# Soltanilara/av-aloha

Measured on AMD Instinct MI355X. Metric: env-steps/sec (whole node) at 4096 parallel envs, SlotInsertion-3Arms, higher is better.
Workload: dtype f32

## Files before the change

### av_aloha_amd/build.py

```python
import os
import subprocess
import sys

HERE = os.path.dirname(os.path.abspath(__file__))
ROOT = os.path.dirname(HERE)
LIB = os.path.join(HERE, "libavsim.so")
SRC = os.path.join(HERE, "csrc")


def _stale(target, sources):
    if not os.path.exists(target):
        return True
    t = os.path.getmtime(target)
    return any(os.path.getmtime(s) > t for s in sources)


def build_hip(force=False, verbose=False):
    srcs = [os.path.join(SRC, f) for f in sorted(os.listdir(SRC)) if not f.endswith(".o") and not f.startswith(".")] + [os.path.join(ROOT, "include", "avsim.h"), os.path.abspath(__file__)]
    if not force and not _stale(LIB, srcs):
        return LIB
    import fcntl
    with open(os.path.join(SRC, ".build.lock"), "w") as lock:
        fcntl.flock(lock, fcntl.LOCK_EX)
        if not force and not _stale(LIB, srcs):
            return LIB
        return _build_hip_locked(verbose)


def _build_hip_locked(verbose):
    hipcc = os.environ.get("HIPCC", "/opt/rocm/bin/hipcc")
    common = [hipcc, "--offload-arch=gfx950", "-std=c++17", "-fPIC", "-fno-gpu-rdc", "-c"]
    F32_FLAGS = ["-O2", "-fno-hip-fp32-correctly-rounded-divide-sqrt", "-fgpu-flush-denormals-to-zero", "-fno-slp-vectorize", "-fno-vectorize",
                 "-mllvm", "-amdgpu-atomic-optimizer-strategy=None", "-mllvm", "-amdgpu-sched-strategy=max-ilp"]
    units = [
        ("avsim_api", F32_FLAGS + (["-DAVSIM_RENDER_STATS"] if os.environ.get("AVSIM_RENDER_STATS") else []) + os.environ.get("AVSIM_EXTRA_FLAGS", "").split()),
        ("avsim_phys_spec", F32_FLAGS + os.environ.get("AVSIM_EXTRA_FLAGS", "").split()),
        ("avsim_phys_f64", ["-O3", "-ffp-contract=off", "-mllvm", "-amdgpu-sched-strategy=max-ilp"] + os.environ.get("AVSIM_EXTRA_FLAGS_F64", "").split()),
        ("avsim_imgaug", ["-O3", "-ffp-contract=off", "-fhip-fp32-correctly-rounded-divide-sqrt", "-fno-gpu-flush-denormals-to-zero"] + os.environ.get("AVSIM_EXTRA_FLAGS_IMGAUG", "").split()),
        ("avsim_chunks", ["-O3", "-ffp-contract=off", "-fhip-fp32-correctly-rounded-divide-sqrt", "-fno-gpu-flush-denormals-to-zero"] + os.environ.get("AVSIM_EXTRA_FLAGS_CHUNKS", "").split()),
        ("avsim_obshist", ["-O3", "-ffp-contract=off", "-fhip-fp32-correctly-rounded-divide-sqrt", "-fno-gpu-flush-denormals-to-zero"] + os.environ.get("AVSIM_EXTRA_FLAGS_OBSHIST", "").split()),
        ("avsim_imgresize", ["-O3", "-ffp-contract=off", "-fhip-fp32-correctly-rounded-divide-sqrt", "-fno-gpu-flush-denormals-to-zero"] + os.environ.get("AVSIM_EXTRA_FLAGS_IMGRESIZE", "").split()),
        ("avsim_pointcloud", ["-O3", "-ffp-contract=off", "-fhip-fp32-correctly-rounded-divide-sqrt", "-fno-gpu-flush-denormals-to-zero"] + os.environ.get("AVSIM_EXTRA_FLAGS_POINTCLOUD", "").split()),
    ]
    procs = []
    for name, extra in units:
        cmd = common + extra + ["-o", os.path.join(SRC, name + ".o"), os.path.join(SRC, name + ".hip")]
        if verbose:
            print(" ".join(cmd), file=sys.stderr)
        procs.append((cmd, subprocess.Popen(cmd)))
    for cmd, p in procs:
        if p.wait() != 0:
            raise subprocess.CalledProcessError(p.returncode, cmd)
    tmp = LIB + ".tmp%d" % os.getpid()
    link = [hipcc, "--offload-arch=gfx950", "-shared", "-fPIC", "-fno-gpu-rdc", "-o", tmp] + [os.path.join(SRC, n + ".o") for n, _ in units]
    if verbose:
        print(" ".join(link).replace(tmp, LIB), file=sys.stderr)
    subprocess.check_call(link)
    os.replace(tmp, LIB)
    return LIB


def build_oracle(force=False):
    d = os.path.join(ROOT, "oracle")
    so = os.path.join(d, "liborc.so")
    srcs = [os.path.join(d, f) for f in os.listdir(d) if f.endswith((".c", ".h"))]
    if force or _stale(so, srcs):
        subprocess.check_call(["make", "-C", d, "-B", "liborc.so"], stdout=subprocess.DEVNULL)
    return so


if __name__ == "__main__":
    print(build_hip(force="--force" in sys.argv, verbose=True))
    print(build_oracle(force="--force" in sys.argv))
```

### av_aloha_amd/csrc/avsim_collide.hip.h

```cpp
#pragma once
#include "avsim_math.hip.h"

namespace avs {

enum { G_SPHERE = 2, G_CYLINDER = 5, G_BOX = 6, G_MESH = 7 };
constexpr int SLOT_W = 24, SLOT_P = 5, SLOT_N = 20, SLOT_MAXC = 5;
constexpr int BOX_MAXC = 8, BOX_SLOTC = 4, BOX_OVF_W = 16;

template <typename T>
struct Shape {
    int type;
    T size[3];
    T pos[3];
    T mat[9];
    GLB_PTR(const T) hull;
    int hbase, hR, hovf;
    int nh;
    T center[3];
    T lc[3], lh[3];
};

template <typename T> struct TieTol;
template <> struct TieTol<double> { static constexpr double rel = 1e-9, len = 1e-12; };
template <> struct TieTol<float> { static constexpr float rel = 1e-5f, len = 1e-7f; };

template <typename T> AVS_DEV T sel3c(const T* v, int k) { return k == 0 ? v[0] : (k == 1 ? v[1] : v[2]); }

template <typename T>
AVS_DEV void support(const Shape<T>& s, const T* d, T* out) {
    T l[3], p[3] = {0, 0, 0};
    mulmatT(s.mat, d, l);
    const T lz = TieTol<T>::rel * (fabs(l[0]) + fabs(l[1]) + fabs(l[2]));
    switch (s.type) {
        case G_SPHERE: {
            T n = sqrt(dot3(l, l));
            if (n > T(0)) { T k = s.size[0] / n; p[0] = k * l[0]; p[1] = k * l[1]; p[2] = k * l[2]; }
            break;
        }
        case G_BOX:
            p[0] = l[0] >= -lz ? s.size[0] : -s.size[0];
            p[1] = l[1] >= -lz ? s.size[1] : -s.size[1];
            p[2] = l[2] >= -lz ? s.size[2] : -s.size[2];
            break;
        case G_CYLINDER: {
            T n = sqrt(l[0] * l[0] + l[1] * l[1]);
            if (n > lz) { T k = s.size[0] / n; p[0] = k * l[0]; p[1] = k * l[1]; }
            p[2] = l[2] >= -lz ? s.size[1] : -s.size[1];
            break;
        }
        default: {
            const T ax = fabs(l[0]), ay = fabs(l[1]), az = fabs(l[2]);
            const int a = (ax >= ay && ax >= az) ? 0 : (ay >= az ? 1 : 2);
            const T lm = sel3c(l, a), am = fabs(lm), inv = am > T(0) ? T(1) / am : T(0);
            const T u = sel3c(l, a == 2 ? 0 : a + 1) * inv, v = sel3c(l, a == 0 ? 2 : a - 1) * inv;
            const int R = s.hR;
            int iu = (int)((u + T(1)) * T(0.5) * T(R)), iv = (int)((v + T(1)) * T(0.5) * T(R));
            iu = iu > 0 ? (iu < R - 1 ? iu : R - 1) : 0;
            iv = iv > 0 ? (iv < R - 1 ? iv : R - 1) : 0;
            GLB_PTR(const T) C = s.hull + 32 * (size_t)(s.hbase + ((2 * a + (lm < T(0) ? 1 : 0)) * R + iu) * R + iv);
            const T tie = TieTol<T>::rel * T(0.1) * (ax + ay + az);
            T vx[8], vy[8], vz[8], pr[8], w0, w1;
#pragma unroll
            for (int k = 0; k < 8; k++) {
                vx[k] = C[4 * k]; vy[k] = C[4 * k + 1]; vz[k] = C[4 * k + 2];
            }
            w0 = C[3]; w1 = C[7];
            const int cnt = (int)w0;
            T bd = T(-1e30);
#pragma unroll
            for (int k = 0; k < 8; k++) { pr[k] = vx[k] * l[0] + vy[k] * l[1] + vz[k] * l[2]; bd = pr[k] > bd ? pr[k] : bd; }
            GLB_PTR(const T) O = s.hull + 4 * ((size_t)s.hovf + (size_t)(cnt > 8 ? (int)w1 : 0));
            const int more = cnt - 8, lastm = more - 1;
            for (int i = 0; i < more; i += 8) {
#pragma unroll
                for (int k = 0; k < 8; k++) {
                    const int ik = i + k < lastm ? i + k : lastm;
                    const T q = O[4 * ik] * l[0] + O[4 * ik + 1] * l[1] + O[4 * ik + 2] * l[2];
                    bd = q > bd ? q : bd;
                }
            }
            const T thr = bd - tie;
            bool found = false;
            T bx = vx[0], by = vy[0], bz = vz[0];
#pragma unroll
            for (int k = 7; k >= 0; k--)
                if (pr[k] >= thr) { bx = vx[k]; by = vy[k]; bz = vz[k]; found = true; }
            for (int i = 0; i < more && !found; i += 8) {
#pragma unroll
                for (int k = 7; k >= 0; k--) {
                    const int ik = i + k < lastm ? i + k : lastm;
                    const T qx = O[4 * ik], qy = O[4 * ik + 1], qz = O[4 * ik + 2];
                    if (qx * l[0] + qy * l[1] + qz * l[2] >= thr) { bx = qx; by = qy; bz = qz; found = true; }
                }
            }
            p[0] = bx; p[1] = by; p[2] = bz;
        }
    }
    mulmat(s.mat, p, out);
    out[0] += s.pos[0]; out[1] += s.pos[1]; out[2] += s.pos[2];
}

template <typename T>
struct MPt {
    T v[3], a[3], b[3];
};

template <typename T>
AVS_DEV void msupport(const Shape<T>& A, const Shape<T>& B, const T* d, MPt<T>& o) {
    T nd[3] = {-d[0], -d[1], -d[2]};
    support(A, d, o.a);
    support(B, nd, o.b);
    sub3(o.a, o.b, o.v);
}

template <typename T>
AVS_DEV T point_tri_dist2(const T* p0, const T* p1, const T* p2, T* w) {
    T e0[3], e1[3];
    sub3(p1, p0, e0);
    sub3(p2, p0, e1);
    T a = dot3(e0, e0), b = dot3(e0, e1), c = dot3(e1, e1), dd = dot3(e0, p0), e = dot3(e1, p0);
    T det = a * c - b * b, s = b * e - c * dd, t = b * dd - a * e;
    if (s + t <= det) {
        if (s < 0) {
            if (t < 0) {
                if (dd < 0) { t = 0; s = (-dd >= a ? T(1) : -dd / a); }
                else { s = 0; t = (e >= 0 ? T(0) : (-e >= c ? T(1) : -e / c)); }
            } else { s = 0; t = (e >= 0 ? T(0) : (-e >= c ? T(1) : -e / c)); }
        } else if (t < 0) { t = 0; s = (dd >= 0 ? T(0) : (-dd >= a ? T(1) : -dd / a)); }
        else { T inv = det > 0 ? T(1) / det : T(0); s *= inv; t *= inv; }
    } else {
        if (s < 0) {
            T t0 = b + dd, t1 = c + e;
            if (t1 > t0) { T num = t1 - t0, den = a - 2 * b + c; s = (num >= den ? T(1) : num / den); t = 1 - s; }
            else { s = 0; t = (t1 <= 0 ? T(1) : (e >= 0 ? T(0) : -e / c)); }
        } else if (t < 0) {
            T t0 = b + e, t1 = a + dd;
            if (t1 > t0) { T num = t1 - t0, den = a - 2 * b + c; t = (num >= den ? T(1) : num / den); s = 1 - t; }
            else { t = 0; s = (t1 <= 0 ? T(1) : (dd >= 0 ? T(0) : -dd / a)); }
        } else {
            T num = (c + e) - (b + dd), den = a - 2 * b + c;
            s = num <= 0 ? T(0) : (num >= den ? T(1) : num / den);
            t = 1 - s;
        }
    }
    for (int i = 0; i < 3; i++) w[i] = p0[i] + s * e0[i] + t * e1[i];
    return dot3(w, w);
}

template <typename T> AVS_DEV void make_frame(const T* n, T* t1, T* t2);
template <typename T> struct MprTol;
template <> struct MprTol<double> { static constexpr double tol = 1e-6, tiny2 = 1e-24, eps = 1e-14; };
template <> struct MprTol<float> { static constexpr float tol = 1e-6f, tiny2 = 1e-16f, eps = 1e-9f; };

template <typename T>
__device__ int mpr_penetration(const Shape<T>& A, const Shape<T>& B, T* depth, T* dir, T* pos) {
    const T tol = MprTol<T>::tol;
    const int maxit = 50;
    MPt<T> v0, v1, v2, v3, v4;
    T d[3], t[3], t2[3];
    sub3(A.center, B.center, v0.v);
    for (int i = 0; i < 3; i++) { v0.a[i] = A.center[i]; v0.b[i] = B.center[i]; }
    if (dot3(v0.v, v0.v) < T(1e-20)) { v0.v[0] = T(1e-5); v0.a[0] += T(1e-5); }
    d[0] = -v0.v[0]; d[1] = -v0.v[1]; d[2] = -v0.v[2];
    normalize3(d);
    msupport(A, B, d, v1);
    if (dot3(v1.v, d) <= 0) return 0;
    cross3(v0.v, v1.v, d);
    if (dot3(d, d) < MprTol<T>::tiny2) {
        T n = sqrt(dot3(v1.v, v1.v));
        *depth = n;
        for (int i = 0; i < 3; i++) { dir[i] = v1.v[i] / n; pos[i] = T(0.5) * (v1.a[i] + v1.b[i]); }
        return 1;
    }
    normalize3(d);
    msupport(A, B, d, v2);
    if (dot3(v2.v, d) <= 0) return 0;
    sub3(v1.v, v0.v, t);
    sub3(v2.v, v0.v, t2);
    cross3(t, t2, d);
    normalize3(d);
    if (dot3(d, v0.v) > 0) { MPt<T> s = v1; v1 = v2; v2 = s; d[0] = -d[0]; d[1] = -d[1]; d[2] = -d[2]; }
    for (int it = 0;; it++) {
        if (it > maxit) return 0;
        msupport(A, B, d, v3);
        if (dot3(v3.v, d) <= 0) return 0;
        cross3(v1.v, v3.v, t);
        if (dot3(t, v0.v) < -MprTol<T>::eps) {
            v2 = v3;
            sub3(v1.v, v0.v, t); sub3(v3.v, v0.v, t2); cross3(t, t2, d); normalize3(d);
            continue;
        }
        cross3(v3.v, v2.v, t);
        if (dot3(t, v0.v) < -MprTol<T>::eps) {
            v1 = v3;
            sub3(v3.v, v0.v, t); sub3(v2.v, v0.v, t2); cross3(t, t2, d); normalize3(d);
            continue;
        }
        break;
    }
    for (int it = 0;; it++) {
        sub3(v2.v, v1.v, t);
        sub3(v3.v, v1.v, t2);
        cross3(t, t2, d);
        if (normalize3(d) == T(0)) return 0;
        msupport(A, B, d, v4);
        T dv1 = dot3(v1.v, d), dv2 = dot3(v2.v, d), dv3 = dot3(v3.v, d), dv4 = dot3(v4.v, d);
        T m = dv4 - dv1;
        if (dv4 - dv2 < m) m = dv4 - dv2;
// ... 280 lines not shown
        { T pv[3]; mulmatT(rmat, rel, pv); poly[3 * q] = pv[0]; poly[3 * q + 1] = pv[1]; poly[3 * q + 2] = pv[2]; }
    }
    int a1 = (ax + 1) % 3, a2 = (ax + 2) % 3;
    AVS_LDS(T) src = poly;
    AVS_LDS(T) dst = tmp;
    for (int side = 0; side < 4; side++) {
        int axis = side < 2 ? a1 : a2;
        T s = (side & 1) ? T(-1) : T(1), lim = sel3(rsize, axis);
        int m = 0;
        const T P0[3] = {src[0], src[1], src[2]};
        T P[3] = {P0[0], P0[1], P0[2]};
        for (int q = 0; q < np; q++) {
            const bool last = q + 1 >= np;
            const int qn = last ? 0 : q + 1;
            T Qp[3] = {src[3 * qn], src[3 * qn + 1], src[3 * qn + 2]};
            if (last) { Qp[0] = P0[0]; Qp[1] = P0[1]; Qp[2] = P0[2]; }
            T dp = s * sel3(P, axis) - lim, dq = s * sel3(Qp, axis) - lim;
            if (dp <= 0 && m < 8) { dst[3 * m] = P[0]; dst[3 * m + 1] = P[1]; dst[3 * m + 2] = P[2]; m++; }
            if (((dp < 0 && dq > 0) || (dp > 0 && dq < 0)) && m < 8) {
                T t = dp / (dp - dq);
                for (int c = 0; c < 3; c++) dst[3 * m + c] = P[c] + t * (Qp[c] - P[c]);
                m++;
            }
            P[0] = Qp[0]; P[1] = Qp[1]; P[2] = Qp[2];
        }
        np = m;
        if (np == 0) return 0;
        AVS_LDS(T) t_ = src; src = dst; dst = t_;
    }
    T refax[3];
    col3(rmat, ax, refax);
    T face = dot3(nr, refax) > 0 ? T(1) : T(-1);
    int m = 0;
    for (int q = 0; q < np; q++) {
        const T px = src[3 * q], py = src[3 * q + 1], pz = src[3 * q + 2];
        const T pc[3] = {px, py, pz};
        T dq = sel3(rsize, ax) - face * sel3(pc, ax);
        if (dq >= 0) { dst[3 * m] = px; dst[3 * m + 1] = py; dst[3 * m + 2] = pz; dep[m] = dq; m++; }
    }
    if (m == 0) return 0;
    const int nk = m < BOX_MAXC ? m : BOX_MAXC;
    for (int x = 0; x < nk; x++) {
        const int q = x;
        T l[3] = {tmp[3 * q], tmp[3 * q + 1], tmp[3 * q + 2]};
#pragma unroll
        for (int j = 0; j < 3; j++) l[j] += (j == ax) ? T(0.5) * dep[q] * face : T(0);
        T wv[3];
        mulmat(rmat, l, wv);
        T dq_ = dep[q];
        if (x < BOX_SLOTC) {
            for (int c = 0; c < 3; c++) scr[SLOT_P + 3 * x + c] = wv[c] + rpos[c];
            scr[x] = -dq_;
        } else {
            ovf[4 * (x - BOX_SLOTC)] = -dq_;
            for (int c = 0; c < 3; c++) ovf[4 * (x - BOX_SLOTC) + 1 + c] = wv[c] + rpos[c];
        }
    }
    for (int c = 0; c < 3; c++) scr[SLOT_N + c] = n[c];
    return nk;
}

template <typename T> AVS_DEV T sel33(const T (*M)[3], int i, int j) { return sel3(i == 0 ? M[0] : (i == 1 ? M[1] : M[2]), j); }
template <typename T> AVS_DEV T row_get(T x, int g16, int l) { return __shfl(x, g16 | l, 64); }

template <typename T, typename OVF>
__device__ int box_box16(const Shape<T>& a, const Shape<T>& b, AVS_LDS(T) scr, AVS_LDS(T) work, OVF ovf, int lane, bool on) {
    const int t = lane & 15, g16 = lane & ~15;
    const unsigned rowmask_sh = g16;
    const T *Ra = a.mat, *Rb = b.mat;
    T p[3], pa[3], pb[3];
    sub3(b.pos, a.pos, p);
    mulmatT(Ra, p, pa);
    mulmatT(Rb, p, pb);
    T R[3][3], Q[3][3];
#pragma unroll
    for (int i = 0; i < 3; i++)
#pragma unroll
        for (int j = 0; j < 3; j++) {
            R[i][j] = Ra[i] * Rb[j] + Ra[3 + i] * Rb[3 + j] + Ra[6 + i] * Rb[6 + j];
            Q[i][j] = fabs(R[i][j]) + T(1e-12);
        }
    T sv = T(-1e30);
    bool skip = t >= 15;
    bool flipv = false;
    T bnv[3] = {0, 0, 0};
    if (t < 3) {
        const int i = t;
        sv = fabs(sel3(pa, i)) - (sel3(a.size, i) + b.size[0] * sel33(Q, i, 0) + b.size[1] * sel33(Q, i, 1) + b.size[2] * sel33(Q, i, 2));
        flipv = sel3(pa, i) < 0;
    } else if (t < 6) {
        const int j = t - 3;
        sv = fabs(sel3(pb, j)) - (sel3(b.size, j) + a.size[0] * sel33(Q, 0, j) + a.size[1] * sel33(Q, 1, j) + a.size[2] * sel33(Q, 2, j));
        flipv = sel3(pb, j) < 0;
    } else if (t < 15) {
        const int i = (t - 6) / 3, j = (t - 6) % 3;
        const int i1 = (i + 1) % 3, i2 = (i + 2) % 3, j1 = (j + 1) % 3, j2 = (j + 2) % 3;
        T c[3] = {sel3(R[0], j), sel3(R[1], j), sel3(R[2], j)}, e[3] = {i == 0 ? T(1) : T(0), i == 1 ? T(1) : T(0), i == 2 ? T(1) : T(0)}, ax[3];
        cross3(e, c, ax);
        const T l = sqrt(dot3(ax, ax));
        if (l < T(1e-8)) skip = true;
        else {
            T sep = fabs(dot3(pa, ax)) - (sel3(a.size, i1) * sel33(Q, i2, j) + sel3(a.size, i2) * sel33(Q, i1, j) + sel3(b.size, j1) * sel33(Q, i, j2) + sel3(b.size, j2) * sel33(Q, i, j1));
            sep /= l;
            sv = sep;
            T axn[3] = {ax[0] / l, ax[1] / l, ax[2] / l};
            flipv = dot3(pa, axn) < 0;
            mulmat(Ra, axn, bnv);
        }
    }
    {
        const unsigned long long sepm = __ballot(!skip && sv > 0);
        if ((sepm >> g16) & 0xffffull) return 0;
    }
    T best = T(-1e30);
    int code = -1;
    const T fudge = T(1.05);
    const unsigned skipm = (unsigned)((__ballot(skip) >> g16) & 0xffffull);
#pragma unroll
    for (int k = 0; k < 15; k++) {
// ... 86 lines not shown
        const int qn = t + 1 >= np ? 0 : t + 1;
        const T Qp[3] = {row_get(P[0], g16, qn), row_get(P[1], g16, qn), row_get(P[2], g16, qn)};
        const T dp = s * sel3(P, axis) - lim, dq = s * sel3(Qp, axis) - lim;
        const bool live = t < np;
        const bool e1 = live && dp <= 0, e2 = live && ((dp < 0 && dq > 0) || (dp > 0 && dq < 0));
        const unsigned m1 = (unsigned)((__ballot(e1) >> g16) & 0xffffull), m2 = (unsigned)((__ballot(e2) >> g16) & 0xffffull);
        const unsigned below = (1u << t) - 1u;
        const int off = __popc(m1 & below) + __popc(m2 & below);
        if (e1 && off < 8) { dst[3 * off] = P[0]; dst[3 * off + 1] = P[1]; dst[3 * off + 2] = P[2]; }
        if (e2 && off + (e1 ? 1 : 0) < 8) {
            const int o2 = off + (e1 ? 1 : 0);
            const T tt = dp / (dp - dq);
            for (int c = 0; c < 3; c++) dst[3 * o2 + c] = P[c] + tt * (Qp[c] - P[c]);
        }
        const int total = __popc(m1) + __popc(m2);
        np = total < 8 ? total : 8;
        if (np == 0) return 0;
        __builtin_amdgcn_fence(__ATOMIC_ACQ_REL, "wavefront");
        __builtin_amdgcn_wave_barrier();
        const int rq = t < np ? t : 0;
        P[0] = dst[3 * rq]; P[1] = dst[3 * rq + 1]; P[2] = dst[3 * rq + 2];
        __builtin_amdgcn_fence(__ATOMIC_ACQ_REL, "wavefront");
        __builtin_amdgcn_wave_barrier();
        dst = dst == tmp ? poly : tmp;
    }
    T refax[3];
    col3(rmat, ax, refax);
    const T face = dot3(nr, refax) > 0 ? T(1) : T(-1);
    int m;
    {
        const T dqv = sel3(rsize, ax) - face * sel3(P, ax);
        const bool kp = t < np && dqv >= 0;
        const unsigned km = (unsigned)((__ballot(kp) >> g16) & 0xffffull);
        const int off = __popc(km & ((1u << t) - 1u));
        if (kp) { tmp[3 * off] = P[0]; tmp[3 * off + 1] = P[1]; tmp[3 * off + 2] = P[2]; dep[off] = dqv; }
        m = __popc(km);
        if (m == 0) return 0;
        __builtin_amdgcn_fence(__ATOMIC_ACQ_REL, "wavefront");
        __builtin_amdgcn_wave_barrier();
    }
    const int nk = m < BOX_MAXC ? m : BOX_MAXC;
    if (on && t < nk) {
        const int q = t;
        T l[3] = {tmp[3 * q], tmp[3 * q + 1], tmp[3 * q + 2]};
        const T dq_ = dep[q];
#pragma unroll
        for (int j = 0; j < 3; j++) l[j] += (j == ax) ? T(0.5) * dq_ * face : T(0);
        T wv[3];
        mulmat(rmat, l, wv);
        if (t < BOX_SLOTC) {
            for (int c = 0; c < 3; c++) scr[SLOT_P + 3 * t + c] = wv[c] + rpos[c];
            scr[t] = -dq_;
        } else {
            ovf[4 * (t - BOX_SLOTC)] = -dq_;
            for (int c = 0; c < 3; c++) ovf[4 * (t - BOX_SLOTC) + 1 + c] = wv[c] + rpos[c];
        }
    }
    if (on && t == 0) { for (int c = 0; c < 3; c++) scr[SLOT_N + c] = n[c]; }
    (void)rowmask_sh;
    return nk;
}

template <typename T>
AVS_DEV bool boxes_separated(const Shape<T>& a, const Shape<T>& b) {
    T ca[3], cb[3], t[3];
    mulmat(a.mat, a.lc, ca);
    mulmat(b.mat, b.lc, cb);
    for (int k = 0; k < 3; k++) t[k] = (b.pos[k] + cb[k]) - (a.pos[k] + ca[k]);
    T R[3][3];
    for (int i = 0; i < 3; i++)
        for (int j = 0; j < 3; j++) R[i][j] = fabs(a.mat[i] * b.mat[j] + a.mat[3 + i] * b.mat[3 + j] + a.mat[6 + i] * b.mat[6 + j]) + T(1e-6);
    for (int i = 0; i < 3; i++) {
        T ta = fabs(t[0] * a.mat[i] + t[1] * a.mat[3 + i] + t[2] * a.mat[6 + i]);
        if (ta > a.lh[i] + b.lh[0] * R[i][0] + b.lh[1] * R[i][1] + b.lh[2] * R[i][2]) return true;
    }
    for (int j = 0; j < 3; j++) {
        T tb = fabs(t[0] * b.mat[j] + t[1] * b.mat[3 + j] + t[2] * b.mat[6 + j]);
        if (tb > b.lh[j] + a.lh[0] * R[0][j] + a.lh[1] * R[1][j] + a.lh[2] * R[2][j]) return true;
    }
    return false;
}

template <typename T>
__device__ int narrow(const Shape<T>& a, const Shape<T>& b, AVS_LDS(T) scr) {
    int ta = a.type, tb = b.type;
    if (boxes_separated(a, b)) return 0;
    T dist[1], pos[3], nrm[3];
    int n;
    if (ta == G_SPHERE && tb == G_SPHERE) n = sphere_sphere(a, b, dist, pos, nrm);
    else if (ta == G_SPHERE && tb == G_BOX) n = sphere_box(a, b, dist, pos, nrm);
    else if (ta == G_BOX && tb == G_SPHERE) {
        n = sphere_box(b, a, dist, pos, nrm);
        nrm[0] = -nrm[0]; nrm[1] = -nrm[1]; nrm[2] = -nrm[2];
    } else {
        T depth;
        n = mpr_penetration(a, b, &depth, nrm, pos);
        dist[0] = -depth;
    }
    if (n) {
        scr[0] = dist[0];
        for (int k = 0; k < 3; k++) { scr[SLOT_P + k] = pos[k]; scr[SLOT_N + k] = nrm[k]; }
    }
    return n;
}

template <typename T>
AVS_DEV void make_frame(const T* n, T* t1, T* t2) {
    t1[0] = t1[1] = t1[2] = 0;
    if (n[1] < T(0.5) && n[1] > T(-0.5)) t1[1] = 1; else t1[2] = 1;
    T d = dot3(n, t1);
    t1[0] -= d * n[0]; t1[1] -= d * n[1]; t1[2] -= d * n[2];
    normalize3(t1);
    cross3(n, t1, t2);
}

}
```

### av_aloha_amd/csrc/avsim_math.hip.h

```cpp
#pragma once
#include <hip/hip_runtime.h>

namespace avs {

#define AVS_DEV __device__ __forceinline__
#ifndef AVS_NTC_MASK
#define AVS_NTC_MASK 6
#endif
#define AVS_OUTLINE __attribute__((noinline))
#define AVS_OUTLINE_NTC __attribute__((noinline, not_tail_called))
#if (AVS_NTC_MASK) & 1
#define AVS_OUTLINE_0 AVS_OUTLINE_NTC
#else
#define AVS_OUTLINE_0 AVS_OUTLINE
#endif
#if (AVS_NTC_MASK) & 2
#define AVS_OUTLINE_1 AVS_OUTLINE_NTC
#else
#define AVS_OUTLINE_1 AVS_OUTLINE
#endif
#if (AVS_NTC_MASK) & 4
#define AVS_OUTLINE_2 AVS_OUTLINE_NTC
#else
#define AVS_OUTLINE_2 AVS_OUTLINE
#endif
#if (AVS_NTC_MASK) & 8
#define AVS_OUTLINE_3 AVS_OUTLINE_NTC
#else
#define AVS_OUTLINE_3 AVS_OUTLINE
#endif
#if (AVS_NTC_MASK) & 16
#define AVS_OUTLINE_4 AVS_OUTLINE_NTC
#else
#define AVS_OUTLINE_4 AVS_OUTLINE
#endif
#if (AVS_NTC_MASK) & 32
#define AVS_OUTLINE_5 AVS_OUTLINE_NTC
#else
#define AVS_OUTLINE_5 AVS_OUTLINE
#endif
#ifndef GLB_PTR
#define GLB_PTR(T) __attribute__((address_space(1))) T*
#endif

template <typename T> AVS_DEV T dot3(const T* a, const T* b) { return a[0] * b[0] + a[1] * b[1] + a[2] * b[2]; }
template <typename T> AVS_DEV void cross3(const T* a, const T* b, T* c) {
    T t0 = a[1] * b[2] - a[2] * b[1], t1 = a[2] * b[0] - a[0] * b[2], t2 = a[0] * b[1] - a[1] * b[0];
    c[0] = t0; c[1] = t1; c[2] = t2;
}
template <typename T> AVS_DEV void sub3(const T* a, const T* b, T* c) { c[0] = a[0] - b[0]; c[1] = a[1] - b[1]; c[2] = a[2] - b[2]; }
template <typename T> AVS_DEV T normalize3(T* a) {
    T n = sqrt(dot3(a, a));
    if (n > T(0)) { T i = T(1) / n; a[0] *= i; a[1] *= i; a[2] *= i; }
    return n;
}
template <typename T, typename M> AVS_DEV void mulmat(const M* R, const T* v, T* o) {
    T t0 = (T)R[0] * v[0] + (T)R[1] * v[1] + (T)R[2] * v[2], t1 = (T)R[3] * v[0] + (T)R[4] * v[1] + (T)R[5] * v[2],
      t2 = (T)R[6] * v[0] + (T)R[7] * v[1] + (T)R[8] * v[2];
    o[0] = t0; o[1] = t1; o[2] = t2;
}
template <typename T, typename M> AVS_DEV void mulmatT(const M* R, const T* v, T* o) {
    T t0 = (T)R[0] * v[0] + (T)R[3] * v[1] + (T)R[6] * v[2], t1 = (T)R[1] * v[0] + (T)R[4] * v[1] + (T)R[7] * v[2],
      t2 = (T)R[2] * v[0] + (T)R[5] * v[1] + (T)R[8] * v[2];
    o[0] = t0; o[1] = t1; o[2] = t2;
}
template <typename T> AVS_DEV void quat2mat(const T* q, T* R) {
    T w = q[0], x = q[1], y = q[2], z = q[3];
    R[0] = 1 - 2 * (y * y + z * z); R[1] = 2 * (x * y - w * z); R[2] = 2 * (x * z + w * y);
    R[3] = 2 * (x * y + w * z); R[4] = 1 - 2 * (x * x + z * z); R[5] = 2 * (y * z - w * x);
    R[6] = 2 * (x * z - w * y); R[7] = 2 * (y * z + w * x); R[8] = 1 - 2 * (x * x + y * y);
}
template <typename T> AVS_DEV void quatmul(const T* a, const T* b, T* c) {
    T t0 = a[0] * b[0] - a[1] * b[1] - a[2] * b[2] - a[3] * b[3], t1 = a[0] * b[1] + a[1] * b[0] + a[2] * b[3] - a[3] * b[2],
      t2 = a[0] * b[2] - a[1] * b[3] + a[2] * b[0] + a[3] * b[1], t3 = a[0] * b[3] + a[1] * b[2] - a[2] * b[1] + a[3] * b[0];
    c[0] = t0; c[1] = t1; c[2] = t2; c[3] = t3;
}
template <typename T> AVS_DEV void quatnorm(T* q) {
    T n = sqrt(q[0] * q[0] + q[1] * q[1] + q[2] * q[2] + q[3] * q[3]);
    if (n < T(1e-15)) { q[0] = 1; q[1] = q[2] = q[3] = 0; return; }
    T i = T(1) / n;
    q[0] *= i; q[1] *= i; q[2] *= i; q[3] *= i;
}
template <typename T> AVS_DEV T tmax(T a, T b) { return a > b ? a : b; }
template <typename T> AVS_DEV T tmin(T a, T b) { return a < b ? a : b; }
template <typename T> AVS_DEV T tclamp(T x, T lo, T hi) { return x < lo ? lo : (x > hi ? hi : x); }

}
```

### av_aloha_amd/csrc/avsim_newton.hip.h

```cpp
#pragma once
#include "avsim_math.hip.h"

namespace avs {

typedef float nv4f __attribute__((ext_vector_type(4)));
typedef double nv2d __attribute__((ext_vector_type(2)));
AVS_DEV void load_row16(GLB_PTR(const float) src, float* v) {
    GLB_PTR(const nv4f) p = (GLB_PTR(const nv4f))src;
    nv4f a = p[0], b = p[1], c = p[2], d = p[3];
    asm volatile("" : "+v"(a), "+v"(b), "+v"(c), "+v"(d));
    v[0] = a.x; v[1] = a.y; v[2] = a.z; v[3] = a.w; v[4] = b.x; v[5] = b.y; v[6] = b.z; v[7] = b.w;
    v[8] = c.x; v[9] = c.y; v[10] = c.z; v[11] = c.w; v[12] = d.x; v[13] = d.y; v[14] = d.z; v[15] = d.w;
}
AVS_DEV void load_row16(GLB_PTR(const double) src, double* v) {
    GLB_PTR(const nv2d) p = (GLB_PTR(const nv2d))src;
    nv2d t[8];
#pragma unroll
    for (int q = 0; q < 8; q++) t[q] = p[q];
    asm volatile("" : "+v"(t[0]), "+v"(t[1]), "+v"(t[2]), "+v"(t[3]), "+v"(t[4]), "+v"(t[5]), "+v"(t[6]), "+v"(t[7]));
#pragma unroll
    for (int q = 0; q < 8; q++) { v[2 * q] = t[q].x; v[2 * q + 1] = t[q].y; }
}

template <typename real>
struct NewtonArgs {
    LDS_PTR(real) rowS;
    LDS_PTR(const int) rowI;
    LDS_PTR(const int) rmeta;
    GLB_PTR(const real) rJ;
    LDS_PTR(const real) M;
    LDS_PTR(real) a;
    LDS_PTR(const real) as;
    LDS_PTR(real) H;
    LDS_PTR(real) g;
    LDS_PTR(real) dl;
    LDS_PTR(real) jv;
    LDS_PTR(const int) cefc;
    LDS_PTR(const int) tree_dofadr;
    LDS_PTR(const int) tree_dofnum;
    LDS_PTR(const int) tree_madr;
    LDS_PTR(const int) dof_tree;
    LDS_PTR(int) prof;
    int nv, nefc, ncon, nlead, ntree, iters;
    real tol, scale, ls_tol;
    int ls_iters;
    int early_exit;
    int k_a0, k_n, k_mb;
};

enum { NR_EQ = 0, NR_FLOSS = 1, NR_LIMIT = 2, NR_CONTACT = 3 };
constexpr int NVMAX = 48;

template <typename real>
AVS_DEV real nrow_dot(const NewtonArgs<real>& A, int i, LDS_PTR(const real) v) {
    const int ra = A.rowI[i];
    const int a0 = ra & 63, nA = (ra >> 6) & 15, b0 = (ra >> 13) & 63, nB = (ra >> 19) & 15;
    GLB_PTR(const real) J = A.rJ + ROW_S * i;
    real s = 0;
#pragma unroll
    for (int k = 0; k < TREE_W; k++) {
        const real ja = J[k], va = v[k < nA ? a0 + k : 0], jb = J[TREE_W + k], vb = v[k < nB ? b0 + k : 0];
        s += (k < nA ? ja * va : real(0)) + (k < nB ? jb * vb : real(0));
    }
    return s;
}

template <typename real>
AVS_DEV real nrow_dot_lead(const NewtonArgs<real>& A, int i, LDS_PTR(const real) v) {
    const int ra = A.rowI[i];
    const int d1 = (ra & 63) + ((ra >> 26) & 7), d2 = (ra & 63) + ((ra >> 29) & 7);
    const real v1 = ((ra >> 13) & 1) ? real(-1) : real(1), v2 = A.rowS[RS_S * i + 7];
    return v1 * v[d1] + v2 * v[d2];
}

template <typename real>
AVS_DEV void nrow_scalar(int type, real z, real R, real eta, real* f, real* h) {
    const real D = real(1) / R;
    if (type == NR_EQ) { *f = -D * z; *h = D; }
    else if (type == NR_FLOSS) {
        if (z <= -R * eta) { *f = eta; *h = 0; }
        else if (z >= R * eta) { *f = -eta; *h = 0; }
        else { *f = -D * z; *h = D; }
    } else {
        if (z < 0) { *f = -D * z; *h = D; } else { *f = 0; *h = 0; }
    }
}

template <typename real>
AVS_DEV real nrow_scalar_cost(int type, real z, real R, real eta) {
    const real D = real(1) / R;
    if (type == NR_EQ) return real(0.5) * D * z * z;
    if (type == NR_FLOSS) {
        if (z <= -R * eta) return -eta * z - real(0.5) * R * eta * eta;
        if (z >= R * eta) return eta * z - real(0.5) * R * eta * eta;
        return real(0.5) * D * z * z;
    }
    return z < 0 ? real(0.5) * D * z * z : real(0);
}

template <typename real>
struct NCon {
    int head, dim;
    real S[6];
    real D[6];
    real mu, Dm;
};

template <typename real>
AVS_DEV int ncone(const NCon<real>& c, const real* jar, real* f, real* cost, real* w, real* c1, real* c2, real* s1, real* s2) {
#pragma unroll
// ... 21 lines not shown
    f[0] = -c.Dm * NT * mu;
    *cost = real(0.5) * c.Dm * NT * NT;
    c1[0] = mu; *s1 = c.Dm; *s2 = kap;
#pragma unroll
    for (int j = 1; j < 6; j++)
        if (j < c.dim) {
            const real us = U[j] * Ti * c.S[j];
            f[j] = -f[0] * us;
            w[j] = kap * c.S[j] * c.S[j];
            c1[j] = -mu * us;
            c2[j] = us;
        }
    return 2;
}

template <typename real>
AVS_DEV void ncone_ls(const NCon<real>& c, const real* jar, const real* jv, real* d1, real* d2) {
    *d1 = 0; *d2 = 0;
    if (c.dim == 1) {
        if (jar[0] < 0) { *d1 = c.D[0] * jar[0] * jv[0]; *d2 = c.D[0] * jv[0] * jv[0]; }
        return;
    }
    real U[6], V[6], t2 = 0, uv = 0, v2 = 0;
    U[0] = jar[0] * c.mu; V[0] = jv[0] * c.mu;
#pragma unroll
    for (int j = 1; j < 6; j++) {
        U[j] = j < c.dim ? jar[j] * c.S[j] : real(0);
        V[j] = j < c.dim ? jv[j] * c.S[j] : real(0);
        t2 += U[j] * U[j]; uv += U[j] * V[j]; v2 += V[j] * V[j];
    }
    const real N = U[0], T = sqrt(t2), mu = c.mu;
    if (N >= mu * T || (T <= 0 && N >= 0)) return;
    if (mu * N + T <= 0 || (T <= 0 && N < 0)) {
#pragma unroll
        for (int j = 0; j < 6; j++)
            if (j < c.dim) { *d1 += c.D[j] * jar[j] * jv[j]; *d2 += c.D[j] * jv[j] * jv[j]; }
        return;
    }
    const real Ti = real(1) / T, T1 = uv * Ti, T2 = (v2 - T1 * T1) * Ti, NT = N - mu * T, N1 = V[0] - mu * T1;
    *d1 = c.Dm * NT * N1;
    *d2 = c.Dm * N1 * N1 - c.Dm * NT * mu * T2;
}

AVS_DEV int nslot_dof(int ra, int s) {
    const int sh = s < TREE_W ? 0 : 13, k = s & (TREE_W - 1);
    return k < ((ra >> (sh + 6)) & 15) ? ((ra >> sh) & 63) + k : -1;
}

AVS_DEV int lead_d1(int ra) { return (ra & 63) + ((ra >> 26) & 7); }
AVS_DEV int lead_d2(int ra) { return (ra & 63) + ((ra >> 29) & 7); }
template <typename real> AVS_DEV real lead_v1(int ra) { return ((ra >> 13) & 1) ? real(-1) : real(1); }

template <typename real>
AVS_DEV void rows_jt_force(LDS_PTR(const real) rowS, LDS_PTR(const int) rowI, LDS_PTR(const int) cefc, GLB_PTR(const real) rJ, LDS_PTR(real) out,
                           int nlead, int ncon, int lane, real sgn) {
    for (int i = lane; i < nlead; i += 64) {
        const real f = rowS[RS_S * i + 6];
        if (f == 0) continue;
        const int ra = rowI[i];
        const real v2 = rowS[RS_S * i + 7];
        __hip_atomic_fetch_add(out + lead_d1(ra), sgn * lead_v1<real>(ra) * f, __ATOMIC_RELAXED, __HIP_MEMORY_SCOPE_WORKGROUP);
        if (v2 != 0) __hip_atomic_fetch_add(out + lead_d2(ra), sgn * v2 * f, __ATOMIC_RELAXED, __HIP_MEMORY_SCOPE_WORKGROUP);
    }
    const int t = lane & 15;
    for (int c0 = 0; c0 < ncon; c0 += 4) {
        const int c = c0 + (lane >> 4);
        const int ce = c < ncon ? cefc[c] : -1;
        const bool on = ce >= 0;
        const int head = on ? (ce & 0xffff) : 0, dim = on ? (ce >> 16) : 0;
        const int ra = rowI[head];
        real acc = 0;
#pragma unroll
        for (int p = 0; p < 6; p++) {
            const int row = head + (p < dim ? p : 0);
            const real Jp = rJ[ROW_S * row + t], fp = rowS[RS_S * row + 6];
            acc += p < dim ? Jp * fp : real(0);
        }
        const int dof = on ? nslot_dof(ra, t) : -1;
        if (dof >= 0 && acc != 0) __hip_atomic_fetch_add(out + dof, sgn * acc, __ATOMIC_RELAXED, __HIP_MEMORY_SCOPE_WORKGROUP);
    }
}

template <typename real>
AVS_DEV void nblock4_load(const NewtonArgs<real>& A, int lane, int r0, int dim, bool on, real* Jraw) {
    const int t = lane & 15;
    GLB_PTR(const real) J = A.rJ + ROW_S * (on ? r0 : 0);
#pragma unroll
    for (int p = 0; p < 6; p++) Jraw[p] = J[ROW_S * (p < dim ? p : 0) + t];
}
template <typename real, bool BATCH>
AVS_DEV void nblock4(const NewtonArgs<real>& A, int lane, int r0, int dim, bool on, bool full, const real* w, int c, const real* cc1, const real* cc2, real cs1, real cs2,
                     const real* Jraw) {
    const int ra = A.rowI[on ? r0 : 0], t = lane & 15, gq = on ? nslot_dof(ra, t) : -1;
    real Jt[6];
#pragma unroll
    for (int p = 0; p < 6; p++) Jt[p] = (on && p < dim) ? Jraw[p] : real(0);
    const bool two = __any(on && ((ra >> 19) & 15) > 0);
    const int smax = two ? 16 : 8;
    if (!__any(full)) {
        if (!two) {
            const int tc = lane & 7, s0 = (lane & 8) >> 1, gqc = on ? nslot_dof(ra, tc) : -1;
            GLB_PTR(const real) J = A.rJ + ROW_S * (on ? r0 : 0);
            real Jc[6], Js[4][6];
#pragma unroll
            for (int p = 0; p < 6; p++) {
                GLB_PTR(const real) Jp = J + ROW_S * (p < dim ? p : 0);
                Jc[p] = Jp[tc];
#pragma unroll
                for (int u = 0; u < 4; u++) Js[u][p] = Jp[s0 + u];
            }
#pragma unroll
            for (int u = 0; u < 4; u++) {
                const int s = s0 + u, gp = nslot_dof(ra, s);
                real acc = 0;
#pragma unroll
                for (int p = 0; p < 6; p++) acc += (on && p < dim) ? w[p] * Js[u][p] * Jc[p] : real(0);
                if (on && gp >= 0 && gqc >= 0 && gqc <= gp) __hip_atomic_fetch_add(A.H + gp * (gp + 1) / 2 + gqc, acc, __ATOMIC_RELAXED, __HIP_MEMORY_SCOPE_WORKGROUP);
            }
            return;
        }
        if constexpr (BATCH) {
            for (int s0 = 0; s0 < smax; s0 += 8) {
                real js[8][6];
#pragma unroll
                for (int u = 0; u < 8; u++)
#pragma unroll
                    for (int p = 0; p < 6; p++) js[u][p] = __shfl(Jt[p], (lane & 48) | (s0 + u), 64);
#pragma unroll
                for (int u = 0; u < 8; u++) {
                    const int gp = nslot_dof(ra, s0 + u);
                    real acc = 0;
#pragma unroll
                    for (int p = 0; p < 6; p++) acc += w[p] * js[u][p] * Jt[p];
                    if (on && gp >= 0 && gq >= 0 && gq <= gp) __hip_atomic_fetch_add(A.H + gp * (gp + 1) / 2 + gq, acc, __ATOMIC_RELAXED, __HIP_MEMORY_SCOPE_WORKGROUP);
                }
            }
            return;
        }
        for (int s = 0; s < smax; s++) {
            const int gp = nslot_dof(ra, s);
            real acc = 0;
#pragma unroll
            for (int p = 0; p < 6; p++) acc += w[p] * __shfl(Jt[p], (lane & 48) | s, 64) * Jt[p];
            if (on && gp >= 0 && gq >= 0 && gq <= gp) __hip_atomic_fetch_add(A.H + gp * (gp + 1) / 2 + gq, acc, __ATOMIC_RELAXED, __HIP_MEMORY_SCOPE_WORKGROUP);
        }
        return;
    }
    real c1[6], c2[6], y1t = 0, y2t = 0;
#pragma unroll
    for (int p = 0; p < 6; p++) { c1[p] = __shfl(cc1[p], c & 63, 64); c2[p] = __shfl(cc2[p], c & 63, 64); }
    const real s1 = __shfl(cs1, c & 63, 64), s2 = __shfl(cs2, c & 63, 64);
#pragma unroll
    for (int p = 0; p < 6; p++) { y1t += c1[p] * Jt[p]; y2t += c2[p] * Jt[p]; }
    if constexpr (BATCH) {
        for (int s0 = 0; s0 < smax; s0 += 8) {
            real jsb[8][6];
#pragma unroll
            for (int u = 0; u < 8; u++)
#pragma unroll
// ... 266 lines not shown
    const real og = A.g[omine ? a0 + i8 : 0];
    real ox = omine ? (FWD ? -og : og) : real(0);
    const int md = c.mydof, rb = md * (md + 1) / 2;
    const bool cm = lane < nc;
    const real cg = A.g[cm ? md : 0];
    real x = cm ? (FWD ? -cg : cg) : real(0);
    const real dinv = cm ? real(1) / A.H[rb + md] : real(0);
    if (nc < nv) {
#pragma unroll
        for (int jj = 0; jj < TREE_W; jj++) {
            const int j = FWD ? jj : TREE_W - 1 - jj;
            const real xj = oct_bcast_n(ox * odinv, j);
            ox = i8 == j ? xj : ox - ocf[j] * xj;
        }
    }
    if (FWD) {
        int cn = __builtin_amdgcn_readlane(md, 0);
        real Lnext = (lane > 0 && cm) ? A.H[rb + cn] : real(0);
        for (int j = 0; j < nc; j++) {
            const real Lc = Lnext;
            if (j + 1 < nc) { cn = __builtin_amdgcn_readlane(md, j + 1); Lnext = (lane > j + 1 && cm) ? A.H[rb + cn] : real(0); }
            const real yj = lane_get(x * dinv, j);
            if (lane == j) x = yj;
            else if (lane > j) x -= Lc * yj;
        }
    } else {
        int cn = __builtin_amdgcn_readlane(md, nc - 1);
        real Lnext = lane < nc - 1 ? A.H[cn * (cn + 1) / 2 + md] : real(0);
        for (int i = nc - 1; i >= 0; i--) {
            const real Lc = Lnext;
            if (i > 0) { cn = __builtin_amdgcn_readlane(md, i - 1); Lnext = lane < i - 1 ? A.H[cn * (cn + 1) / 2 + md] : real(0); }
            const real xi = lane_get(x * dinv, i);
            if (lane == i) x = xi;
            else if (lane < i) x -= Lc * xi;
        }
    }
    NSYNC();
    LDS_PTR(real) out = FWD ? A.g : A.dl;
    if (cm) out[md] = x;
    if (nc < nv && omine) out[a0 + i8] = ox;
}

template <typename real, int NCH, bool COUPLED, typename KA>
__device__ __attribute__((always_inline)) int newton_solve(KA ka, GLB_PTR(const real) rows, LDS_PTR(real) r_, LDS_PTR(int) ii_, LDS_PTR(const int) li_, int nefc, int ncon, int nlead,
                                                      int iters, real tol, real scale, int profiling) {
    const int lane = threadIdx.x & 63;
    NewtonArgs<real> A;
    {
        LDS_PTR(real) r = (LDS_PTR(real))(unsigned long long)(unsigned)__builtin_amdgcn_readfirstlane((int)(unsigned)(unsigned long long)r_);
        LDS_PTR(int) ii = (LDS_PTR(int))(unsigned long long)(unsigned)__builtin_amdgcn_readfirstlane((int)(unsigned)(unsigned long long)ii_);
        LDS_PTR(const int) li = (LDS_PTR(const int))(unsigned long long)(unsigned)__builtin_amdgcn_readfirstlane((int)(unsigned)(unsigned long long)li_);
        tol = lane_get(tol, 0); scale = lane_get(scale, 0);
        A.rowS = r + ka->lay.rowS; A.rowI = ii + ka->lay.rowI; A.rmeta = ii + ka->lay.rmeta;
        {
            const unsigned long long p_ = (unsigned long long)rows;
            A.rJ = (GLB_PTR(const real))(((unsigned long long)(unsigned)__builtin_amdgcn_readfirstlane((int)(unsigned)(p_ >> 32)) << 32) | (unsigned)__builtin_amdgcn_readfirstlane((int)(unsigned)p_));
        }
        A.M = r + ka->lay.M; A.a = r + ka->lay.qacc; A.as = r + ka->lay.asm_;
        A.H = r + ka->lay.nH; A.g = r + ka->lay.ng; A.dl = r + ka->lay.ndl; A.jv = r + ka->lay.njv;
        A.cefc = ii + ka->lay.cefc;
        A.prof = profiling ? ii + ka->lay.nprof : (LDS_PTR(int))nullptr;
        A.tree_dofadr = li + ka->mo.tree_dofadr; A.tree_dofnum = li + ka->mo.tree_dofnum; A.tree_madr = li + ka->mo.tree_madr; A.dof_tree = li + ka->mo.dof_tree;
        A.nv = __builtin_amdgcn_readfirstlane(ka->m.nv); A.ntree = __builtin_amdgcn_readfirstlane(ka->m.ntree);
        A.nefc = __builtin_amdgcn_readfirstlane(nefc); A.ncon = __builtin_amdgcn_readfirstlane(ncon);
        A.nlead = __builtin_amdgcn_readfirstlane(nlead); A.iters = __builtin_amdgcn_readfirstlane(iters);
        A.tol = tol; A.scale = scale; A.ls_tol = ka->m.ls_tolerance; A.ls_iters = __builtin_amdgcn_readfirstlane(ka->m.ls_iterations);
        A.early_exit = __builtin_amdgcn_readfirstlane(ka->m.newton_early_exit);
    }
    const int nv = A.nv, ne = A.nefc;
    {
        const int k = lane < nv ? lane : 0, t = A.dof_tree[k];
        A.k_a0 = A.tree_dofadr[t]; A.k_n = A.tree_dofnum[t]; A.k_mb = A.tree_madr[t] + (k - A.k_a0) * A.k_n;
    }
    int used = 0;
    constexpr bool coupled = COUPLED;
    NComp comp;
    if constexpr (coupled) comp = ncomponent<real>(A, lane, ne, (LDS_PTR(int))A.dl, __builtin_amdgcn_readfirstlane(ka->m.newton_component) == 0);
    long long tp0 = A.prof ? __builtin_readcyclecounter() : 0;
    NCon<real> con[NCH];
#pragma unroll
    for (int ch = 0; ch < NCH; ch++) {
        NCon<real>& c = con[ch];
        const int ci = ch * 64 + lane;
        const int ce = ci < A.ncon ? A.cefc[ci] : -1;
        c.head = ce >= 0 ? (ce & 0xffff) : -1;
        c.dim = ce >= 0 ? (ce >> 16) : 0;
        c.mu = 0; c.Dm = 0;
#pragma unroll
        for (int j = 0; j < 6; j++) { c.S[j] = 0; c.D[j] = 0; }
        if (c.head >= 0) {
#pragma unroll
            for (int j = 0; j < 6; j++)
                if (j < c.dim) { c.D[j] = real(1) / A.rowS[RS_S * (c.head + j) + 1]; if (j > 0) c.S[j] = real(1) / A.rowS[RS_S * (c.head + j) + 7]; }
            if (c.dim > 1) {
                const real R0 = A.rowS[RS_S * c.head + 1], R1 = A.rowS[RS_S * (c.head + 1) + 1];
                c.mu = c.S[1] * sqrt(R1 / R0);
                c.S[0] = c.mu;
                c.Dm = (real(1) / R0) / tmax(real(1e-15), c.mu * c.mu * (1 + c.mu * c.mu));
            }
        }
    }
    const bool jar_ready = true;
    {
        const real c1 = ncost<real, NCH>(A, lane, con, A.as, 8, false);
        const real c0 = ncost<real, NCH>(A, lane, con, (LDS_PTR(const real))A.a, 2);
        if (!(c0 < c1)) {
            for (int k = lane; k < nv; k += 64) A.a[k] = A.as[k];
            for (int i = lane; i < ne; i += 64) A.rowS[RS_S * i + 2] = A.rowS[RS_S * i + 8];
        }
        NSYNC();
// ... 197 lines not shown
            if (fabs(dphi) < A.ls_tol * fabs(dphi0)) break;
            if (dphi < 0) lo = alpha; else hi = alpha;
            real nx = alpha - dphi / ddphi;
            if (hi < 0) { if (!(nx > lo)) nx = 2 * alpha + real(1e-12); }
            else if (!(nx > lo && nx < hi) || fabs(nx - alpha) > real(0.5) * fabs(dxold)) nx = real(0.5) * (lo + hi);
            dxold = dx;
            dx = nx - alpha;
            if (fabs(nx - alpha) < (sizeof(real) == 8 ? real(1e-14) : real(1e-7)) * (1 + fabs(alpha))) { alpha = nx; break; }
            alpha = nx;
        }
        NPROF(4);
#ifdef AVSIM_DEBUG_NEWTON
        if (lane == 0 && A.iters == 99) printf("      line search: dphi0 %.6e alpha %.6e q1 %.6e q2 %.6e lo %.6e hi %.6e  same-H %d middle %d\n", (double)dphi0, (double)alpha, (double)q1, (double)q2, (double)lo, (double)hi, (int)(same && !middle), (int)middle);
#endif
        if (!(dphi0 < 0)) break;
        real st2 = 0;
        for (int k = lane; k < nv; k += 64) { const real s = alpha * A.dl[k]; A.a[k] += s; st2 += s * s; }
        alpha_prev = alpha;
        st2 = wave_sum(st2);
        NSYNC();
        if (sqrt(st2) * A.scale < real(1e-2) * A.tol) break;
        if (real(-0.5) * alpha * dphi0 * A.scale < A.tol) break;
    }
    if (!forces_current) {
        for (int i = lane; i < ne; i += 64) A.rowS[RS_S * i + 2] = (i < A.nlead ? nrow_dot_lead(A, i, (LDS_PTR(const real))A.a) : nrow_dot(A, i, (LDS_PTR(const real))A.a)) - A.rowS[RS_S * i];
        NSYNC();
        for (int i = lane; i < A.nlead; i += 64) {
            real f, h;
            nrow_scalar<real>(A.rmeta[i] & 3, A.rowS[RS_S * i + 2], A.rowS[RS_S * i + 1], A.rowS[RS_S * i + 5], &f, &h);
            A.rowS[RS_S * i + 6] = f;
        }
    #pragma unroll
        for (int ch = 0; ch < NCH; ch++) {
            if (ch * 64 >= A.ncon) break;
            const NCon<real>& c = con[ch];
            if (c.head >= 0) {
                real jar[6], f[6], w[6], c1[6], c2[6], cc, s1, s2;
    #pragma unroll
                for (int j = 0; j < 6; j++) jar[j] = j < c.dim ? A.rowS[RS_S * (c.head + j) + 2] : real(0);
                ncone(c, jar, f, &cc, w, c1, c2, &s1, &s2);
    #pragma unroll
                for (int j = 0; j < 6; j++) if (j < c.dim) A.rowS[RS_S * (c.head + j) + 6] = f[j];
            }
        }
    }
    NSYNC();
    NPROF(5);
    return used;
}

template <typename real, int NCH, typename KA>
__device__ AVS_OUTLINE_5 int newton_solve_coupled(KA ka, GLB_PTR(const real) rows, LDS_PTR(real) r_, LDS_PTR(int) ii_, LDS_PTR(const int) li_, int nefc, int ncon, int nlead,
                                                              int iters, real tol, real scale, int profiling) {
    return newton_solve<real, NCH, true>(ka, rows, r_, ii_, li_, nefc, ncon, nlead, iters, tol, scale, profiling);
}

}
```

### av_aloha_amd/csrc/avsim_phys.hip.h

```cpp
#pragma once
#include <hip/hip_runtime.h>

#include <cstddef>
#include <cstring>
#include <string>
#include <type_traits>
#include <vector>

#include "avsim_collide.hip.h"
#include "avsim_dev.h"
#include "avsim_math.hip.h"
#include "avsim_model.h"
#include "avsim_phys_layout.h"

namespace avs {

enum { J_FREE = 0, J_BALL = 1, J_SLIDE = 2, J_HINGE = 3 };
enum { R_EQ = 0, R_FLOSS = 1, R_LIMIT = 2, R_CONTACT = 3 };
constexpr int TREE_W = 8;
constexpr int ROW_W = 2 * TREE_W;
constexpr int ROW_S = ROW_W;
constexpr int CAND_MAX = 256;
constexpr int PROF_W = 26;
constexpr int NEAR_MAX = 512;
// ... 272 lines not shown
        case 4: return oct_bcast<4>(x); case 5: return oct_bcast<5>(x); case 6: return oct_bcast<6>(x); default: return oct_bcast<7>(x);
    }
}
AVS_DEV float lane_get(float x, int l) { return __builtin_bit_cast(float, __builtin_amdgcn_readlane(__builtin_bit_cast(int, x), l)); }
AVS_DEV double lane_get(double x, int l) {
    const long long b = __builtin_bit_cast(long long, x);
    const unsigned lo = (unsigned)__builtin_amdgcn_readlane((int)(unsigned)b, l), hi = (unsigned)__builtin_amdgcn_readlane((int)(unsigned)(b >> 32), l);
    return __builtin_bit_cast(double, ((long long)hi << 32) | (long long)lo);
}

constexpr int GRP_MAX = 6;
constexpr int GA_W = 64, GA_Q = 16, GA_QW = 6;
template <typename T> AVS_DEV T qdiv(T t, T d, T dinv) { return sizeof(T) == 4 ? t * dinv : t / d; }
AVS_DEV float qrsqrt(float x) { return __builtin_amdgcn_rsqf(x); }
AVS_DEV double qrsqrt(double x) { return 1.0 / sqrt(x); }
template <typename T> struct QTol;
template <> struct QTol<double> { static constexpr double abs = 1e-10, rel = 0.0; };
template <> struct QTol<float> { static constexpr float abs = 1e-10f, rel = 2e-6f; };

template <bool B> struct BoolTag { static constexpr bool value = B; };

template <typename real>
struct NoslipLead {
    LDS_PTR(const real) Minv;
    LDS_PTR(const int) tadr;
    LDS_PTR(const int) tnum;
    LDS_PTR(const int) floss_dof;
    LDS_PTR(int) dmap;
    LDS_PTR(int) prof;
    int tridiag;
    int ntree, nv, neq, nfloss, nlg;
};

typedef int nl_v4 __attribute__((ext_vector_type(4)));
#define NL_PARAMS nl_v4 nl_a_, nl_v4 nl_b_, nl_v4 nl_c_
#define NL_ARGS(nl) nl_pack_a(nl), nl_pack_b(nl), nl_pack_c(nl)
#define NL_UNPACK(real) NoslipLead<real> nl = nl_unpack<real>(nl_a_, nl_b_, nl_c_)
template <typename real> AVS_DEV nl_v4 nl_pack_a(const NoslipLead<real>& n) {
    return nl_v4{(int)(__SIZE_TYPE__)n.Minv, (int)(__SIZE_TYPE__)n.tadr, (int)(__SIZE_TYPE__)n.tnum, (int)(__SIZE_TYPE__)n.floss_dof};
}
template <typename real> AVS_DEV nl_v4 nl_pack_b(const NoslipLead<real>& n) { return nl_v4{(int)(__SIZE_TYPE__)n.dmap, (int)(__SIZE_TYPE__)n.prof, n.tridiag, n.ntree}; }
template <typename real> AVS_DEV nl_v4 nl_pack_c(const NoslipLead<real>& n) { return nl_v4{n.nv, n.neq, n.nfloss, n.nlg}; }
template <typename real> AVS_DEV NoslipLead<real> nl_unpack(nl_v4 a, nl_v4 b, nl_v4 c) {
    NoslipLead<real> n;
    n.Minv = (LDS_PTR(const real))(__SIZE_TYPE__)(unsigned)a.x; n.tadr = (LDS_PTR(const int))(__SIZE_TYPE__)(unsigned)a.y; n.tnum = (LDS_PTR(const int))(__SIZE_TYPE__)(unsigned)a.z;
    n.floss_dof = (LDS_PTR(const int))(__SIZE_TYPE__)(unsigned)a.w; n.dmap = (LDS_PTR(int))(__SIZE_TYPE__)(unsigned)b.x; n.prof = (LDS_PTR(int))(__SIZE_TYPE__)(unsigned)b.y;
    n.tridiag = b.z; n.ntree = b.w; n.nv = c.x; n.neq = c.y; n.nfloss = c.z; n.nlg = c.w;
    return n;
}

template <typename T> AVS_DEV LDS_PTR(T) uni_lds(LDS_PTR(T) p) {
    return (LDS_PTR(T))(unsigned long long)(unsigned)__builtin_amdgcn_readfirstlane((int)(unsigned)(unsigned long long)p);
}
template <typename T> AVS_DEV GLB_PTR(T) uni_glb(GLB_PTR(T) p) {
    const unsigned long long v = (unsigned long long)p;
    return (GLB_PTR(T))(((unsigned long long)(unsigned)__builtin_amdgcn_readfirstlane((int)(unsigned)(v >> 32)) << 32) | (unsigned)__builtin_amdgcn_readfirstlane((int)(unsigned)v));
}

template <typename T> AVS_DEV T secular_step(T val, T r2, T r, T yw) {
    const T yy = val + r2, ny = sqrt(yy);
    return val * yy / ((ny + r) * r * yw);
}

template <typename real>
__device__ AVS_OUTLINE_2 void pgs_groups(LDS_PTR(real) rowS, LDS_PTR(const int) rowI, GLB_PTR(const real) rJ, GLB_PTR(const real) rB,
                                                     LDS_PTR(real) q, LDS_PTR(const int) gI, GLB_PTR(const real) gA, int ngrp, int iters,
                                                     int noslip_iters, real noslip_tol_scaled, NL_PARAMS) {
    NL_UNPACK(real);
    const long long tent = __builtin_readcyclecounter();
    rowS = uni_lds(rowS); rowI = uni_lds(rowI); q = uni_lds(q); gI = uni_lds(gI);
    rJ = uni_glb(rJ); rB = uni_glb(rB); gA = uni_glb(gA);
    ngrp = __builtin_amdgcn_readfirstlane(ngrp); iters = __builtin_amdgcn_readfirstlane(iters); noslip_iters = __builtin_amdgcn_readfirstlane(noslip_iters);
    noslip_tol_scaled = lane_get(noslip_tol_scaled, 0);
    nl.Minv = uni_lds(nl.Minv); nl.tadr = uni_lds(nl.tadr); nl.tnum = uni_lds(nl.tnum); nl.floss_dof = uni_lds(nl.floss_dof); nl.dmap = uni_lds(nl.dmap); nl.prof = uni_lds(nl.prof);
    nl.ntree = __builtin_amdgcn_readfirstlane(nl.ntree); nl.nv = __builtin_amdgcn_readfirstlane(nl.nv); nl.neq = __builtin_amdgcn_readfirstlane(nl.neq);
    nl.nfloss = __builtin_amdgcn_readfirstlane(nl.nfloss); nl.nlg = __builtin_amdgcn_readfirstlane(nl.nlg); nl.tridiag = __builtin_amdgcn_readfirstlane(nl.tridiag);
    const int lane = threadIdx.x & 63, d = lane >> 3, k8 = lane & 7, dr = d < GRP_MAX ? d : 0;
    const int lr = lane < GRP_MAX ? lane : 0;
    const int tri = lr * (lr - 1) / 2;
    if (ngrp <= 0) return;
    const bool fl = noslip_iters > 0 && nl.nlg >= 0;
    const int ft = lane >> 3, fi = lane & 7, fgb = lane & ~7;
    bool fm = false;
    int fdof = 0, frow = -1;
    real mrow[TREE_W], faref = 0, finv = 0, fdiag = 0, flo = 0, fhi = 0;
#pragma unroll
    for (int s = 0; s < TREE_W; s++) mrow[s] = 0;
    if (fl) {
        for (int k = lane; k < nl.nv; k += 64) nl.dmap[k] = -1;
        __builtin_amdgcn_fence(__ATOMIC_ACQ_REL, "wavefront");
        __builtin_amdgcn_wave_barrier();
        for (int r = lane; r < nl.nfloss; r += 64) nl.dmap[nl.floss_dof[r]] = nl.neq + r;
        __builtin_amdgcn_fence(__ATOMIC_ACQ_REL, "wavefront");
        __builtin_amdgcn_wave_barrier();
        fm = ft < nl.ntree && fi < nl.tnum[ft < nl.ntree ? ft : 0];
        fdof = fm ? nl.tadr[ft] + fi : 0;
        frow = fm ? nl.dmap[fdof] : -1;
        if (fm) {
#pragma unroll
            for (int s = 0; s < TREE_W; s++) mrow[s] = nl.Minv[64 * ft + 8 * fi + s];
        }
        LDS_PTR(const real) FS = rowS + RS_S * (frow >= 0 ? frow : 0);
        faref = FS[0]; finv = frow >= 0 ? FS[3] : real(0); flo = FS[4]; fhi = FS[5];
        fdiag = finv != 0 ? real(1) / finv : real(0);
    }
    real imp = 0, imp_c = 0;
#ifdef AVSIM_PROBE_ROWS
    LDS_PTR(int) prof = (LDS_PTR(int))nullptr;
#else
    LDS_PTR(int) prof = nl.prof;
// ... 952 lines not shown
                        const real sq = v0 * v0 / (dq0 * dq0) + v1 * v1 / (dq1 * dq1);
                        const real sc = sqrt(r2 / tmax(real(1e-15), sq));
                        v0 *= sc; v1 *= sc;
                    }
                }
                const real change = (v0 - of0) * (real(0.5) * (A00 * (v0 - of0) + A10 * (v1 - of1)) + resq0) + (v1 - of1) * (real(0.5) * (A10 * (v0 - of0) + A11 * (v1 - of1)) + resq1);
                if (!(change > real(1e-10)) && dim == 3) {
                    if (fi == 0 && cur.side == 0) imp -= change;
                    if (fi == 1) f = v0;
                    if (fi == 2) f = v1;
                }
            }
            const real dl = row ? f - cur.f0 : real(0);
#pragma unroll
            for (int r = 1; r < GRP_MAX; r++) x += (r < dim ? cur.B[r] : real(0)) * oct_bcast_n(dl, r);
            if (row && cur.side == 0) rowS[RS_S * (cur.h + fi) + 8] = f;
        };
        rem = chain;
        fetch(0, ca);
        for (int step = 0; step < nstep; step += 2) {
            fetch(step + 1, cb);
            one_step(ca);
            if (step + 1 < nstep) {
                fetch(step + 2, ca);
                one_step(cb);
            }
        }
        if (__any(slid)) { if (prof && lane == 0) prof[2] += 1; return 0; }
        __builtin_amdgcn_fence(__ATOMIC_ACQ_REL, "wavefront");
        __builtin_amdgcn_wave_barrier();
        if (lane_get(wave_sum(imp), 0) < noslip_tol_scaled) break;
    }
    return 1;
    };
    if (!(__any(tB >= 0) ? sweeps(BoolTag<true>{}) : sweeps(BoolTag<false>{}))) return 0;
    if (prof && lane == 0) prof[3] += 1;
    if (fm) q[fdof] = x;
    if (frow >= 0) FS[8] = ff;
    __builtin_amdgcn_fence(__ATOMIC_ACQ_REL, "wavefront");
    __builtin_amdgcn_wave_barrier();
    for (int i = lane; i < nefc; i += 64) rowS[RS_S * i + 6] = rowS[RS_S * i + 8];
    __builtin_amdgcn_fence(__ATOMIC_ACQ_REL, "wavefront");
    __builtin_amdgcn_wave_barrier();
    return 1;
}


}
#include "avsim_newton.hip.h"
namespace avs {

typedef float avs_v4f __attribute__((ext_vector_type(4)));
typedef double avs_v2d __attribute__((ext_vector_type(2)));
AVS_DEV void store_row16(GLB_PTR(float) dst, const float* v) {
#pragma unroll
    for (int q = 0; q < 4; q++) { avs_v4f t = {v[4 * q], v[4 * q + 1], v[4 * q + 2], v[4 * q + 3]}; ((GLB_PTR(avs_v4f))dst)[q] = t; }
}
AVS_DEV void store_row16(GLB_PTR(double) dst, const double* v) {
#pragma unroll
    for (int q = 0; q < 8; q++) { avs_v2d t = {v[2 * q], v[2 * q + 1]}; ((GLB_PTR(avs_v2d))dst)[q] = t; }
}

AVS_DEV void lds_load8(const float* p, float* v) {
    LDS_PTR(const avs_v4f) q = (LDS_PTR(const avs_v4f))p;
    const avs_v4f a = q[0], b = q[1];
    v[0] = a.x; v[1] = a.y; v[2] = a.z; v[3] = a.w; v[4] = b.x; v[5] = b.y; v[6] = b.z; v[7] = b.w;
}
AVS_DEV void lds_load8(const double* p, double* v) {
    LDS_PTR(const avs_v2d) q = (LDS_PTR(const avs_v2d))p;
#pragma unroll
    for (int k = 0; k < 4; k++) { const avs_v2d a = q[k]; v[2 * k] = a.x; v[2 * k + 1] = a.y; }
}

template <int G>
AVS_DEV unsigned long long group_mask(int grp) {
    if (G == 64) return ~0ull;
    return ((1ull << G) - 1ull) << (grp * G);
}
template <int G>
AVS_DEV int group_rank(bool flag, int grp, int lane, int* total) {
    unsigned long long b = __ballot(flag) & group_mask<G>(grp);
    unsigned long long lower = (G == 64) ? ((1ull << lane) - 1ull) : (((1ull << lane) - 1ull) << (grp * G));
    *total = __popcll(b);
    return __popcll(b & lower);
}

template <typename real>
struct SInert {
    real m, h[3], I[6];
};

template <typename real, typename KA>
AVS_DEV void body_inertia(KA ka, const real* xmat, const real* xipos, int b, SInert<real>& s) {
    const real* R = xmat + 9 * b;
    GLB_PTR(const real) Ib = ka->m.body_inertia + 6 * b;
    real I3[9] = {Ib[0], Ib[3], Ib[4], Ib[3], Ib[1], Ib[5], Ib[4], Ib[5], Ib[2]}, T[9], Ic[9];
#pragma unroll
    for (int i = 0; i < 3; i++)
#pragma unroll
        for (int j = 0; j < 3; j++) T[3 * i + j] = R[3 * i] * I3[j] + R[3 * i + 1] * I3[3 + j] + R[3 * i + 2] * I3[6 + j];
#pragma unroll
    for (int i = 0; i < 3; i++)
#pragma unroll
        for (int j = 0; j < 3; j++) Ic[3 * i + j] = T[3 * i] * R[3 * j] + T[3 * i + 1] * R[3 * j + 1] + T[3 * i + 2] * R[3 * j + 2];
    real ms = ka->m.body_mass[b];
    real c[3] = {xipos[3 * b], xipos[3 * b + 1], xipos[3 * b + 2]};
    real cc = dot3(c, c);
    s.m = ms;
    s.h[0] = ms * c[0]; s.h[1] = ms * c[1]; s.h[2] = ms * c[2];
    s.I[0] = Ic[0] + ms * (cc - c[0] * c[0]); s.I[1] = Ic[4] + ms * (cc - c[1] * c[1]); s.I[2] = Ic[8] + ms * (cc - c[2] * c[2]);
    s.I[3] = Ic[1] - ms * c[0] * c[1]; s.I[4] = Ic[2] - ms * c[0] * c[2]; s.I[5] = Ic[5] - ms * c[1] * c[2];
}

template <typename real>
AVS_DEV void inert_mul(const real* s , const real* mv, real* f) {
    const real *w = mv, *v = mv + 3, *h = s + 1, *I = s + 4;
    real hv[3], hw[3];
    cross3(h, v, hv);
    cross3(h, w, hw);
    f[0] = I[0] * w[0] + I[3] * w[1] + I[4] * w[2] + hv[0];
    f[1] = I[3] * w[0] + I[1] * w[1] + I[5] * w[2] + hv[1];
    f[2] = I[4] * w[0] + I[5] * w[1] + I[2] * w[2] + hv[2];
    f[3] = s[0] * v[0] - hw[0]; f[4] = s[0] * v[1] - hw[1]; f[5] = s[0] * v[2] - hw[2];
}

template <typename real>
AVS_DEV void cross_motion(const real* v, const real* s, real* o) {
    real a[3], b[3], c[3];
    cross3(v, s, a);
    cross3(v, s + 3, b);
    cross3(v + 3, s, c);
    o[0] = a[0]; o[1] = a[1]; o[2] = a[2];
    o[3] = b[0] + c[0]; o[4] = b[1] + c[1]; o[5] = b[2] + c[2];
}
template <typename real>
AVS_DEV void cross_force(const real* v, const real* f, real* o) {
    real a[3], b[3], c[3];
    cross3(v, f, a);
    cross3(v + 3, f + 3, b);
    cross3(v, f + 3, c);
    o[0] = a[0] + b[0]; o[1] = a[1] + b[1]; o[2] = a[2] + b[2];
    o[3] = c[0]; o[4] = c[1]; o[5] = c[2];
}

template <typename real>
AVS_DEV void chol_block(const real* A, real* L, int n) {
    for (int j = 0; j < n; j++) {
        real dd = A[j * n + j];
        for (int k = 0; k < j; k++) dd -= L[j * n + k] * L[j * n + k];
        dd = sqrt(tmax(dd, real(1e-30)));
        L[j * n + j] = dd;
        real inv = real(1) / dd;
        for (int i = j + 1; i < n; i++) {
            real s = A[i * n + j];
            for (int k = 0; k < j; k++) s -= L[i * n + k] * L[j * n + k];
            L[i * n + j] = s * inv;
        }
    }
// ... 77 lines not shown
            if (tl && tr) rw = 1;
            if (tl && tr && !a_table) rw = 2;
            if (ab && !a_table) rw = 3;
            if (cd) rw = 4;
    }
    return rw;
}
#if !defined(AVSIM_TU_F64) && !defined(AVSIM_NO_F32_LAUNCH)
__global__ void k_reward_pairs(GLB_PTR(const int) geom_class, int ngeom, int task_id, const int* __restrict__ pairs, int n, int cap, int* __restrict__ latch, int* __restrict__ reward) {
    const int i = blockIdx.x * blockDim.x + threadIdx.x;
    if (i >= n) return;
    int f = 0;
    for (int c = 0; c < cap; c++) {
        const int g1 = pairs[((size_t)i * cap + c) * 2], g2 = pairs[((size_t)i * cap + c) * 2 + 1];
        if (g1 < 0 || g2 < 0 || g1 >= ngeom || g2 >= ngeom) continue;
        f |= reward_pair_flags(geom_class[g1], geom_class[g2], task_id);
    }
    int l = latch ? latch[i] : 0;
    reward[i] = reward_from_flags(f, task_id, &l);
    if (latch) latch[i] = l;
}
#endif


template <typename real, int G, typename SPEC = GenericSpec>
struct Env {
    KRef<real, SPEC> ka;
    int env = 0;
    int diverged = 0;
    int nit_sum = 0, nit_max = 0;
    bool profiling = false;
    real* r;
    int* ii;
    int lane, grp;
    const real* lr;
    const int* li;
    long long t_broad = 0, t_narrow = 0;
    __device__ Env(KRef<real, SPEC> ka_, real* r_, int* i_, int lane_, int grp_, const real* lr_, const int* li_)
        : ka(ka_), r(r_), ii(i_), lane(lane_), grp(grp_), lr(lr_), li(li_) {}
    AVS_DEV const int* LI() const {
        const int* p = li;
        if constexpr (spec_fixed<SPEC>) p = lds_at<const int>((unsigned)(ka->mo.nreal * sizeof(real)));
        AVS_ASSUME_LDS(p);
        return p;
    }
    AVS_DEV const real* LR() const {
        const real* p = lr;
        if constexpr (spec_fixed<SPEC>) p = lds_at<const real>(0u);
        AVS_ASSUME_LDS(p);
        return p;
    }
    AVS_DEV int nobj_() const { if constexpr (spec_fixed<SPEC>) return SPEC::nobj; else return ka->m.nobj; }
    AVS_DEV int hull_ovf_() const { if constexpr (spec_fixed<SPEC>) return SPEC::hull_ovf; else return ka->m.hull_ovf; }
    AVS_DEV GLB_PTR(real) rows_() const { return (GLB_PTR(real))ka->m.rJ_glob + (size_t)env * ka->lay.gefc * ROW_S; }
    AVS_DEV GLB_PTR(real) rowsB_() const { return (GLB_PTR(real))ka->m.rB_glob + (size_t)env * ka->lay.gefc * ROW_S; }
    AVS_DEV GLB_PTR(real) coup_() const { return (GLB_PTR(real))ka->m.gA_glob + (size_t)env * ka->lay.ggrp * GA_W; }
    AVS_DEV GLB_PTR(int) near_() const { return (GLB_PTR(int))ka->m.near_glob + (size_t)env * NEAR_MAX; }
    AVS_DEV GLB_PTR(int) cand_() const { return (GLB_PTR(int))ka->m.cand_glob + (size_t)env * CAND_MAX; }
    AVS_DEV GLB_PTR(real) bxo_() const { return (GLB_PTR(real))ka->m.bxo_glob + (size_t)env * 64 * BOX_OVF_W; }
    AVS_DEV GLB_PTR(real) gref_() const { return (GLB_PTR(real))ka->m.gref_glob + (size_t)env * ka->m.ngeom * 3; }
    AVS_DEV const int* body_parent_() const { return LI() + ka->mo.body_parent; }
    AVS_DEV const int* body_jntadr_() const { return LI() + ka->mo.body_jntadr; }
    AVS_DEV const int* body_jntnum_() const { return LI() + ka->mo.body_jntnum; }
    AVS_DEV const int* body_dofadr_() const { return LI() + ka->mo.body_dofadr; }
    AVS_DEV const int* body_dofnum_() const { return LI() + ka->mo.body_dofnum; }
    AVS_DEV const int* body_tree_() const { return LI() + ka->mo.body_tree; }
    AVS_DEV const int* body_dofmask_() const { return LI() + ka->mo.body_dofmask; }
    AVS_DEV const int* body_last_() const { return LI() + ka->mo.body_last; }
    AVS_DEV const int* tree_bodyadr_() const { return LI() + ka->mo.tree_bodyadr; }
    AVS_DEV const int* tree_bodylist_() const { return LI() + ka->mo.tree_bodylist; }
    AVS_DEV const int* tree_dofadr_() const { return LI() + ka->mo.tree_dofadr; }
    AVS_DEV const int* tree_dofnum_() const { return LI() + ka->mo.tree_dofnum; }
    AVS_DEV const int* tree_madr_() const { return LI() + ka->mo.tree_madr; }
    AVS_DEV const int* jnt_type_() const { return LI() + ka->mo.jnt_type; }
    AVS_DEV const int* jnt_qposadr_() const { return LI() + ka->mo.jnt_qposadr; }
    AVS_DEV const int* jnt_dofadr_() const { return LI() + ka->mo.jnt_dofadr; }
    AVS_DEV const int* jnt_actfrclimited_() const { return LI() + ka->mo.jnt_actfrclimited; }
    AVS_DEV const int* limited_jnt_() const { return LI() + ka->mo.limited_jnt; }
    AVS_DEV const int* dof_body_() const { return LI() + ka->mo.dof_body; }
    AVS_DEV const int* dof_parent_() const { return LI() + ka->mo.dof_parent; }
    AVS_DEV const int* dof_tree_() const { return LI() + ka->mo.dof_tree; }
    AVS_DEV const int* dof_jnt_() const { return LI() + ka->mo.dof_jnt; }
    AVS_DEV const int* floss_dof_() const { return LI() + ka->mo.floss_dof; }
    AVS_DEV const int* ment_i_() const { return LI() + ka->mo.ment_i; }
    AVS_DEV const int* ment_j_() const { return LI() + ka->mo.ment_j; }
    AVS_DEV const int* act_dof_() const { return LI() + ka->mo.act_dof; }
    AVS_DEV const int* act_qposadr_() const { return LI() + ka->mo.act_qposadr; }
    AVS_DEV const int* act_ctrllimited_() const { return LI() + ka->mo.act_ctrllimited; }
    AVS_DEV const int* geom_type_() const { return LI() + ka->mo.geom_type; }
    AVS_DEV const int* geom_body_() const { return LI() + ka->mo.geom_body; }
    AVS_DEV const int* geom_static_() const { return LI() + ka->mo.geom_static; }
    AVS_DEV const real* body_pos_() const { return LR() + ka->mo.body_pos; }
    AVS_DEV const real* body_quat_() const { return LR() + ka->mo.body_quat; }
    AVS_DEV const real* body_mass_() const { return LR() + ka->mo.body_mass; }
    AVS_DEV const real* body_ipos_() const { return LR() + ka->mo.body_ipos; }
    AVS_DEV const real* body_inertia_() const { return LR() + ka->mo.body_inertia; }
    AVS_DEV const real* body_invweight0_() const { return LR() + ka->mo.body_invweight0; }
    AVS_DEV const real* jnt_pos_() const { return LR() + ka->mo.jnt_pos; }
    AVS_DEV const real* jnt_axis_() const { return LR() + ka->mo.jnt_axis; }
    AVS_DEV const real* jnt_range_() const { return LR() + ka->mo.jnt_range; }
    AVS_DEV const real* jnt_actfrcrange_() const { return LR() + ka->mo.jnt_actfrcrange; }
    AVS_DEV const real* jnt_margin_() const { return LR() + ka->mo.jnt_margin; }
    AVS_DEV const real* dof_armature_() const { return LR() + ka->mo.dof_armature; }
    AVS_DEV const real* dof_damping_() const { return LR() + ka->mo.dof_damping; }
    AVS_DEV const real* dof_frictionloss_() const { return LR() + ka->mo.dof_frictionloss; }
    AVS_DEV const real* dof_invweight0_() const { return LR() + ka->mo.dof_invweight0; }
    AVS_DEV const real* act_kp_() const { return LR() + ka->mo.act_kp; }
    AVS_DEV const real* act_kv_() const { return LR() + ka->mo.act_kv; }
    AVS_DEV const real* act_gear_() const { return LR() + ka->mo.act_gear; }
    AVS_DEV const real* act_ctrlrange_() const { return LR() + ka->mo.act_ctrlrange; }
    AVS_DEV const real* geom_cpos_() const { return LR() + ka->mo.geom_cpos; }
    AVS_DEV const real* geom_rbound_() const { return LR() + ka->mo.geom_rbound; }

// ... 7 lines not shown
        for (int k = 0; k < TREE_W; k++) row[k] = (i < n && k <= i) ? A[base + i * n + k] : (k == i ? real(1) : real(0));
        if (diag_add && i < n) {
#pragma unroll
            for (int k = 0; k < TREE_W; k++) if (k == i) row[k] += diag_scale * diag_add[a0 + i];
        }
#pragma unroll
        for (int j = 0; j < TREE_W; j++) {
            const real d = sqrt(tmax(oct_bcast_n(row[j], j), real(1e-30)));
            const real lij = i == j ? d : row[j] / d;
            row[j] = lij;
            const real mul = i > j ? lij : real(0);
#pragma unroll
            for (int k = j + 1; k < TREE_W; k++) row[k] -= mul * oct_bcast_n(lij, k);
        }
        if (i < n) {
#pragma unroll
            for (int k = 0; k < TREE_W; k++) if (k <= i) Ldst[base + i * n + k] = row[k];
        }
    }
    __device__ real tree_solve(const real* L, real x) {
        const int t = lane >> 3, i = lane & 7, gb = lane & ~7;
        const bool act = t < ka->m.ntree;
        const int n = act ? tree_dofnum_()[t] : 0, base = act ? tree_madr_()[t] : 0;
        real row[TREE_W], col[TREE_W];
#pragma unroll
        for (int k = 0; k < TREE_W; k++) {
            row[k] = (i < n && k < i) ? L[base + i * n + k] : real(0);
            col[k] = (k < n && k > i) ? L[base + k * n + i] : real(0);
        }
        const real dinv = i < n ? real(1) / L[base + i * n + i] : real(1);
        if (!(i < n)) x = 0;
#pragma unroll
        for (int j = 0; j < TREE_W; j++) {
            const real yj = oct_bcast_n(x * dinv, j);
            x = i == j ? yj : x - row[j] * yj;
        }
#pragma unroll
        for (int j = TREE_W - 1; j >= 0; j--) {
            const real xj = oct_bcast_n(x * dinv, j);
            x = i == j ? xj : x - col[j] * xj;
        }
        return x;
    }

    __device__ void kinematics() {
        PHASE_BEGIN();
        real *xpos = r + ka->lay.xpos, *xmat = r + ka->lay.xmat, *xipos = r + ka->lay.xipos, *cdof = r + ka->lay.cdof, *qpos = r + ka->lay.qpos;
        int* anc = ii + ka->lay.cand;
        const int nb = ka->m.nbody;
        for (int b = lane; b < nb; b += G) {
            real R[9], pos[3];
            int a = -1;
            if (body_tree_()[b] < 0) {
                for (int k = 0; k < 3; k++) pos[k] = ka->m.static_xpos[3 * b + k];
                for (int k = 0; k < 9; k++) R[k] = ka->m.static_xmat[9 * b + k];
            } else {
                const int p = body_parent_()[b], ja = body_jntadr_()[b], jn = body_jntnum_()[b];
                const int jt = jn > 0 ? jnt_type_()[ja] : -1;
                if (jt == J_FREE) {
                    const int qa = jnt_qposadr_()[ja];
                    real quat[4];
                    for (int k = 0; k < 3; k++) pos[k] = qpos[qa + k];
                    for (int k = 0; k < 4; k++) quat[k] = qpos[qa + 3 + k];
                    quatnorm(quat);
                    quat2mat(quat, R);
                } else {
                    real Rl[9], bq[4] = {body_quat_()[4 * b], body_quat_()[4 * b + 1], body_quat_()[4 * b + 2], body_quat_()[4 * b + 3]};
                    quat2mat(bq, Rl);
                    for (int k = 0; k < 3; k++) pos[k] = body_pos_()[3 * b + k];
                    for (int k = 0; k < 9; k++) R[k] = Rl[k];
                    if (jt == J_HINGE) {
                        const real q = qpos[jnt_qposadr_()[ja]];
                        const real ax[3] = {jnt_axis_()[3 * ja], jnt_axis_()[3 * ja + 1], jnt_axis_()[3 * ja + 2]};
                        const real jp[3] = {jnt_pos_()[3 * ja], jnt_pos_()[3 * ja + 1], jnt_pos_()[3 * ja + 2]};
                        const real sn = sin(q), co = cos(q), oc = 1 - co;
                        const real Rq[9] = {co + ax[0] * ax[0] * oc, ax[0] * ax[1] * oc - ax[2] * sn, ax[0] * ax[2] * oc + ax[1] * sn,
                                            ax[1] * ax[0] * oc + ax[2] * sn, co + ax[1] * ax[1] * oc, ax[1] * ax[2] * oc - ax[0] * sn,
                                            ax[2] * ax[0] * oc - ax[1] * sn, ax[2] * ax[1] * oc + ax[0] * sn, co + ax[2] * ax[2] * oc};
                        for (int i = 0; i < 3; i++)
                            for (int j = 0; j < 3; j++) R[3 * i + j] = Rl[3 * i] * Rq[j] + Rl[3 * i + 1] * Rq[3 + j] + Rl[3 * i + 2] * Rq[6 + j];
                        real t0[3], t1[3];
                        mulmat(Rl, jp, t0);
                        mulmat(R, jp, t1);
                        for (int k = 0; k < 3; k++) pos[k] += t0[k] - t1[k];
                    } else if (jt == J_SLIDE) {
                        const real q = qpos[jnt_qposadr_()[ja]];
                        const real ax[3] = {jnt_axis_()[3 * ja], jnt_axis_()[3 * ja + 1], jnt_axis_()[3 * ja + 2]};
                        real t0[3];
                        mulmat(Rl, ax, t0);
                        for (int k = 0; k < 3; k++) pos[k] += t0[k] * q;
                    }
                    if (body_tree_()[p] < 0) {
                        GLB_PTR(const real) Rp = ka->m.static_xmat + 9 * p;
                        real Rn[9], t0[3];
                        for (int i = 0; i < 3; i++)
                            for (int j = 0; j < 3; j++) Rn[3 * i + j] = Rp[3 * i] * R[j] + Rp[3 * i + 1] * R[3 + j] + Rp[3 * i + 2] * R[6 + j];
                        mulmat(Rp, pos, t0);
                        for (int k = 0; k < 3; k++) pos[k] = ka->m.static_xpos[3 * p + k] + t0[k];
                        for (int k = 0; k < 9; k++) R[k] = Rn[k];
                    } else a = p;
                }
            }
            for (int k = 0; k < 3; k++) xpos[3 * b + k] = pos[k];
            for (int k = 0; k < 9; k++) xmat[9 * b + k] = R[k];
            anc[b] = a;
        }
        GSYNC();
        for (int round = 0; round < 6; round++) {
            bool any = false;
            real Ra[9], pa[3];
            int a = -1, aa = -1;
            const int b = lane;
            if (b < nb) {
                a = anc[b];
                if (a >= 0) {
                    any = true;
                    aa = anc[a];
                    for (int k = 0; k < 9; k++) Ra[k] = xmat[9 * a + k];
                    for (int k = 0; k < 3; k++) pa[k] = xpos[3 * a + k];
                }
            }
            if (!__any(any)) break;
            GSYNC();
            if (a >= 0) {
                real R[9], pos[3], Rn[9], t0[3];
                for (int k = 0; k < 9; k++) R[k] = xmat[9 * b + k];
                for (int k = 0; k < 3; k++) pos[k] = xpos[3 * b + k];
                for (int i = 0; i < 3; i++)
                    for (int j = 0; j < 3; j++) Rn[3 * i + j] = Ra[3 * i] * R[j] + Ra[3 * i + 1] * R[3 + j] + Ra[3 * i + 2] * R[6 + j];
                mulmat(Ra, pos, t0);
                for (int k = 0; k < 3; k++) xpos[3 * b + k] = pa[k] + t0[k];
                for (int k = 0; k < 9; k++) xmat[9 * b + k] = Rn[k];
                anc[b] = aa;
            }
            GSYNC();
        }
        for (int b = lane; b < nb; b += G) {
            real t3[3] = {0, 0, 0};
            if (body_tree_()[b] >= 0) {
                const real ip[3] = {body_ipos_()[3 * b], body_ipos_()[3 * b + 1], body_ipos_()[3 * b + 2]};
                mulmat(xmat + 9 * b, ip, t3);
                for (int k = 0; k < 3; k++) t3[k] += xpos[3 * b + k];
            }
            for (int k = 0; k < 3; k++) xipos[3 * b + k] = t3[k];
        }
        for (int d = lane; d < ka->m.nv; d += G) {
            const int j = dof_jnt_()[d], b = dof_body_()[d], jt = jnt_type_()[j], k = d - jnt_dofadr_()[j];
            const real *R = xmat + 9 * b, *pos = xpos + 3 * b;
            real cd[6] = {0, 0, 0, 0, 0, 0};
            if (jt == J_FREE) {
                if (k < 3) cd[3 + k] = 1;
// ... 163 lines not shown
                inert_mul(sv, v, Iv);
                cross_force(v, Iv, vIv);
                for (int q = 0; q < 6; q++) f[q] = Ia[q] + vIv[q];
            }
            for (int q = 0; q < 6; q++) cfrc[6 * b + q] = f[q];
        }
        GSYNC();
        for (int i = lane; i < ka->m.nv; i += G) {
            const int b = dof_body_()[i];
            real f[6] = {0, 0, 0, 0, 0, 0};
            for (int d = b; d <= body_last_()[b]; d++)
                for (int q = 0; q < 6; q++) f[q] += cfrc[6 * d + q];
            real sacc = 0;
            for (int q = 0; q < 6; q++) sacc += cdof[6 * i + q] * f[q];
            bias[i] = sacc;
        }
        GSYNC();
    }

    __device__ void smooth() {
        PHASE_BEGIN();
        real *qpos = r + ka->lay.qpos, *qvel = r + ka->lay.qvel, *ctrl = r + ka->lay.ctrl, *bias = r + ka->lay.bias, *fsm = r + ka->lay.fsm, *as = r + ka->lay.asm_;
        real* act = r + ka->lay.fcon;
        for (int i = lane; i < ka->m.nv; i += G) act[i] = 0;
        GSYNC();
        for (int u = lane; u < ka->m.nu; u += G) {
            real c = ctrl[u];
            if (act_ctrllimited_()[u]) c = tclamp(c, act_ctrlrange_()[2 * u], act_ctrlrange_()[2 * u + 1]);
            int dof = act_dof_()[u];
            real f = act_kp_()[u] * c - act_kp_()[u] * qpos[act_qposadr_()[u]] - act_kv_()[u] * qvel[dof];
            act[dof] += act_gear_()[u] * f;
        }
        GSYNC();
        for (int i = lane; i < ka->m.nv; i += G) {
            int j = dof_jnt_()[i];
            real a = act[i];
            if (jnt_actfrclimited_()[j] && jnt_type_()[j] != J_FREE) a = tclamp(a, jnt_actfrcrange_()[2 * j], jnt_actfrcrange_()[2 * j + 1]);
            real f = -dof_damping_()[i] * qvel[i] - bias[i] + a;
            fsm[i] = f;
            as[i] = f;
        }
        GSYNC();
        {
            const int t = lane >> 3, i = lane & 7;
            const bool mine = t < ka->m.ntree && i < tree_dofnum_()[t];
            const int k = mine ? tree_dofadr_()[t] + i : 0;
            const real x = tree_solve(r + ka->lay.L, mine ? as[k] : real(0));
            GSYNC();
            if (mine) as[k] = x;
        }
        GSYNC();
    }

    __device__ void load_shape(int g, Shape<real>& s) {
        LDS_BASES();
        real *xpos = r + ka->lay.xpos, *xmat = r + ka->lay.xmat, *gcen = r + ka->lay.gcen;
        s.type = geom_type_()[g];
        for (int k = 0; k < 3; k++) s.size[k] = ka->m.geom_size[3 * g + k];
        s.hull = ka->m.hull_vert;
        s.hbase = ka->m.geom_hull[2 * g];
        s.hR = ka->m.geom_hull[2 * g + 1];
        s.hovf = hull_ovf_();
        s.nh = 0;
        for (int k = 0; k < 3; k++) { s.lc[k] = ka->m.geom_lbox[6 * g + k]; s.lh[k] = ka->m.geom_lbox[6 * g + 3 + k]; }
        if (geom_static_()[g]) {
            for (int k = 0; k < 3; k++) { s.pos[k] = ka->m.geom_xpos0[3 * g + k]; s.center[k] = ka->m.geom_cen0[3 * g + k]; }
            for (int k = 0; k < 9; k++) s.mat[k] = ka->m.geom_xmat0[9 * g + k];
        } else {
            int b = geom_body_()[g];
            real gp[3] = {ka->m.geom_pos[3 * g], ka->m.geom_pos[3 * g + 1], ka->m.geom_pos[3 * g + 2]}, t3[3];
            mulmat(xmat + 9 * b, gp, t3);
            for (int k = 0; k < 3; k++) { s.pos[k] = xpos[3 * b + k] + t3[k]; s.center[k] = gcen[3 * g + k]; }
            const real* Rb = xmat + 9 * b;
            GLB_PTR(const real) Rg = ka->m.geom_mat + 9 * g;
            for (int i = 0; i < 3; i++)
                for (int j = 0; j < 3; j++) s.mat[3 * i + j] = Rb[3 * i] * Rg[j] + Rb[3 * i + 1] * Rg[3 + j] + Rb[3 * i + 2] * Rg[6 + j];
        }
    }

    __device__ AVS_OUTLINE_0 static void multi_perturb(KRef<real, SPEC> ka_, real* r_, int* i_, int lane_, int grp_, const real* lr_, const int* li_, int env_,
                                                                   int pga, int pgb, int src, int pert) {
        Env e(ka_, r_, i_, lane_, grp_, lr_, li_);
        e.env = env_;
        LDS_PTR(real) os = (LDS_PTR(real))(e.r + e.ka->lay.scr + SLOT_W * src);
        const real p0[3] = {os[SLOT_P], os[SLOT_P + 1], os[SLOT_P + 2]}, n0[3] = {os[SLOT_N], os[SLOT_N + 1], os[SLOT_N + 2]};
        Shape<real> a, b;
        e.load_shape(pga, a);
        e.load_shape(pgb, b);
        real dk = real(1e30), pk[3] = {0, 0, 0};
        if (!mpr_perturbed(a, b, p0, n0, pert, &dk, pk)) dk = real(1e30);
        os[1 + pert] = dk;
        for (int c = 0; c < 3; c++) os[SLOT_P + 3 * (1 + pert) + c] = pk[c];
    }

    __device__ AVS_OUTLINE void collide() {
        Env e(*this);
        e.collide_i();
        diverged = e.diverged; nit_sum = e.nit_sum; nit_max = e.nit_max; t_broad = e.t_broad; t_narrow = e.t_narrow;
    }
    __device__ __attribute__((always_inline)) void collide_i() {
        PHASE_BEGIN();
        real* gcen = r + ka->lay.gcen;
        int* misc = ii + ka->lay.misc;
        GLB_PTR(int) cand = cand_();
        int ncand = 0;
        long long tb0 = __builtin_readcyclecounter();
        const real skin = real(0.03);
        GLB_PTR(real) gref = gref_();
        GLB_PTR(int) nearl = near_();
        auto pair_hit = [&](int p, real pad) -> bool {
            int g1 = ka->m.pair_geom[2 * p], g2 = ka->m.pair_geom[2 * p + 1];
            bool s1 = geom_static_()[g1], s2 = geom_static_()[g2];
            real mg = ka->m.pair_margin[p] + pad;
            if (s1 || s2) {
                int gs = s1 ? g1 : g2, gd = s1 ? g2 : g1;
                real rd = geom_rbound_()[gd] + mg, d2 = 0;
                for (int k = 0; k < 3; k++) {
                    real c = gcen[3 * gd + k], lo = ka->m.geom_aabb0[6 * gs + k], hi = ka->m.geom_aabb0[6 * gs + 3 + k];
                    real e = c < lo ? lo - c : (c > hi ? c - hi : real(0));
                    d2 += e * e;
                }
                return !(d2 > rd * rd);
            }
            real d[3], rr = geom_rbound_()[g1] + geom_rbound_()[g2] + mg;
            sub3(gcen + 3 * g2, gcen + 3 * g1, d);
            return !(dot3(d, d) > rr * rr);
        };
        bool moved = false;
        if (misc[7]) {
            for (int g = lane; g < ka->m.ngeom; g += G)
                if (!geom_static_()[g]) {
                    const real d[3] = {gcen[3 * g] - gref[3 * g], gcen[3 * g + 1] - gref[3 * g + 1], gcen[3 * g + 2] - gref[3 * g + 2]};
                    moved |= dot3(d, d) > real(0.25) * skin * skin;
                }
        }
        bool rebuild = !misc[7] || __any(moved);
        int nnear = misc[6];
        if (rebuild) {
            nnear = 0;
#pragma unroll 1
            for (int base = 0; base < ka->m.npair; base += G) {
                int p = base + lane;
                bool hit = p < ka->m.npair && pair_hit(p, skin);
                int tot, rk = group_rank<G>(hit, grp, lane, &tot);
                if (hit && nnear + rk < NEAR_MAX) nearl[nnear + rk] = p;
                nnear += tot;
            }
            for (int i = lane; i < 3 * ka->m.ngeom; i += G) gref[i] = gcen[i];
            if (lane == 0) { misc[6] = nnear < NEAR_MAX ? nnear : NEAR_MAX; misc[7] = nnear <= NEAR_MAX; if (nnear > NEAR_MAX) misc[2] |= 8; }
            GSYNC();
        }
        if (nnear <= NEAR_MAX) {
            for (int base = 0; base < nnear; base += G) {
                int i = base + lane, p = i < nnear ? nearl[i] : 0;
                bool hit = i < nnear && pair_hit(p, real(0));
                int tot, rk = group_rank<G>(hit, grp, lane, &tot);
                if (hit && ncand + rk < CAND_MAX) cand[ncand + rk] = p;
                if (ncand + tot > CAND_MAX && lane == 0) misc[2] |= 4;
                ncand = ncand + tot < CAND_MAX ? ncand + tot : CAND_MAX;
            }
        } else {
#pragma unroll 1
            for (int base = 0; base < ka->m.npair; base += G) {
                int p = base + lane;
                bool hit = p < ka->m.npair && pair_hit(p, real(0));
                int tot, rk = group_rank<G>(hit, grp, lane, &tot);
                if (hit && ncand + rk < CAND_MAX) cand[ncand + rk] = p;
                if (ncand + tot > CAND_MAX && lane == 0) misc[2] |= 4;
                ncand = ncand + tot < CAND_MAX ? ncand + tot : CAND_MAX;
            }
        }
        if (lane == 0) misc[3] = ncand;
        GSYNC();
        long long tb1 = __builtin_readcyclecounter();
        t_broad += tb1 - tb0;
        real *cdist = r + ka->lay.cdist, *cpos = r + ka->lay.cpos, *cnrm = r + ka->lay.cnrm;
        int* cpair = ii + ka->lay.cpair;
        int ncon = 0, ovf = 0;
        int* mlist = ii + ka->lay.cand;
        GLB_PTR(real) bxo = bxo_();
        for (int base = 0; base < ncand; base += G) {
            const int ci = base + lane;
            int n = 0, p = 0, nn = 0;
            LDS_PTR(real) scr = (LDS_PTR(real))(r + ka->lay.scr + SLOT_W * lane);
            const bool valid = ci < ncand;
            if (valid) p = cand[ci];
            const int ga = ka->m.pair_geom[2 * p], gb = ka->m.pair_geom[2 * p + 1];
            const int tya = geom_type_()[ga], tyb = geom_type_()[gb];
            const bool isbox = valid && tya == G_BOX && tyb == G_BOX;
            const long long tn0_ = profiling ? __builtin_readcyclecounter() : 0;
            {
                bool boxlive = false;
                if (isbox) {
                    Shape<real> a, b;
                    load_shape(ga, a);
                    load_shape(gb, b);
                    boxlive = !boxes_separated(a, b);
                }
                int nbox, rk = group_rank<G>(boxlive, grp, lane, &nbox);
                const int row = lane >> 4;
                for (int b0 = 0; b0 < nbox; b0 += 4) {
                    int src = 0;
                    bool on = false;
#pragma unroll
                    for (int gg = 0; gg < 4; gg++) {
                        const unsigned long long mm = __ballot(boxlive && rk == b0 + gg);
                        if (row == gg && mm != 0) { src = __builtin_ctzll(mm); on = true; }
                    }
                    const int pga = __shfl(ga, src, 64), pgb = __shfl(gb, src, 64);
                    Shape<real> a, b;
                    load_shape(pga, a);
                    load_shape(pgb, b);
                    const int n16 = box_box16(a, b, (LDS_PTR(real))(r + ka->lay.scr + SLOT_W * src), (LDS_PTR(real))(r + ka->lay.scr + SLOT_W * G + 56 * row), bxo + BOX_OVF_W * src, lane, on);
                    __builtin_amdgcn_fence(__ATOMIC_ACQ_REL, "wavefront");
                    __builtin_amdgcn_wave_barrier();
                    const int got = __shfl(on ? n16 : 0, 16 * ((rk - b0) & 3), 64);
                    if (boxlive && rk >= b0 && rk < b0 + 4) nn = got;
                }
            }
            const long long tn1 = profiling ? __builtin_readcyclecounter() : 0;
            if (valid && !isbox) {
                Shape<real> a, b;
                load_shape(ga, a);
                load_shape(gb, b);
                nn = narrow(a, b, scr);
            }
            if (profiling) {
                const long long tn2 = __builtin_readcyclecounter();
                if (lane == 0) { (ii + ka->lay.nprof)[14] += (int)(tn1 - tn0_); (ii + ka->lay.nprof)[15] += (int)(tn2 - tn1); }
            }
            {
                const bool multi = valid && !isbox && nn == 1 && tya != G_SPHERE && tyb != G_SPHERE;
                int nm, mrk = group_rank<G>(multi, grp, lane, &nm);
                if (nm > 0) {
                    if (multi) mlist[mrk] = lane;
                    GSYNC();
                    for (int m0 = 0; m0 < nm; m0 += 16) {
                        const int q = m0 + (lane >> 2), pert = lane & 3;
                        const bool on = q < nm;
                        const int src = on ? mlist[q] : 0;
                        const int pga = __shfl(ga, src, 64), pgb = __shfl(gb, src, 64);
                        if (on) multi_perturb(ka, r, ii, lane, grp, lr, li, env, pga, pgb, src, pert);
                    }
                    GSYNC();
                    if (multi) {
                        const real rb1 = geom_rbound_()[ga], rb2 = geom_rbound_()[gb];
                        const real tol = MultiCcd<real>::reltol * (rb1 < rb2 ? rb1 : rb2);
                        int kept = 1;
                        for (int k = 1; k <= 4; k++) {
                            const real dk = scr[k];
                            const real pk[3] = {scr[SLOT_P + 3 * k], scr[SLOT_P + 3 * k + 1], scr[SLOT_P + 3 * k + 2]};
                            if (dk < real(1e29) && multiccd_distinct(pk, scr + SLOT_P, kept, tol)) {
                                scr[kept] = dk;
                                for (int c = 0; c < 3; c++) scr[SLOT_P + 3 * kept + c] = pk[c];
                                kept++;
                            }
                        }
                        nn = kept;
                    }
                }
            }
            int keepmask = 0;
            GLB_PTR(const real) ov = bxo + BOX_OVF_W * lane;
            if (valid) {
                real mg = ka->m.pair_margin[p];
                for (int k = 0; k < nn; k++)
                    if ((isbox && k >= BOX_SLOTC ? ov[4 * (k - BOX_SLOTC)] : scr[k]) < mg) { keepmask |= 1 << k; n++; }
            }
            int off = 0, tot = 0;
            for (int j = 1; j <= BOX_MAXC; j++) {
                int tj, rj = group_rank<G>(n >= j, grp, lane, &tj);
                if (tj == 0) break;
                off += rj;
                tot += tj;
            }
            int w = 0;
            for (int k = 0; k < BOX_MAXC; k++)
                if ((keepmask >> k) & 1) {
                    int c = ncon + off + w;
                    w++;
                    if (c < ka->lay.maxcon) {
                        const bool o = isbox && k >= BOX_SLOTC;
                        cdist[c] = o ? ov[4 * (k - BOX_SLOTC)] : scr[k];
                        cpair[c] = p;
                        for (int q = 0; q < 3; q++) { cpos[3 * c + q] = o ? ov[4 * (k - BOX_SLOTC) + 1 + q] : scr[SLOT_P + 3 * k + q]; cnrm[3 * c + q] = scr[SLOT_N + q]; }
                    }
                }
            if (ncon + tot > ka->lay.maxcon) ovf = 1;
            ncon = ncon + tot < ka->lay.maxcon ? ncon + tot : ka->lay.maxcon;
        }
        if (lane == 0) { misc[0] = ncon; misc[2] |= ovf; }
        GSYNC();
        t_narrow += __builtin_readcyclecounter() - tb1;
    }

#ifndef AVS_NO_SPLIT_PRE
    __device__ AVS_OUTLINE void pre_phases() {
        Env e(*this);
        e.kinematics(); e.crb(); e.rne_bias(); e.smooth();
    }
    __device__ AVS_OUTLINE void post_phases() {
        Env e(*this);
        e.euler(); e.check_divergence();
        diverged = e.diverged;
    }
#endif
    __device__ AVS_OUTLINE void make_constraints() {
        Env e(*this);
        e.make_constraints_i();
        diverged = e.diverged; nit_sum = e.nit_sum; nit_max = e.nit_max; t_broad = e.t_broad; t_narrow = e.t_narrow;
    }
    __device__ __attribute__((always_inline)) void make_constraints_i() {
        PHASE_BEGIN();
#ifdef AVSIM_PROBE_ROWS
        long long tpr_ = __builtin_readcyclecounter();
#define ROWPROBE(k) do { if (profiling) { const long long t_ = __builtin_readcyclecounter(); if (lane == 0) (ii + ka->lay.nprof)[8 + (k)] += (int)(t_ - tpr_); tpr_ = t_; } } while (0)
#else
#define ROWPROBE(k) ((void)0)
#endif
        real *qpos = r + ka->lay.qpos, *qvel = r + ka->lay.qvel;
        int *misc = ii + ka->lay.misc, *rmeta = ii + ka->lay.rmeta, *cpair = ii + ka->lay.cpair, *cefc = ii + ka->lay.cefc;
        real *cdist = r + ka->lay.cdist, *cpos = r + ka->lay.cpos, *cnrm = r + ka->lay.cnrm;
        int ncon = misc[0];
        int nefc = ka->m.neq + ka->m.nfloss;
        for (int i = lane; i < ka->m.neq; i += G) rmeta[i] = R_EQ | (i << 2);
        for (int i = lane; i < ka->m.nfloss; i += G) rmeta[ka->m.neq + i] = R_FLOSS | (i << 2);
        for (int base = 0; base < ka->m.nlimited; base += G) {
            int li = base + lane, lo = 0, hi = 0, j = 0;
            if (li < ka->m.nlimited) {
                j = limited_jnt_()[li];
                real q = qpos[jnt_qposadr_()[j]];
                lo = (q - jnt_range_()[2 * j]) < jnt_margin_()[j];
                hi = (jnt_range_()[2 * j + 1] - q) < jnt_margin_()[j];
            }
            int t1, t2, r1 = group_rank<G>(lo, grp, lane, &t1), r2 = group_rank<G>(hi, grp, lane, &t2);
            int pos = nefc + r1 + r2;
            if (lo && pos < ka->lay.maxefc) rmeta[pos] = R_LIMIT | (j << 2) | (0 << 12);
            if (hi && pos + lo < ka->lay.maxefc) rmeta[pos + lo] = R_LIMIT | (j << 2) | (1 << 12);
            nefc += t1 + t2;
        }
        int ovf = 0;
        if (nefc > ka->lay.maxefc) { nefc = ka->lay.maxefc; ovf = 1; }
        if (lane == 0) misc[4] = nefc;
        const int nlead0 = nefc;
        int cend = nefc;
        for (int base = 0; base < ncon; base += G) {
            int c = base + lane, dim = 0;
            if (c < ncon) {
                int p = cpair[c];
                if (cdist[c] < ka->m.pair_margin[p] - ka->m.pair_gap[p]) dim = ka->m.pair_condim[p];
            }
            int off = 0, tot = 0;
            for (int j = 1; j <= 6; j++) {
                int tj, rj = group_rank<G>(dim >= j, grp, lane, &tj);
                off += rj;
                tot += tj;
            }
            int myend = 0;
            if (c < ncon) {
                int first = nefc + off;
                if (dim > 0 && first + dim <= ka->lay.maxefc) {
                    cefc[c] = first | (dim << 16);
                    myend = first + dim;
                    for (int s = 0; s < dim; s++) rmeta[first + s] = R_CONTACT | (c << 2) | (s << 12) | (dim << 20);
                } else {
                    cefc[c] = -1;
                    if (dim > 0) ovf = 1;
                }
            }
            for (int o = 1; o < G; o <<= 1) { int x = __shfl_xor(myend, o, G); myend = x > myend ? x : myend; int y = __shfl_xor(ovf, o, G); ovf |= y; }
            cend = myend > cend ? myend : cend;
            nefc += tot;
        }
        nefc = cend;
        if (lane == 0) { misc[1] = nefc; if (ovf) misc[2] |= 2; }
        GSYNC();
        ROWPROBE(0);
        GLB_PTR(real) rJ = rows_();
        real *rowS = r + ka->lay.rowS, *warm = r + ka->lay.warm, *Minv = r + ka->lay.Minv, *asm_ = r + ka->lay.asm_;
        const bool newton = ka->m.solver == 1;
        const bool lead_slim = newton && lead_per_tree();
        int* rowI = ii + ka->lay.rowI;
        real* Lm = r + ka->lay.L;
        const int *bmask = body_dofmask_(), *tadr = tree_dofadr_(), *tnum = tree_dofnum_();
        const real* cdofp = r + ka->lay.cdof;
        const int nvm = ka->m.nv - 1;
        auto fill = [&](int i, auto lead_tag) {
            constexpr bool LEAD = decltype(lead_tag)::value;
            int meta = rmeta[i], type = meta & 3, id = (meta >> 2) & 1023, sub = (meta >> 12) & 255, dim = meta >> 20;
            real J[ROW_W];
#pragma unroll
            for (int k = 0; k < ROW_W; k++) J[k] = 0;
            int tA = -1, tB = -1;
            int j1 = -1, j2 = -1;
            real v1 = 0, v2 = 0;
            real pos = 0, margin = 0, diag0 = 0, floss = 0;
            real solref[2], solimp[5];
            bool valid = true;
            if (LEAD && type == R_EQ) {
                GLB_PTR(const real) c = ka->m.eq_polycoef + 5 * id;
                real q1 = qpos[ka->m.eq_qpos1[id]] - ka->m.qpos0[ka->m.eq_qpos1[id]], q2 = qpos[ka->m.eq_qpos2[id]] - ka->m.qpos0[ka->m.eq_qpos2[id]];
                real poly = c[0] + q2 * (c[1] + q2 * (c[2] + q2 * (c[3] + q2 * c[4])));
                real dpoly = c[1] + q2 * (2 * c[2] + q2 * (3 * c[3] + q2 * 4 * c[4]));
                int d1 = ka->m.eq_dof1[id], d2 = ka->m.eq_dof2[id];
                tA = dof_tree_()[d1];
                pos = q1 - poly;
                diag0 = dof_invweight0_()[d1] + dof_invweight0_()[d2];
                j1 = d1 - tree_dofadr_()[tA]; v1 = 1;
                j2 = d2 - tree_dofadr_()[tA]; v2 = -dpoly;
                for (int k = 0; k < 2; k++) solref[k] = ka->m.eq_solref[2 * id + k];
                for (int k = 0; k < 5; k++) solimp[k] = ka->m.eq_solimp[5 * id + k];
            } else if (LEAD && type == R_FLOSS) {
                int d = floss_dof_()[id];
                tA = dof_tree_()[d];
                diag0 = dof_invweight0_()[d];
                floss = dof_frictionloss_()[d];
                j1 = d - tree_dofadr_()[tA]; v1 = 1;
                for (int k = 0; k < 2; k++) solref[k] = ka->m.dof_solref[2 * d + k];
                for (int k = 0; k < 5; k++) solimp[k] = ka->m.dof_solimp[5 * d + k];
            } else if (LEAD && type == R_LIMIT) {
                int j = id, d = jnt_dofadr_()[j];
                real q = qpos[jnt_qposadr_()[j]];
                tA = dof_tree_()[d];
                pos = sub == 0 ? q - jnt_range_()[2 * j] : jnt_range_()[2 * j + 1] - q;
                margin = jnt_margin_()[j];
                diag0 = dof_invweight0_()[d];
                j1 = d - tree_dofadr_()[tA]; v1 = sub == 0 ? real(1) : real(-1);
                for (int k = 0; k < 2; k++) solref[k] = ka->m.jnt_solref[2 * j + k];
                for (int k = 0; k < 5; k++) solimp[k] = ka->m.jnt_solimp[5 * j + k];
            } else if (!LEAD) {
                int c = id, p = cpair[c];
                int g1 = ka->m.pair_geom[2 * p], g2 = ka->m.pair_geom[2 * p + 1], b1 = geom_body_()[g1], b2 = geom_body_()[g2];
                int t1 = body_tree_()[b1], t2 = body_tree_()[b2];
                tA = t1 >= 0 ? t1 : t2;
                tB = (t1 >= 0 && t2 >= 0 && t2 != t1) ? t2 : -1;
                real n[3] = {cnrm[3 * c], cnrm[3 * c + 1], cnrm[3 * c + 2]}, t1v[3], t2v[3], cp[3] = {cpos[3 * c], cpos[3 * c + 1], cpos[3 * c + 2]};
                make_frame(n, t1v, t2v);
                const int sm = sub % 3;
                real ax[3];
#pragma unroll
                for (int q = 0; q < 3; q++) ax[q] = sm == 0 ? n[q] : (sm == 1 ? t1v[q] : t2v[q]);
                const bool rot = sub >= 3;
                real cx[3], Wa[3], Wl[3];
                cross3(cp, ax, cx);
#pragma unroll
                for (int q = 0; q < 3; q++) { Wa[q] = rot ? ax[q] : cx[q]; Wl[q] = rot ? real(0) : ax[q]; }
                const int mA = (t1 == tA ? bmask[b1] : 0), pA = (t2 == tA ? bmask[b2] : 0);
                const int mB = (tB >= 0 && t1 == tB ? bmask[b1] : 0), pB = (tB >= 0 ? bmask[b2] : 0);
                const int aA = tadr[tA], aB = tadr[tB >= 0 ? tB : tA];
#pragma unroll
                for (int k = 0; k < TREE_W; k++) {
                    const real* ca = cdofp + 6 * (aA + k < nvm ? aA + k : nvm);
                    const real ea = Wa[0] * ca[0] + Wa[1] * ca[1] + Wa[2] * ca[2] + Wl[0] * ca[3] + Wl[1] * ca[4] + Wl[2] * ca[5];
                    J[k] = real(((pA >> k) & 1) - ((mA >> k) & 1)) * ea;
                }
                if (tB >= 0) {
#pragma unroll
                    for (int k = 0; k < TREE_W; k++) {
                        const real* cb = cdofp + 6 * (aB + k < nvm ? aB + k : nvm);
                        const real eb = Wa[0] * cb[0] + Wa[1] * cb[1] + Wa[2] * cb[2] + Wl[0] * cb[3] + Wl[1] * cb[4] + Wl[2] * cb[5];
                        J[TREE_W + k] = real(((pB >> k) & 1) - ((mB >> k) & 1)) * eb;
                    }
                }
                pos = sub == 0 ? cdist[c] : real(0);
                margin = ka->m.pair_margin[p] - ka->m.pair_gap[p];
                diag0 = body_invweight0_()[2 * b1] + body_invweight0_()[2 * b2];
                for (int k = 0; k < 2; k++) solref[k] = ka->m.pair_solref[2 * p + k];
                for (int k = 0; k < 5; k++) solimp[k] = ka->m.pair_solimp[5 * p + k];
            }
            (void)valid;
            const int j2c = j2 >= 0 ? j2 : (j1 >= 0 ? j1 : 0), j1c = j1 >= 0 ? j1 : 0;
            const real v2c = j2 >= 0 ? v2 : real(0);
            if (LEAD) {
#pragma unroll
                for (int k = 0; k < TREE_W; k++) J[k] += (k == j1 ? v1 : real(0)) + (k == j2 ? v2 : real(0));
            }
            real dmax = tclamp(solimp[1], real(0.0001), real(0.9999));
            real tc = tmax(solref[0], 2 * ka->m.timestep), dr = solref[1];
            real K = real(1) / tmax(real(1e-15), dmax * dmax * tc * tc * dr * dr), Bd = real(2) / tmax(real(1e-15), dmax * tc);
            real imp, R;
            const real imp_row = impedance(solimp, (!LEAD && sub > 0) ? cdist[id] : pos, margin);
            if (!LEAD && sub > 0) {
                int c = id, p = cpair[c];
                real imp0 = imp_row;
                real R0 = tmax(real(1e-15), (1 - imp0) * diag0 / imp0);
                real R1 = R0 / tmax(real(1e-15), ka->m.impratio);
                real mu0 = ka->m.pair_friction[5 * p], mur = ka->m.pair_friction[5 * p + sub - 1];
                R = sub == 1 ? R1 : R1 * mu0 * mu0 / tmax(real(1e-15), mur * mur);
                imp = imp0;
                K = 0;
                floss = mur;
            } else {
                imp = imp_row;
                R = tmax(real(1e-15), (1 - imp) * diag0 / imp);
            }
            real vel = 0;
            if (LEAD) {
                const int a0 = tadr[tA];
                vel = v1 * qvel[a0 + j1c] + v2c * qvel[a0 + j2c];
            } else {
                const int a0 = tadr[tA], b0 = tadr[tB >= 0 ? tB : tA];
#pragma unroll
                for (int k = 0; k < TREE_W; k++) vel += J[k] * qvel[a0 + k < nvm ? a0 + k : nvm];
                if (tB >= 0) {
#pragma unroll
                    for (int k = 0; k < TREE_W; k++) vel += J[TREE_W + k] * qvel[b0 + k < nvm ? b0 + k : nvm];
                }
            }
            const real aref = -Bd * vel - K * imp * (pos - margin);
            real dg = 0;
            real Bv[ROW_W];
            if (LEAD) {
                const real* Mi = Minv + 64 * tA;
                const real s1 = Mi[8 * j1c + j1c] * v1 + Mi[8 * j1c + j2c] * v2c, s2 = Mi[8 * j2c + j1c] * v1 + Mi[8 * j2c + j2c] * v2c;
                dg = v1 * s1 + v2c * s2;
                if (!lead_slim) {
#pragma unroll
                    for (int k = 0; k < TREE_W; k++) { Bv[k] = Mi[8 * k + j1c] * v1 + Mi[8 * k + j2c] * v2c; Bv[TREE_W + k] = 0; }
                }
            } else {
#pragma unroll
            for (int k = 0; k < TREE_W; k++) {
                real mr[TREE_W], sa = 0;
                lds_load8(Minv + 64 * tA + 8 * k, mr);
#pragma unroll
                for (int j = 0; j < TREE_W; j++) sa += mr[j] * J[j];
                dg += J[k] * sa;
                Bv[k] = sa;
                Bv[TREE_W + k] = 0;
            }
            if (tB >= 0) {
#pragma unroll
                for (int k = 0; k < TREE_W; k++) {
                    real mr[TREE_W], sb = 0;
                    lds_load8(Minv + 64 * tB + 8 * k, mr);
#pragma unroll
                    for (int j = 0; j < TREE_W; j++) sb += mr[j] * J[TREE_W + j];
                    dg += J[TREE_W + k] * sb;
                    Bv[TREE_W + k] = sb;
                }
// ... 4 lines not shown
#pragma unroll
                for (int k = 0; k < TREE_W; k++) { JB_[k] = J[k]; JB_[TREE_W + k] = Bv[k]; }
                store_row16(rJ + ROW_S * i, JB_);
            } else if (!LEAD || !lead_slim) {
                store_row16(rJ + ROW_S * i, J);
                store_row16(rowsB_() + ROW_S * i, Bv);
            }
            const int a0 = tadr[tA], nA = tnum[tA], b0 = tB >= 0 ? tadr[tB] : 0, nB = tB >= 0 ? tnum[tB] : 0;
            real jw = 0, jas = 0;
            if (LEAD) {
                jw = v1 * warm[a0 + j1c] + v2c * warm[a0 + j2c];
                jas = v1 * asm_[a0 + j1c] + v2c * asm_[a0 + j2c];
            } else {
#pragma unroll
            for (int k = 0; k < TREE_W; k++) {
                const int da = a0 + k < nvm ? a0 + k : nvm;
                jw += J[k] * warm[da];
                jas += J[k] * asm_[da];
            }
            if (tB >= 0) {
#pragma unroll
                for (int k = 0; k < TREE_W; k++) {
                    const int db = b0 + k < nvm ? b0 + k : nvm;
                    jw += J[TREE_W + k] * warm[db];
                    jas += J[TREE_W + k] * asm_[db];
                }
            }
            }
            const real big = real(1e30);
            real lo = -big, hi = big, muinv = 0;
            bool ns = false;
            if (LEAD && type == R_FLOSS) { lo = -floss; hi = floss; ns = true; }
            else if (LEAD && type == R_LIMIT) lo = 0;
            else if (!LEAD) {
                if (sub == 0) lo = 0;
                else { ns = true; muinv = real(1) / tmax(real(1e-15), floss); }
            }
            real f = -(jw - aref) / R;
            f = tmin(tmax(f, lo), hi);
            real* S = rowS + RS_S * i;
            S[0] = aref; S[1] = R; S[2] = newton ? jw - aref : real(1) / (dg + R); S[3] = ns ? real(1) / tmax(dg, real(1e-15)) : real(0);
            S[4] = lo; S[5] = hi; S[6] = f; S[7] = muinv; S[8] = jas - aref;
            const int lead_bits = !LEAD ? 0 : ((v1 < 0 ? 1 : 0) << 13) | (j1c << 26) | (j2c << 29);
            if (LEAD) S[7] = v2c;
            rowI[i] = a0 | (nA << 6) | (tA << 10) | ((b0 | (nB << 6) | ((tB >= 0 ? tB : 0) << 10)) << 13) | lead_bits;
            rmeta[i] = (meta & 0xfffff) | ((tA + 1) << 20) | ((tB + 1) << 24);
        };
        for (int i = lane; i < nlead0; i += G) fill(i, BoolTag<true>{});
        ROWPROBE(1);
        for (int i = nlead0 + lane; i < nefc; i += G) fill(i, BoolTag<false>{});
        GSYNC();
        ROWPROBE(2);
        int* gI = ii + ka->lay.gI;
        GLB_PTR(real) gA = coup_();
        const int nlead = misc[4];
        int ngrp = 0;
        for (int base = 0; base < nefc; base += G) {
            int i = base + lane;
            bool head = false;
            int cnt = 0, isc = 0;
            if (i < nefc) {
                if (i < nlead) { head = (i % GRP_MAX) == 0; cnt = nlead - i < GRP_MAX ? nlead - i : GRP_MAX; }
                else { int meta = rmeta[i]; head = ((meta >> 12) & 255) == 0; cnt = ka->m.pair_condim[cpair[(meta >> 2) & 1023]]; isc = 1; }
            }
            int tot, rk = group_rank<G>(head, grp, lane, &tot);
            if (head && ngrp + rk < ka->lay.maxgrp) gI[ngrp + rk] = i | (cnt << 16) | (isc << 24);
            ngrp += tot;
        }
        if (ngrp > ka->lay.maxgrp) ngrp = ka->lay.maxgrp;
        if (lane == 0) misc[5] = ngrp;
        GSYNC();
        ROWPROBE(3);
        const int nlg = (nlead + GRP_MAX - 1) / GRP_MAX;
        const int per_c = newton ? 10 : 15, nl15 = lead_slim ? 0 : nlg * 15, nitem = ngrp <= nlg ? (lead_slim ? 0 : ngrp * 15) : nl15 + (ngrp - nlg) * per_c;
        for (int w = lane; w < nitem; w += G) {
            int g, e, rr = 1, ss;
            if (w < nl15 || !newton) {
                g = w / 15; e = w - 15 * g;
                while ((rr + 1) * rr / 2 <= e) rr++;
                ss = e - rr * (rr - 1) / 2;
            } else {
                const int wc = w - nl15, e2 = wc % 10;
                g = nlg + wc / 10;
                while ((rr + 1) * rr / 2 <= e2) rr++;
                ss = e2 - rr * (rr - 1) / 2 + 1;
                rr += 1;
                e = rr * (rr - 1) / 2 + ss;
                if (e2 < 5) gA[GA_W * g + (e2 + 1) * e2 / 2] = 0;
            }
            int gi = gI[g], start = gi & 0xffff, cnt = (gi >> 16) & 15;
            real v = 0;
            if (rr < cnt) {
                int ir = start + rr, is = start + ss, ra = rowI[ir], rs = rowI[is];
                GLB_PTR(const real) Jr = rJ + ROW_S * ir;
                const bool packed_s = g >= nlg && ((rs >> 19) & 15) == 0;
                GLB_PTR(const real) Bs = packed_s ? (GLB_PTR(const real))(rJ + ROW_S * is + TREE_W) : (GLB_PTR(const real))(rowsB_() + ROW_S * is);
#pragma unroll
                for (int wr = 0; wr < 2; wr++) {
                    const bool on_r = ((ra >> (13 * wr + 6)) & 15) != 0;
                    const int tr = (ra >> (13 * wr + 10)) & 7;
#pragma unroll
                    for (int ws = 0; ws < 2; ws++) {
                        const bool match = on_r && ((rs >> (13 * ws + 6)) & 15) != 0 && ((rs >> (13 * ws + 10)) & 7) == tr;
                        real t = 0;
#pragma unroll
                        for (int k = 0; k < TREE_W; k++) t += Jr[TREE_W * wr + k] * Bs[TREE_W * ws + k];
                        v += match ? t : real(0);
                    }
                }
            }
            gA[GA_W * g + e] = v;
        }
        GSYNC();
        ROWPROBE(4);
        if (ka->m.noslip_iters > 0)
        for (int g = nlg + lane; g < ngrp; g += G) {
            const int gi = gI[g], start = gi & 0xffff, n = ((gi >> 16) & 15) - 1;
            if (n < 3) continue;
            real A[5][5], As[5][5], L[5][5], Inv[5][5], mu[5];
#pragma unroll
            for (int j = 0; j < 5; j++) {
                const bool in = j < n;
                const real* S = rowS + RS_S * (start + 1 + (in ? j : 0));
                mu[j] = in ? real(1) / S[7] : real(1);
                A[j][j] = in ? real(1) / S[3] : real(1);
#pragma unroll
                for (int k = 0; k < j; k++) { const real c = in ? gA[GA_W * g + (j + 1) * j / 2 + (k + 1)] : real(0); A[j][k] = c; A[k][j] = c; }
            }
#pragma unroll
            for (int i = 0; i < 5; i++)
#pragma unroll
                for (int j = 0; j < 5; j++) As[i][j] = (i < n && j < n) ? A[i][j] * mu[i] * mu[j] : (i == j ? real(1) : real(0));
            bool singular = false;
#pragma unroll
            for (int j = 0; j < 5; j++) {
                real dd = As[j][j];
#pragma unroll
                for (int k = 0; k < j; k++) dd -= L[j][k] * L[j][k];
                if (j < n && dd < real(1e-10)) singular = true;
                dd = sqrt(tmax(dd, real(1e-30)));
                L[j][j] = dd;
#pragma unroll
                for (int i = j + 1; i < 5; i++) {
                    real t = As[i][j];
#pragma unroll
                    for (int k = 0; k < j; k++) t -= L[i][k] * L[j][k];
                    L[i][j] = t / dd;
                }
            }
#pragma unroll
            for (int c = 0; c < 5; c++) {
                real x[5];
#pragma unroll
                for (int i = 0; i < 5; i++) { real t = (i == c) ? real(1) : real(0); for (int k = 0; k < i; k++) t -= L[i][k] * x[k]; x[i] = t / L[i][i]; }
#pragma unroll
                for (int i = 4; i >= 0; i--) { real t = x[i]; for (int k = i + 1; k < 5; k++) t -= L[k][i] * x[k]; x[i] = t / L[i][i]; }
#pragma unroll
                for (int i = 0; i < 5; i++) Inv[i][c] = x[i];
            }
#pragma unroll
            for (int j = 0; j < 5; j++) {
                GLB_PTR(real) o = gA + GA_W * g + GA_Q + j;
#pragma unroll
                for (int k = 0; k < 5; k++) o[8 * k] = mu[j] * Inv[j][k] * mu[k];
                o[40] = singular ? real(1) : real(0);
            }
        }
        GSYNC();
        ROWPROBE(5);
    }

    __device__ AVS_OUTLINE void solve(int pgs_iters, int solver, int newton_iters, real newton_tol, real scale) {
        Env e(*this);
        e.solve_i(pgs_iters, solver, newton_iters, newton_tol, scale);
        diverged = e.diverged; nit_sum = e.nit_sum; nit_max = e.nit_max; t_broad = e.t_broad; t_narrow = e.t_narrow;
    }
    __device__ __attribute__((always_inline)) void solve_i(int pgs_iters, int solver, int newton_iters, real newton_tol, real scale) {
        PHASE_BEGIN();
        if constexpr (spec_fixed<SPEC>) { solver = ka->m.solver; newton_iters = ka->m.newton_iters; }
        int *misc = ii + ka->lay.misc, *rmeta = ii + ka->lay.rmeta, *cefc = ii + ka->lay.cefc, *rowI = ii + ka->lay.rowI;
        real *qacc = r + ka->lay.qacc, *as = r + ka->lay.asm_, *rowS = r + ka->lay.rowS, *fcon = r + ka->lay.fcon;
        GLB_PTR(real) rJ = rows_();
        int nefc = misc[1], ncon = misc[0];
        real* Minv = r + ka->lay.Minv;
        if (solver == 1) {
            real* warm = r + ka->lay.warm;
            for (int k = lane; k < ka->m.nv; k += G) qacc[k] = warm[k];
            GSYNC();
            bool two_ = false;
            for (int i = lane; i < nefc; i += G) two_ = two_ || ((rowI[i] >> 19) & 15) != 0;
            const bool coupled = __any(two_) != 0 || ka->m.ntree > 8;
#define AVS_NEWTON_ARGS ka, (GLB_PTR(const real))rJ, (LDS_PTR(real))r, (LDS_PTR(int))ii, (LDS_PTR(const int))LI(), nefc, ncon, misc[4], newton_iters, newton_tol, scale, profiling ? 1 : 0
            int used = __builtin_amdgcn_readfirstlane(ncon) <= 64 ? (coupled ? newton_solve_coupled<real, 1>(AVS_NEWTON_ARGS) : newton_solve<real, 1, false>(AVS_NEWTON_ARGS))
                                                                  : (coupled ? newton_solve_coupled<real, 2>(AVS_NEWTON_ARGS) : newton_solve<real, 2, false>(AVS_NEWTON_ARGS));
#undef AVS_NEWTON_ARGS
            nit_sum += used; nit_max = used > nit_max ? used : nit_max;
            GSYNC();
            long long tn0 = profiling ? __builtin_readcyclecounter() : 0;
            int done_ = 0;
            if (ka->m.noslip_trees && lead_per_tree() && __builtin_amdgcn_readfirstlane(misc[8]) == 0)
                done_ = noslip_trees<real>((LDS_PTR(real))rowS, (LDS_PTR(const int))rowI, (LDS_PTR(const int))cefc, (GLB_PTR(const real))rJ, (LDS_PTR(real))qacc,
                                           (LDS_PTR(const int))(ii + ka->lay.gI), (GLB_PTR(const real))coup_(), ncon, nefc, ka->m.noslip_iters, real(1e-6) / ka->m.nscale, NL_ARGS(noslip_lead()));
            if (__builtin_amdgcn_readfirstlane(done_) == 2)
                done_ = noslip_trees2<real>((LDS_PTR(real))rowS, (LDS_PTR(const int))rowI, (LDS_PTR(const int))cefc, (GLB_PTR(const real))rJ, (GLB_PTR(const real))rowsB_(), (LDS_PTR(real))qacc,
                                            (LDS_PTR(const int))(ii + ka->lay.gI), (GLB_PTR(const real))coup_(), ncon, nefc, ka->m.noslip_iters, real(1e-6) / ka->m.nscale, NL_ARGS(noslip_lead()));
            if (__builtin_amdgcn_readfirstlane(done_) != 1 && lane == 0) misc[8] = 1;
            if (__builtin_amdgcn_readfirstlane(done_) != 1)
            pgs_groups<real>((LDS_PTR(real))rowS, (LDS_PTR(const int))rowI, (GLB_PTR(const real))rJ, (GLB_PTR(const real))rowsB_(), (LDS_PTR(real))qacc,
                             (LDS_PTR(const int))(ii + ka->lay.gI), (GLB_PTR(const real))coup_(), misc[5], 0, ka->m.noslip_iters, real(1e-6) / ka->m.nscale, NL_ARGS(noslip_lead()));
            if (profiling && lane == 0) (ii + ka->lay.nprof)[6] += (int)(__builtin_readcyclecounter() - tn0);
        } else {
        for (int c = lane; c < ncon; c += G) {
            int first = cefc[c];
            if (first < 0) continue;
            first &= 0xffff;
            int dim = ka->m.pair_condim[(ii + ka->lay.cpair)[c]];
            real fn = rowS[RS_S * first + 6], s2 = 0;
            for (int s = 1; s < dim; s++) { real t = rowS[RS_S * (first + s) + 6] * rowS[RS_S * (first + s) + 7]; s2 += t * t; }
            if (s2 > fn * fn) { real sc = fn / sqrt(s2); for (int s = 1; s < dim; s++) rowS[RS_S * (first + s) + 6] *= sc; }
        }
        GSYNC();
        jt_force(fcon, nefc);
        for (int k = lane; k < ka->m.nv; k += G) {
            int t = dof_tree_()[k], a0 = tree_dofadr_()[t], kk = k - a0, n = tree_dofnum_()[t];
            real s = as[k];
            for (int j = 0; j < n; j++) s += Minv[64 * t + 8 * kk + j] * fcon[a0 + j];
            qacc[k] = s;
        }
        GSYNC();
        static_assert(G == 64, "the solver maps one env to one wavefront");
        pgs_groups<real>((LDS_PTR(real))rowS, (LDS_PTR(const int))rowI, (GLB_PTR(const real))rJ, (GLB_PTR(const real))rowsB_(), (LDS_PTR(real))qacc,
                         (LDS_PTR(const int))(ii + ka->lay.gI), (GLB_PTR(const real))coup_(), misc[5], pgs_iters, ka->m.noslip_iters, real(1e-6) / ka->m.nscale, NL_ARGS(noslip_lead()));
        }
        GSYNC();
        jt_force(fcon, nefc);
    }

    AVS_DEV bool lead_per_tree() const { return ka->m.ntree <= 8 && ka->m.noslip_iters > 0 && ka->m.noslip_per_tree != 0; }
    AVS_DEV NoslipLead<real> noslip_lead() const {
        NoslipLead<real> nl;
        nl.Minv = (LDS_PTR(const real))(r + ka->lay.Minv);
        nl.tadr = (LDS_PTR(const int))tree_dofadr_(); nl.tnum = (LDS_PTR(const int))tree_dofnum_(); nl.floss_dof = (LDS_PTR(const int))floss_dof_();
        nl.dmap = (LDS_PTR(int))(r + ka->lay.ng);
        nl.ntree = ka->m.ntree; nl.nv = ka->m.nv; nl.neq = ka->m.neq; nl.nfloss = ka->m.nfloss; nl.tridiag = ka->m.qcqp_tridiag;
        nl.prof = profiling ? (LDS_PTR(int))(ii + ka->lay.nprof + 8) : (LDS_PTR(int))nullptr;
        nl.nlg = lead_per_tree() ? ((ii + ka->lay.misc)[4] + GRP_MAX - 1) / GRP_MAX : -1;
        return nl;
    }

    __device__ void check_divergence() {
        LDS_BASES();
        real *qpos = r + ka->lay.qpos, *qvel = r + ka->lay.qvel, *warm = r + ka->lay.warm;
        bool bad = false;
        for (int i = lane; i < ka->m.nq; i += G) bad |= !(fabs(qpos[i]) < real(1e6));
        for (int i = lane; i < ka->m.nv; i += G) bad |= !(fabs(qvel[i]) < real(1e6));
        if (!__any(bad)) return;
        diverged = 1;
        for (int i = lane; i < ka->m.nq; i += G) qpos[i] = ka->m.qpos_home[i];
        GSYNC();
        for (int i = lane; i < nobj_() * 7; i += G) qpos[ka->m.obj_qadr[i / 7] + i % 7] = (real)ka->m.obj_reset[((size_t)env * nobj_()) * 7 + i];
        for (int i = lane; i < ka->m.nv; i += G) { qvel[i] = 0; warm[i] = 0; }
        if (lane == 0) (ii + ka->lay.misc)[7] = 0;
        GSYNC();
    }

    __device__ __attribute__((always_inline)) void jt_force(real* out, int nefc) {
        LDS_BASES();
        AVS_ASSUME_LDS(out);
        (void)nefc;
        int* misc = ii + ka->lay.misc;
        for (int k = lane; k < ka->m.nv; k += G) out[k] = 0;
        GSYNC();
        rows_jt_force<real>((LDS_PTR(const real))(r + ka->lay.rowS), (LDS_PTR(const int))(ii + ka->lay.rowI), (LDS_PTR(const int))(ii + ka->lay.cefc),
                            (GLB_PTR(const real))rows_(), (LDS_PTR(real))out, misc[4], misc[0], lane, real(1));
        GSYNC();
    }

    __device__ void euler() {
        PHASE_BEGIN();
        real *qpos = r + ka->lay.qpos, *qvel = r + ka->lay.qvel, *warm = r + ka->lay.warm, *qacc = r + ka->lay.qacc, *fsm = r + ka->lay.fsm, *fcon = r + ka->lay.fcon;
        real *M = r + ka->lay.M, *L = r + ka->lay.L, *tmp = r + ka->lay.bias;
        real h = ka->m.timestep;
        for (int i = lane; i < ka->m.nv; i += G) { tmp[i] = fsm[i] + fcon[i]; warm[i] = qacc[i]; }
        GSYNC();
        tree_chol(M, L, dof_damping_(), h);
        GSYNC();
        {
            const int t = lane >> 3, i = lane & 7;
            const bool mine = t < ka->m.ntree && i < tree_dofnum_()[t];
            const int k = mine ? tree_dofadr_()[t] + i : 0;
            const real x = tree_solve(L, mine ? tmp[k] : real(0));
            if (mine) qvel[k] += h * x;
        }
        GSYNC();
        for (int j = lane; j < ka->m.njnt; j += G) {
            int qa = jnt_qposadr_()[j], da = jnt_dofadr_()[j];
            if (jnt_type_()[j] == J_FREE) {
                for (int k = 0; k < 3; k++) qpos[qa + k] += h * qvel[da + k];
                real q[4] = {qpos[qa + 3], qpos[qa + 4], qpos[qa + 5], qpos[qa + 6]}, w[3] = {qvel[da + 3], qvel[da + 4], qvel[da + 5]};
                real wn = sqrt(dot3(w, w)), ang = h * wn;
                if (ang > 0) {
                    real s = sin(ang / 2) / wn, qr[4] = {cos(ang / 2), s * w[0], s * w[1], s * w[2]};
                    quatmul(q, qr, q);
                }
                quatnorm(q);
                for (int k = 0; k < 4; k++) qpos[qa + 3 + k] = q[k];
            } else {
                qpos[qa] += h * qvel[da];
            }
        }
        GSYNC();
    }

    __device__ int reward(int* latch) {
        PHASE_BEGIN();
        int *misc = ii + ka->lay.misc, *cpair = ii + ka->lay.cpair;
        int ncon = misc[0];
        int f = 0;
        const int t = ka->m.task_id;
        for (int c = lane; c < ncon; c += G) {
            int p = cpair[c];
            f |= reward_pair_flags(ka->m.geom_class[ka->m.pair_geom[2 * p]], ka->m.geom_class[ka->m.pair_geom[2 * p + 1]], t);
        }
        for (int o = 1; o < G; o <<= 1) f |= __shfl_xor(f, o, G);
        return reward_from_flags(f, t, latch);
    }
};
// ... 449 lines not shown
                }
                std::vector<double> pts;
                if (gtype[g] == G_MESH) {
                    for (int v = 0; v < ghull[2 * g + 1]; v++) for (int k = 0; k < 3; k++) pts.push_back(hv[3 * (ghull[2 * g] + v) + k]);
                } else {
                    double ex[3] = {gsize[3 * g], gsize[3 * g + 1], gsize[3 * g + 2]};
                    if (gtype[g] == G_SPHERE) ex[1] = ex[2] = ex[0];
                    if (gtype[g] == G_CYLINDER) { ex[2] = ex[1]; ex[1] = ex[0]; }
                    for (int c = 0; c < 8; c++) for (int k = 0; k < 3; k++) pts.push_back(((c >> k) & 1) ? ex[k] : -ex[k]);
                }
                for (int k = 0; k < 3; k++) { gaabb[6 * g + k] = 1e30; gaabb[6 * g + 3 + k] = -1e30; }
                for (size_t v = 0; v < pts.size() / 3; v++)
                    for (int i = 0; i < 3; i++) {
                        double w = gx0[3 * g + i] + gm0[9 * g + 3 * i] * pts[3 * v] + gm0[9 * g + 3 * i + 1] * pts[3 * v + 1] + gm0[9 * g + 3 * i + 2] * pts[3 * v + 2];
                        if (w < gaabb[6 * g + i]) gaabb[6 * g + i] = w;
                        if (w > gaabb[6 * g + 3 + i]) gaabb[6 * g + 3 + i] = w;
                    }
            }
        }
        m.geom_type = up(I("geom_type")); moff.geom_type = (int)img_int.size(); { auto v_ = I("geom_type"); img_int.insert(img_int.end(), v_.begin(), v_.end()); } m.geom_body = up(gbody); moff.geom_body = (int)img_int.size(); { auto v_ = gbody; img_int.insert(img_int.end(), v_.begin(), v_.end()); } m.geom_hull = up(I("geom_ctab")); m.geom_class = up(I("geom_class")); m.geom_static = up(gstat); moff.geom_static = (int)img_int.size(); { auto v_ = gstat; img_int.insert(img_int.end(), v_.begin(), v_.end()); }
        m.geom_pos = upr<real>(gpos); m.geom_mat = upr<real>(gmat); m.geom_size = upr<real>(F("geom_size")); m.geom_cpos = upr<real>(gcp); moff.geom_cpos = (int)img_real.size(); { auto v_ = gcp; img_real.insert(img_real.end(), v_.begin(), v_.end()); }
        m.geom_rbound = upr<real>(F("geom_rbound")); moff.geom_rbound = (int)img_real.size(); { auto v_ = F("geom_rbound"); img_real.insert(img_real.end(), v_.begin(), v_.end()); } m.geom_xpos0 = upr<real>(gx0); m.geom_xmat0 = upr<real>(gm0); m.geom_cen0 = upr<real>(gc0); m.geom_aabb0 = upr<real>(gaabb); m.geom_lbox = upr<real>(glbox);
        {
            auto ctab = I("geom_ctab"), cells = I("chull_cells"), cand = I("chull_cand");
            const size_t ncell = cells.size();
            std::vector<double> tab(32 * ncell, 0.0), ovf;
            std::vector<char> done(ncell, 0);
            for (int g = 0; g < ng; g++) {
                if (gtype[g] != G_MESH) continue;
                const int cb = ctab[2 * g], R = ctab[2 * g + 1], adr = ghull[2 * g];
                for (int c = 0; c < 6 * R * R; c++) {
                    if (done[cb + c]) continue;
                    done[cb + c] = 1;
                    const int rec = cells[cb + c], off = rec >> 8, cnt = rec & 255;
                    if (cnt < 1) throw std::runtime_error("support table: empty cell");
                    double* o = &tab[32 * (size_t)(cb + c)];
                    for (int k = 0; k < 8; k++) {
                        const int v = cand[off + (k < cnt ? k : cnt - 1)];
                        if (v < 0 || v >= ghull[2 * g + 1]) throw std::runtime_error("support table: candidate index outside its hull");
                        for (int q = 0; q < 3; q++) o[4 * k + q] = hv[3 * (size_t)(adr + v) + q];
                        o[4 * k + 3] = (double)v;
                    }
                    o[3] = (double)cnt;
                    o[7] = (double)(ovf.size() / 4);
                    for (int k = 8; k < cnt; k++) {
                        const int v = cand[off + k];
                        if (v < 0 || v >= ghull[2 * g + 1]) throw std::runtime_error("support table: candidate index outside its hull");
                        for (int q = 0; q < 3; q++) ovf.push_back(hv[3 * (size_t)(adr + v) + q]);
                        ovf.push_back((double)v);
                    }
                }
            }
            if (ovf.size() / 4 >= (1u << 24)) throw std::runtime_error("support table: overflow part too large");
            m.hull_ovf = (int)(tab.size() / 4);
            tab.insert(tab.end(), ovf.begin(), ovf.end());
            if (tab.empty()) tab.assign(4, 0.0);
            m.hull_vert = upr<real>(tab);
        }
        m.pair_geom = up(I("pair_geom")); m.pair_condim = up(I("pair_condim"));
        m.pair_friction = upr<real>(F("pair_friction")); m.pair_solref = upr<real>(F("pair_solref")); m.pair_solimp = upr<real>(F("pair_solimp"));
        m.pair_margin = upr<real>(F("pair_margin")); m.pair_gap = upr<real>(F("pair_gap"));
        m.obs_qposadr = up(I("obs_qposadr")); m.obs_offset = upr<real>(F("obs_offset")); m.obs_scale = upr<real>(F("obs_scale"));
        while (img_real.size() % 4) img_real.push_back(0.0);
        while (img_int.size() % 4) img_int.push_back(0);
        moff.nreal = (int)img_real.size();
        moff.nint = (int)img_int.size();
        d_img_real = (void*)upr<real>(img_real);
        d_img_int = up(img_int);
    }

    const void* spec_kernel(const char** name) const {
        if (f64 || specialised == 0 || two_pass()) return nullptr;
        return phys_spec_kernel(*this, name);
    }
    bool refuses(std::string& err) const {
        if (specialised != 2 || spec_kernel(nullptr)) return false;
        err = std::string("phys_specialised = 2: no kernel compiled for this handle's model and layout (") +
              (f64 ? "f64 handle" : two_pass() ? "two capacity tiers" : "Layout, table offsets, dims or solver options (solver, noslip_*, qcqp_tridiag, newton_*, ls_iterations, num_joints) match no spec of avsim_phys_specs.h") + "); the launch would take the generic k_phys";
        return true;
    }
    int spec_note = 0;

    void make_layout(int nq, int nv, int nu, int nb, int ng, int msize, int ntree) {
        if (maxcon1 > maxcon) maxcon1 = maxcon;
        if (maxefc1 > maxefc) maxefc1 = maxefc;
        make_layout_of(lay, maxcon1, maxefc1, nq, nv, nu, nb, ng, msize, ntree);
        make_layout_of(lay2, maxcon, maxefc, nq, nv, nu, nb, ng, msize, ntree);
    }
    void make_layout_of(Layout& L, const int maxcon, const int maxefc, int nq, int nv, int nu, int nb, int ng, int msize, int ntree) {
        kargs_dirty = true;
        L = avs::make_layout_of(maxcon, maxefc, this->maxcon, this->maxefc, nq, nv, nu, nb, ng, msize, ntree, f64 ? 8 : 4);
        if (getenv("AVSIM_DEBUG_LAYOUT")) {
            const int pb = L.rowS + RS_S * maxefc > L.scr + NARROW_SCR_W ? L.rowS + RS_S * maxefc : L.scr + NARROW_SCR_W;
            fprintf(stderr, "avsim layout: %d reals + %d ints = %d B per env (U at %d: phase A %d, phase B %d words); tables %zu B\n", L.nreal, L.nint,
                    L.bytes_per_env, L.U, 38 * nb, pb - L.U, (size_t)moff.nreal * (f64 ? 8 : 4) + (size_t)moff.nint * 4);
        }
    }

    int dims[7] = {0, 0, 0, 0, 0, 0, 0};
    size_t lds_bytes() const { return (size_t)lay.bytes_per_env + (size_t)moff.nreal * (f64 ? 8 : 4) + (size_t)moff.nint * 4; }
    DevBuf rows, coup, near, gref;
    void alloc_contacts() {
        if (host_only) return;
        if (rows.alloc((size_t)N * maxefc * ROW_S * (f64 ? 8 : 4) * 2) != hipSuccess) throw std::runtime_error("hipMalloc of the constraint row buffers failed");
        mf.rJ_glob = rows.as<float>(); md.rJ_glob = rows.as<double>();
        mf.rB_glob = mf.rJ_glob + (size_t)N * maxefc * ROW_S; md.rB_glob = md.rJ_glob + (size_t)N * maxefc * ROW_S;
// ... 209 lines not shown
```

Baseline: 1.044 million.

## Address global tables via uniform base plus 32-bit offsets and inline collision helpers

Adds a GArr wrapper that keeps a global base pointer, made wave-uniform through readfirstlane, plus a 32-bit unsigned byte offset. Model tables, Jacobian rows and hull support tables are read through it across physics, collision and Newton code. The goal is scalar-base plus VGPR-offset addressing in place of 64-bit per-lane address arithmetic, which saves VALU work and registers. It also forces inlining of mpr_penetration, box_box16 and narrow and launders a phase in the coupled Newton solve, and it adds a host check that the support table stays under 4 GiB, the limit of the 32-bit offsets.

Result: faster. 1.055 million (median of 6 runs) (+1.1%).

```diff
diff --git a/av_aloha_amd/build.py b/av_aloha_amd/build.py
--- a/av_aloha_amd/build.py
+++ b/av_aloha_amd/build.py
@@ -6,6 +6,12 @@
 ROOT = os.path.dirname(HERE)
 LIB = os.path.join(HERE, "libavsim.so")
 SRC = os.path.join(HERE, "csrc")
+
+
+COMMON_FLAGS = ["--offload-arch=gfx950", "-std=c++17", "-fPIC", "-fno-gpu-rdc"]
+F32_FLAGS = ["-O2", "-fno-hip-fp32-correctly-rounded-divide-sqrt", "-fgpu-flush-denormals-to-zero", "-fno-slp-vectorize", "-fno-vectorize",
+             "-mllvm", "-amdgpu-atomic-optimizer-strategy=None", "-mllvm", "-amdgpu-sched-strategy=max-ilp"]
+F64_FLAGS = ["-O3", "-ffp-contract=off", "-mllvm", "-amdgpu-sched-strategy=max-ilp"]
 
 
 def _stale(target, sources):
@@ -29,13 +35,11 @@
 
 def _build_hip_locked(verbose):
     hipcc = os.environ.get("HIPCC", "/opt/rocm/bin/hipcc")
-    common = [hipcc, "--offload-arch=gfx950", "-std=c++17", "-fPIC", "-fno-gpu-rdc", "-c"]
-    F32_FLAGS = ["-O2", "-fno-hip-fp32-correctly-rounded-divide-sqrt", "-fgpu-flush-denormals-to-zero", "-fno-slp-vectorize", "-fno-vectorize",
-                 "-mllvm", "-amdgpu-atomic-optimizer-strategy=None", "-mllvm", "-amdgpu-sched-strategy=max-ilp"]
+    common = [hipcc] + COMMON_FLAGS + ["-c"]
     units = [
         ("avsim_api", F32_FLAGS + (["-DAVSIM_RENDER_STATS"] if os.environ.get("AVSIM_RENDER_STATS") else []) + os.environ.get("AVSIM_EXTRA_FLAGS", "").split()),
         ("avsim_phys_spec", F32_FLAGS + os.environ.get("AVSIM_EXTRA_FLAGS", "").split()),
-        ("avsim_phys_f64", ["-O3", "-ffp-contract=off", "-mllvm", "-amdgpu-sched-strategy=max-ilp"] + os.environ.get("AVSIM_EXTRA_FLAGS_F64", "").split()),
+        ("avsim_phys_f64", F64_FLAGS + os.environ.get("AVSIM_EXTRA_FLAGS_F64", "").split()),
         ("avsim_imgaug", ["-O3", "-ffp-contract=off", "-fhip-fp32-correctly-rounded-divide-sqrt", "-fno-gpu-flush-denormals-to-zero"] + os.environ.get("AVSIM_EXTRA_FLAGS_IMGAUG", "").split()),
         ("avsim_chunks", ["-O3", "-ffp-contract=off", "-fhip-fp32-correctly-rounded-divide-sqrt", "-fno-gpu-flush-denormals-to-zero"] + os.environ.get("AVSIM_EXTRA_FLAGS_CHUNKS", "").split()),
         ("avsim_obshist", ["-O3", "-ffp-contract=off", "-fhip-fp32-correctly-rounded-divide-sqrt", "-fno-gpu-flush-denormals-to-zero"] + os.environ.get("AVSIM_EXTRA_FLAGS_OBSHIST", "").split()),
diff --git a/av_aloha_amd/csrc/avsim_collide.hip.h b/av_aloha_amd/csrc/avsim_collide.hip.h
--- a/av_aloha_amd/csrc/avsim_collide.hip.h
+++ b/av_aloha_amd/csrc/avsim_collide.hip.h
@@ -57,7 +57,8 @@
             int iu = (int)((u + T(1)) * T(0.5) * T(R)), iv = (int)((v + T(1)) * T(0.5) * T(R));
             iu = iu > 0 ? (iu < R - 1 ? iu : R - 1) : 0;
             iv = iv > 0 ? (iv < R - 1 ? iv : R - 1) : 0;
-            GLB_PTR(const T) C = s.hull + 32 * (size_t)(s.hbase + ((2 * a + (lm < T(0) ? 1 : 0)) * R + iu) * R + iv);
+            const GArr<const T> H(glb_uniform(s.hull));
+            const GArr<const T> C = H + 32 * (s.hbase + ((2 * a + (lm < T(0) ? 1 : 0)) * R + iu) * R + iv);
             const T tie = TieTol<T>::rel * T(0.1) * (ax + ay + az);
             T vx[8], vy[8], vz[8], pr[8], w0, w1;
 #pragma unroll
@@ -69,7 +70,7 @@
             T bd = T(-1e30);
 #pragma unroll
             for (int k = 0; k < 8; k++) { pr[k] = vx[k] * l[0] + vy[k] * l[1] + vz[k] * l[2]; bd = pr[k] > bd ? pr[k] : bd; }
-            GLB_PTR(const T) O = s.hull + 4 * ((size_t)s.hovf + (size_t)(cnt > 8 ? (int)w1 : 0));
+            const GArr<const T> O = H + 4 * (s.hovf + (cnt > 8 ? (int)w1 : 0));
             const int more = cnt - 8, lastm = more - 1;
             for (int i = 0; i < more; i += 8) {
 #pragma unroll
@@ -153,7 +154,7 @@
 template <> struct MprTol<float> { static constexpr float tol = 1e-6f, tiny2 = 1e-16f, eps = 1e-9f; };
 
 template <typename T>
-__device__ int mpr_penetration(const Shape<T>& A, const Shape<T>& B, T* depth, T* dir, T* pos) {
+__device__ __attribute__((always_inline)) int mpr_penetration(const Shape<T>& A, const Shape<T>& B, T* depth, T* dir, T* pos) {
     const T tol = MprTol<T>::tol;
     const int maxit = 50;
     MPt<T> v0, v1, v2, v3, v4;
@@ -540,8 +541,8 @@
             for (int c = 0; c < 3; c++) scr[SLOT_P + 3 * x + c] = wv[c] + rpos[c];
             scr[x] = -dq_;
         } else {
-            ovf[4 * (x - BOX_SLOTC)] = -dq_;
-            for (int c = 0; c < 3; c++) ovf[4 * (x - BOX_SLOTC) + 1 + c] = wv[c] + rpos[c];
+            (ovf + 4 * (x - BOX_SLOTC))[0] = -dq_;
+            for (int c = 0; c < 3; c++) (ovf + 4 * (x - BOX_SLOTC))[1 + c] = wv[c] + rpos[c];
         }
     }
     for (int c = 0; c < 3; c++) scr[SLOT_N + c] = n[c];
@@ -552,7 +553,7 @@
 template <typename T> AVS_DEV T row_get(T x, int g16, int l) { return __shfl(x, g16 | l, 64); }
 
 template <typename T, typename OVF>
-__device__ int box_box16(const Shape<T>& a, const Shape<T>& b, AVS_LDS(T) scr, AVS_LDS(T) work, OVF ovf, int lane, bool on) {
+__device__ __attribute__((always_inline)) int box_box16(const Shape<T>& a, const Shape<T>& b, AVS_LDS(T) scr, AVS_LDS(T) work, OVF ovf, int lane, bool on) {
     const int t = lane & 15, g16 = lane & ~15;
     const unsigned rowmask_sh = g16;
     const T *Ra = a.mat, *Rb = b.mat;
@@ -745,8 +746,8 @@
             for (int c = 0; c < 3; c++) scr[SLOT_P + 3 * t + c] = wv[c] + rpos[c];
             scr[t] = -dq_;
         } else {
-            ovf[4 * (t - BOX_SLOTC)] = -dq_;
-            for (int c = 0; c < 3; c++) ovf[4 * (t - BOX_SLOTC) + 1 + c] = wv[c] + rpos[c];
+            (ovf + 4 * (t - BOX_SLOTC))[0] = -dq_;
+            for (int c = 0; c < 3; c++) (ovf + 4 * (t - BOX_SLOTC))[1 + c] = wv[c] + rpos[c];
         }
     }
     if (on && t == 0) { for (int c = 0; c < 3; c++) scr[SLOT_N + c] = n[c]; }
@@ -775,7 +776,7 @@
 }
 
 template <typename T>
-__device__ int narrow(const Shape<T>& a, const Shape<T>& b, AVS_LDS(T) scr) {
+__device__ __attribute__((always_inline)) int narrow(const Shape<T>& a, const Shape<T>& b, AVS_LDS(T) scr) {
     int ta = a.type, tb = b.type;
     if (boxes_separated(a, b)) return 0;
     T dist[1], pos[3], nrm[3];
diff --git a/av_aloha_amd/csrc/avsim_math.hip.h b/av_aloha_amd/csrc/avsim_math.hip.h
--- a/av_aloha_amd/csrc/avsim_math.hip.h
+++ b/av_aloha_amd/csrc/avsim_math.hip.h
@@ -1,5 +1,8 @@
 #pragma once
 #include <hip/hip_runtime.h>
+
+#include <type_traits>
+#include <utility>
 
 namespace avs {
 
@@ -43,6 +46,40 @@
 #define GLB_PTR(T) __attribute__((address_space(1))) T*
 #endif
 
+#if defined(__HIPCC__)
+AVS_DEV int wave_first(int x) { return __builtin_amdgcn_readfirstlane(x); }
+#else
+AVS_DEV int wave_first(int x) { return x; }
+#endif
+template <typename T>
+struct GArr {
+    typedef GLB_PTR(char) BP;
+    typedef decltype(*std::declval<GLB_PTR(T)>()) Ref;
+    GLB_PTR(T) b;
+    unsigned ob;
+    AVS_DEV GArr() : b(nullptr), ob(0u) {}
+    AVS_DEV explicit GArr(GLB_PTR(T) b_, unsigned ob_ = 0u) : b(b_), ob(ob_) {}
+    template <typename U, typename = typename std::enable_if<std::is_same<const U, T>::value>::type>
+    AVS_DEV GArr(const GArr<U>& a) : b((GLB_PTR(T))a.b), ob(a.ob) {}
+    AVS_DEV GArr operator+(int i) const { return GArr(b, ob + (unsigned)i * (unsigned)sizeof(T)); }
+    AVS_DEV GArr operator+(unsigned i) const { return GArr(b, ob + i * (unsigned)sizeof(T)); }
+    AVS_DEV Ref operator[](int i) const {
+        if (__builtin_constant_p(i)) return *(GLB_PTR(T))((BP)b + (unsigned long long)ob + (long long)i * (long long)sizeof(T));
+        return *(GLB_PTR(T))((BP)b + (unsigned long long)(ob + (unsigned)i * (unsigned)sizeof(T)));
+    }
+    AVS_DEV Ref operator*() const { return (*this)[0]; }
+    AVS_DEV explicit operator GLB_PTR(const T)() const { return (GLB_PTR(const T))((GLB_PTR(const char))b + (unsigned long long)ob); }
+    template <typename U> AVS_DEV GArr<U> as() const { return GArr<U>((GLB_PTR(U))b, ob); }
+};
+template <typename T> AVS_DEV GLB_PTR(T) glb_uniform(GLB_PTR(T) p) {
+    const unsigned long long v = (unsigned long long)p;
+    return (GLB_PTR(T))(((unsigned long long)(unsigned)wave_first((int)(unsigned)(v >> 32)) << 32) | (unsigned)wave_first((int)(unsigned)v));
+}
+template <typename T> AVS_DEV GArr<T> glb_block(GLB_PTR(T) base, int blk, unsigned stride) {
+    const unsigned long long off = (unsigned long long)(unsigned)wave_first(blk) * (unsigned long long)stride;
+    return GArr<T>(base + off);
+}
+
 template <typename T> AVS_DEV T dot3(const T* a, const T* b) { return a[0] * b[0] + a[1] * b[1] + a[2] * b[2]; }
 template <typename T> AVS_DEV void cross3(const T* a, const T* b, T* c) {
     T t0 = a[1] * b[2] - a[2] * b[1], t1 = a[2] * b[0] - a[0] * b[2], t2 = a[0] * b[1] - a[1] * b[0];
@@ -54,12 +91,12 @@
     if (n > T(0)) { T i = T(1) / n; a[0] *= i; a[1] *= i; a[2] *= i; }
     return n;
 }
-template <typename T, typename M> AVS_DEV void mulmat(const M* R, const T* v, T* o) {
+template <typename T, typename M> AVS_DEV void mulmat(M R, const T* v, T* o) {
     T t0 = (T)R[0] * v[0] + (T)R[1] * v[1] + (T)R[2] * v[2], t1 = (T)R[3] * v[0] + (T)R[4] * v[1] + (T)R[5] * v[2],
       t2 = (T)R[6] * v[0] + (T)R[7] * v[1] + (T)R[8] * v[2];
     o[0] = t0; o[1] = t1; o[2] = t2;
 }
-template <typename T, typename M> AVS_DEV void mulmatT(const M* R, const T* v, T* o) {
+template <typename T, typename M> AVS_DEV void mulmatT(M R, const T* v, T* o) {
     T t0 = (T)R[0] * v[0] + (T)R[3] * v[1] + (T)R[6] * v[2], t1 = (T)R[1] * v[0] + (T)R[4] * v[1] + (T)R[7] * v[2],
       t2 = (T)R[2] * v[0] + (T)R[5] * v[1] + (T)R[8] * v[2];
     o[0] = t0; o[1] = t1; o[2] = t2;
diff --git a/av_aloha_amd/csrc/avsim_newton.hip.h b/av_aloha_amd/csrc/avsim_newton.hip.h
--- a/av_aloha_amd/csrc/avsim_newton.hip.h
+++ b/av_aloha_amd/csrc/avsim_newton.hip.h
@@ -5,15 +5,15 @@
 
 typedef float nv4f __attribute__((ext_vector_type(4)));
 typedef double nv2d __attribute__((ext_vector_type(2)));
-AVS_DEV void load_row16(GLB_PTR(const float) src, float* v) {
-    GLB_PTR(const nv4f) p = (GLB_PTR(const nv4f))src;
+AVS_DEV void load_row16(GArr<const float> src, float* v) {
+    const GArr<const nv4f> p = src.as<const nv4f>();
     nv4f a = p[0], b = p[1], c = p[2], d = p[3];
     asm volatile("" : "+v"(a), "+v"(b), "+v"(c), "+v"(d));
     v[0] = a.x; v[1] = a.y; v[2] = a.z; v[3] = a.w; v[4] = b.x; v[5] = b.y; v[6] = b.z; v[7] = b.w;
     v[8] = c.x; v[9] = c.y; v[10] = c.z; v[11] = c.w; v[12] = d.x; v[13] = d.y; v[14] = d.z; v[15] = d.w;
 }
-AVS_DEV void load_row16(GLB_PTR(const double) src, double* v) {
-    GLB_PTR(const nv2d) p = (GLB_PTR(const nv2d))src;
+AVS_DEV void load_row16(GArr<const double> src, double* v) {
+    const GArr<const nv2d> p = src.as<const nv2d>();
     nv2d t[8];
 #pragma unroll
     for (int q = 0; q < 8; q++) t[q] = p[q];
@@ -27,7 +27,7 @@
     LDS_PTR(real) rowS;
     LDS_PTR(const int) rowI;
     LDS_PTR(const int) rmeta;
-    GLB_PTR(const real) rJ;
+    GArr<const real> rJ;
     LDS_PTR(const real) M;
     LDS_PTR(real) a;
     LDS_PTR(const real) as;
@@ -55,7 +55,7 @@
 AVS_DEV real nrow_dot(const NewtonArgs<real>& A, int i, LDS_PTR(const real) v) {
     const int ra = A.rowI[i];
     const int a0 = ra & 63, nA = (ra >> 6) & 15, b0 = (ra >> 13) & 63, nB = (ra >> 19) & 15;
-    GLB_PTR(const real) J = A.rJ + ROW_S * i;
+    const GArr<const real> J = A.rJ + ROW_S * i;
     real s = 0;
 #pragma unroll
     for (int k = 0; k < TREE_W; k++) {
@@ -183,7 +183,7 @@
 template <typename real> AVS_DEV real lead_v1(int ra) { return ((ra >> 13) & 1) ? real(-1) : real(1); }
 
 template <typename real>
-AVS_DEV void rows_jt_force(LDS_PTR(const real) rowS, LDS_PTR(const int) rowI, LDS_PTR(const int) cefc, GLB_PTR(const real) rJ, LDS_PTR(real) out,
+AVS_DEV void rows_jt_force(LDS_PTR(const real) rowS, LDS_PTR(const int) rowI, LDS_PTR(const int) cefc, GArr<const real> rJ, LDS_PTR(real) out,
                            int nlead, int ncon, int lane, real sgn) {
     for (int i = lane; i < nlead; i += 64) {
         const real f = rowS[RS_S * i + 6];
@@ -215,7 +215,7 @@
 template <typename real>
 AVS_DEV void nblock4_load(const NewtonArgs<real>& A, int lane, int r0, int dim, bool on, real* Jraw) {
     const int t = lane & 15;
-    GLB_PTR(const real) J = A.rJ + ROW_S * (on ? r0 : 0);
+    const GArr<const real> J = A.rJ + ROW_S * (on ? r0 : 0);
 #pragma unroll
     for (int p = 0; p < 6; p++) Jraw[p] = J[ROW_S * (p < dim ? p : 0) + t];
 }
@@ -231,11 +231,11 @@
     if (!__any(full)) {
         if (!two) {
             const int tc = lane & 7, s0 = (lane & 8) >> 1, gqc = on ? nslot_dof(ra, tc) : -1;
-            GLB_PTR(const real) J = A.rJ + ROW_S * (on ? r0 : 0);
+            const GArr<const real> J = A.rJ + ROW_S * (on ? r0 : 0);
             real Jc[6], Js[4][6];
 #pragma unroll
             for (int p = 0; p < 6; p++) {
-                GLB_PTR(const real) Jp = J + ROW_S * (p < dim ? p : 0);
+                const GArr<const real> Jp = J + ROW_S * (p < dim ? p : 0);
                 Jc[p] = Jp[tc];
 #pragma unroll
                 for (int u = 0; u < 4; u++) Js[u][p] = Jp[s0 + u];
@@ -608,10 +608,7 @@
         LDS_PTR(const int) li = (LDS_PTR(const int))(unsigned long long)(unsigned)__builtin_amdgcn_readfirstlane((int)(unsigned)(unsigned long long)li_);
         tol = lane_get(tol, 0); scale = lane_get(scale, 0);
         A.rowS = r + ka->lay.rowS; A.rowI = ii + ka->lay.rowI; A.rmeta = ii + ka->lay.rmeta;
-        {
-            const unsigned long long p_ = (unsigned long long)rows;
-            A.rJ = (GLB_PTR(const real))(((unsigned long long)(unsigned)__builtin_amdgcn_readfirstlane((int)(unsigned)(p_ >> 32)) << 32) | (unsigned)__builtin_amdgcn_readfirstlane((int)(unsigned)p_));
-        }
+        A.rJ = GArr<const real>(glb_uniform(rows));
         A.M = r + ka->lay.M; A.a = r + ka->lay.qacc; A.as = r + ka->lay.asm_;
         A.H = r + ka->lay.nH; A.g = r + ka->lay.ng; A.dl = r + ka->lay.ndl; A.jv = r + ka->lay.njv;
         A.cefc = ii + ka->lay.cefc;
@@ -915,6 +912,7 @@
 template <typename real, int NCH, typename KA>
 __device__ AVS_OUTLINE_5 int newton_solve_coupled(KA ka, GLB_PTR(const real) rows, LDS_PTR(real) r_, LDS_PTR(int) ii_, LDS_PTR(const int) li_, int nefc, int ncon, int nlead,
                                                               int iters, real tol, real scale, int profiling) {
+    PHASE_LAUNDER();
     return newton_solve<real, NCH, true>(ka, rows, r_, ii_, li_, nefc, ncon, nlead, iters, tol, scale, profiling);
 }
 
diff --git a/av_aloha_amd/csrc/avsim_phys.hip.h b/av_aloha_amd/csrc/avsim_phys.hip.h
--- a/av_aloha_amd/csrc/avsim_phys.hip.h
+++ b/av_aloha_amd/csrc/avsim_phys.hip.h
@@ -348,10 +348,9 @@
 template <typename T> AVS_DEV LDS_PTR(T) uni_lds(LDS_PTR(T) p) {
     return (LDS_PTR(T))(unsigned long long)(unsigned)__builtin_amdgcn_readfirstlane((int)(unsigned)(unsigned long long)p);
 }
-template <typename T> AVS_DEV GLB_PTR(T) uni_glb(GLB_PTR(T) p) {
-    const unsigned long long v = (unsigned long long)p;
-    return (GLB_PTR(T))(((unsigned long long)(unsigned)__builtin_amdgcn_readfirstlane((int)(unsigned)(v >> 32)) << 32) | (unsigned)__builtin_amdgcn_readfirstlane((int)(unsigned)v));
-}
+template <typename T> AVS_DEV GLB_PTR(T) uni_glb(GLB_PTR(T) p) { return glb_uniform(p); }
+template <typename T> AVS_DEV GArr<T> garr(GLB_PTR(T) p) { return GArr<T>(p); }
+#define TAB(name) garr(ka->m.name)
 
 template <typename T> AVS_DEV T secular_step(T val, T r2, T r, T yw) {
     const T yy = val + r2, ny = sqrt(yy);
@@ -1410,13 +1409,13 @@
 
 typedef float avs_v4f __attribute__((ext_vector_type(4)));
 typedef double avs_v2d __attribute__((ext_vector_type(2)));
-AVS_DEV void store_row16(GLB_PTR(float) dst, const float* v) {
-#pragma unroll
-    for (int q = 0; q < 4; q++) { avs_v4f t = {v[4 * q], v[4 * q + 1], v[4 * q + 2], v[4 * q + 3]}; ((GLB_PTR(avs_v4f))dst)[q] = t; }
-}
-AVS_DEV void store_row16(GLB_PTR(double) dst, const double* v) {
-#pragma unroll
-    for (int q = 0; q < 8; q++) { avs_v2d t = {v[2 * q], v[2 * q + 1]}; ((GLB_PTR(avs_v2d))dst)[q] = t; }
+AVS_DEV void store_row16(GArr<float> dst, const float* v) {
+#pragma unroll
+    for (int q = 0; q < 4; q++) { avs_v4f t = {v[4 * q], v[4 * q + 1], v[4 * q + 2], v[4 * q + 3]}; dst.as<avs_v4f>()[q] = t; }
+}
+AVS_DEV void store_row16(GArr<double> dst, const double* v) {
+#pragma unroll
+    for (int q = 0; q < 8; q++) { avs_v2d t = {v[2 * q], v[2 * q + 1]}; dst.as<avs_v2d>()[q] = t; }
 }
 
 AVS_DEV void lds_load8(const float* p, float* v) {
@@ -1451,7 +1450,7 @@
 template <typename real, typename KA>
 AVS_DEV void body_inertia(KA ka, const real* xmat, const real* xipos, int b, SInert<real>& s) {
     const real* R = xmat + 9 * b;
-    GLB_PTR(const real) Ib = ka->m.body_inertia + 6 * b;
+    const GArr<const real> Ib = TAB(body_inertia) + 6 * b;
     real I3[9] = {Ib[0], Ib[3], Ib[4], Ib[3], Ib[1], Ib[5], Ib[4], Ib[5], Ib[2]}, T[9], Ic[9];
 #pragma unroll
     for (int i = 0; i < 3; i++)
@@ -1461,7 +1460,7 @@
     for (int i = 0; i < 3; i++)
 #pragma unroll
         for (int j = 0; j < 3; j++) Ic[3 * i + j] = T[3 * i] * R[3 * j] + T[3 * i + 1] * R[3 * j + 1] + T[3 * i + 2] * R[3 * j + 2];
-    real ms = ka->m.body_mass[b];
+    real ms = TAB(body_mass)[b];
     real c[3] = {xipos[3 * b], xipos[3 * b + 1], xipos[3 * b + 2]};
     real cc = dot3(c, c);
     s.m = ms;
@@ -1645,13 +1644,13 @@
     }
     AVS_DEV int nobj_() const { if constexpr (spec_fixed<SPEC>) return SPEC::nobj; else return ka->m.nobj; }
     AVS_DEV int hull_ovf_() const { if constexpr (spec_fixed<SPEC>) return SPEC::hull_ovf; else return ka->m.hull_ovf; }
-    AVS_DEV GLB_PTR(real) rows_() const { return (GLB_PTR(real))ka->m.rJ_glob + (size_t)env * ka->lay.gefc * ROW_S; }
-    AVS_DEV GLB_PTR(real) rowsB_() const { return (GLB_PTR(real))ka->m.rB_glob + (size_t)env * ka->lay.gefc * ROW_S; }
-    AVS_DEV GLB_PTR(real) coup_() const { return (GLB_PTR(real))ka->m.gA_glob + (size_t)env * ka->lay.ggrp * GA_W; }
-    AVS_DEV GLB_PTR(int) near_() const { return (GLB_PTR(int))ka->m.near_glob + (size_t)env * NEAR_MAX; }
-    AVS_DEV GLB_PTR(int) cand_() const { return (GLB_PTR(int))ka->m.cand_glob + (size_t)env * CAND_MAX; }
-    AVS_DEV GLB_PTR(real) bxo_() const { return (GLB_PTR(real))ka->m.bxo_glob + (size_t)env * 64 * BOX_OVF_W; }
-    AVS_DEV GLB_PTR(real) gref_() const { return (GLB_PTR(real))ka->m.gref_glob + (size_t)env * ka->m.ngeom * 3; }
+    AVS_DEV GArr<real> rows_() const { return glb_block((GLB_PTR(real))ka->m.rJ_glob, env, (unsigned)(ka->lay.gefc * ROW_S)); }
+    AVS_DEV GArr<real> rowsB_() const { return glb_block((GLB_PTR(real))ka->m.rB_glob, env, (unsigned)(ka->lay.gefc * ROW_S)); }
+    AVS_DEV GArr<real> coup_() const { return glb_block((GLB_PTR(real))ka->m.gA_glob, env, (unsigned)(ka->lay.ggrp * GA_W)); }
+    AVS_DEV GArr<int> near_() const { return glb_block((GLB_PTR(int))ka->m.near_glob, env, (unsigned)NEAR_MAX); }
+    AVS_DEV GArr<int> cand_() const { return glb_block((GLB_PTR(int))ka->m.cand_glob, env, (unsigned)CAND_MAX); }
+    AVS_DEV GArr<real> bxo_() const { return glb_block((GLB_PTR(real))ka->m.bxo_glob, env, (unsigned)(64 * BOX_OVF_W)); }
+    AVS_DEV GArr<real> gref_() const { return glb_block((GLB_PTR(real))ka->m.gref_glob, env, (unsigned)(ka->m.ngeom * 3)); }
     AVS_DEV const int* body_parent_() const { return LI() + ka->mo.body_parent; }
     AVS_DEV const int* body_jntadr_() const { return LI() + ka->mo.body_jntadr; }
     AVS_DEV const int* body_jntnum_() const { return LI() + ka->mo.body_jntnum; }
@@ -1765,8 +1764,8 @@
             real R[9], pos[3];
             int a = -1;
             if (body_tree_()[b] < 0) {
-                for (int k = 0; k < 3; k++) pos[k] = ka->m.static_xpos[3 * b + k];
-                for (int k = 0; k < 9; k++) R[k] = ka->m.static_xmat[9 * b + k];
+                for (int k = 0; k < 3; k++) pos[k] = (TAB(static_xpos) + 3 * b)[k];
+                for (int k = 0; k < 9; k++) R[k] = (TAB(static_xmat) + 9 * b)[k];
             } else {
                 const int p = body_parent_()[b], ja = body_jntadr_()[b], jn = body_jntnum_()[b];
                 const int jt = jn > 0 ? jnt_type_()[ja] : -1;
@@ -1804,12 +1803,12 @@
                         for (int k = 0; k < 3; k++) pos[k] += t0[k] * q;
                     }
                     if (body_tree_()[p] < 0) {
-                        GLB_PTR(const real) Rp = ka->m.static_xmat + 9 * p;
+                        const GArr<const real> Rp = TAB(static_xmat) + 9 * p;
                         real Rn[9], t0[3];
                         for (int i = 0; i < 3; i++)
                             for (int j = 0; j < 3; j++) Rn[3 * i + j] = Rp[3 * i] * R[j] + Rp[3 * i + 1] * R[3 + j] + Rp[3 * i + 2] * R[6 + j];
                         mulmat(Rp, pos, t0);
-                        for (int k = 0; k < 3; k++) pos[k] = ka->m.static_xpos[3 * p + k] + t0[k];
+                        for (int k = 0; k < 3; k++) pos[k] = (TAB(static_xpos) + 3 * p)[k] + t0[k];
                         for (int k = 0; k < 9; k++) R[k] = Rn[k];
                     } else a = p;
                 }
@@ -2079,27 +2078,27 @@
         GSYNC();
     }
 
-    __device__ void load_shape(int g, Shape<real>& s) {
+    __device__ __attribute__((always_inline)) void load_shape(int g, Shape<real>& s) {
         LDS_BASES();
         real *xpos = r + ka->lay.xpos, *xmat = r + ka->lay.xmat, *gcen = r + ka->lay.gcen;
         s.type = geom_type_()[g];
-        for (int k = 0; k < 3; k++) s.size[k] = ka->m.geom_size[3 * g + k];
+        for (int k = 0; k < 3; k++) s.size[k] = (TAB(geom_size) + 3 * g)[k];
         s.hull = ka->m.hull_vert;
-        s.hbase = ka->m.geom_hull[2 * g];
-        s.hR = ka->m.geom_hull[2 * g + 1];
+        s.hbase = (TAB(geom_hull) + 2 * g)[0];
+        s.hR = (TAB(geom_hull) + 2 * g)[1];
         s.hovf = hull_ovf_();
         s.nh = 0;
-        for (int k = 0; k < 3; k++) { s.lc[k] = ka->m.geom_lbox[6 * g + k]; s.lh[k] = ka->m.geom_lbox[6 * g + 3 + k]; }
+        for (int k = 0; k < 3; k++) { s.lc[k] = (TAB(geom_lbox) + 6 * g)[k]; s.lh[k] = (TAB(geom_lbox) + 6 * g)[3 + k]; }
         if (geom_static_()[g]) {
-            for (int k = 0; k < 3; k++) { s.pos[k] = ka->m.geom_xpos0[3 * g + k]; s.center[k] = ka->m.geom_cen0[3 * g + k]; }
-            for (int k = 0; k < 9; k++) s.mat[k] = ka->m.geom_xmat0[9 * g + k];
+            for (int k = 0; k < 3; k++) { s.pos[k] = (TAB(geom_xpos0) + 3 * g)[k]; s.center[k] = (TAB(geom_cen0) + 3 * g)[k]; }
+            for (int k = 0; k < 9; k++) s.mat[k] = (TAB(geom_xmat0) + 9 * g)[k];
         } else {
             int b = geom_body_()[g];
-            real gp[3] = {ka->m.geom_pos[3 * g], ka->m.geom_pos[3 * g + 1], ka->m.geom_pos[3 * g + 2]}, t3[3];
+            real gp[3] = {(TAB(geom_pos) + 3 * g)[0], (TAB(geom_pos) + 3 * g)[1], (TAB(geom_pos) + 3 * g)[2]}, t3[3];
             mulmat(xmat + 9 * b, gp, t3);
             for (int k = 0; k < 3; k++) { s.pos[k] = xpos[3 * b + k] + t3[k]; s.center[k] = gcen[3 * g + k]; }
             const real* Rb = xmat + 9 * b;
-            GLB_PTR(const real) Rg = ka->m.geom_mat + 9 * g;
+            const GArr<const real> Rg = TAB(geom_mat) + 9 * g;
             for (int i = 0; i < 3; i++)
                 for (int j = 0; j < 3; j++) s.mat[3 * i + j] = Rb[3 * i] * Rg[j] + Rb[3 * i + 1] * Rg[3 + j] + Rb[3 * i + 2] * Rg[6 + j];
         }
@@ -2129,21 +2128,21 @@
         PHASE_BEGIN();
         real* gcen = r + ka->lay.gcen;
         int* misc = ii + ka->lay.misc;
-        GLB_PTR(int) cand = cand_();
+        const GArr<int> cand = cand_();
         int ncand = 0;
         long long tb0 = __builtin_readcyclecounter();
         const real skin = real(0.03);
-        GLB_PTR(real) gref = gref_();
-        GLB_PTR(int) nearl = near_();
+        const GArr<real> gref = gref_();
+        const GArr<int> nearl = near_();
         auto pair_hit = [&](int p, real pad) -> bool {
-            int g1 = ka->m.pair_geom[2 * p], g2 = ka->m.pair_geom[2 * p + 1];
+            int g1 = (TAB(pair_geom) + 2 * p)[0], g2 = (TAB(pair_geom) + 2 * p)[1];
             bool s1 = geom_static_()[g1], s2 = geom_static_()[g2];
-            real mg = ka->m.pair_margin[p] + pad;
+            real mg = TAB(pair_margin)[p] + pad;
             if (s1 || s2) {
                 int gs = s1 ? g1 : g2, gd = s1 ? g2 : g1;
                 real rd = geom_rbound_()[gd] + mg, d2 = 0;
                 for (int k = 0; k < 3; k++) {
-                    real c = gcen[3 * gd + k], lo = ka->m.geom_aabb0[6 * gs + k], hi = ka->m.geom_aabb0[6 * gs + 3 + k];
+                    real c = gcen[3 * gd + k], lo = (TAB(geom_aabb0) + 6 * gs)[k], hi = (TAB(geom_aabb0) + 6 * gs)[3 + k];
                     real e = c < lo ? lo - c : (c > hi ? c - hi : real(0));
                     d2 += e * e;
                 }
@@ -2157,7 +2156,7 @@
         if (misc[7]) {
             for (int g = lane; g < ka->m.ngeom; g += G)
                 if (!geom_static_()[g]) {
-                    const real d[3] = {gcen[3 * g] - gref[3 * g], gcen[3 * g + 1] - gref[3 * g + 1], gcen[3 * g + 2] - gref[3 * g + 2]};
+                    const real d[3] = {gcen[3 * g] - (gref + 3 * g)[0], gcen[3 * g + 1] - (gref + 3 * g)[1], gcen[3 * g + 2] - (gref + 3 * g)[2]};
                     moved |= dot3(d, d) > real(0.25) * skin * skin;
                 }
         }
@@ -2205,14 +2204,14 @@
         int* cpair = ii + ka->lay.cpair;
         int ncon = 0, ovf = 0;
         int* mlist = ii + ka->lay.cand;
-        GLB_PTR(real) bxo = bxo_();
+        const GArr<real> bxo = bxo_();
         for (int base = 0; base < ncand; base += G) {
             const int ci = base + lane;
             int n = 0, p = 0, nn = 0;
             LDS_PTR(real) scr = (LDS_PTR(real))(r + ka->lay.scr + SLOT_W * lane);
             const bool valid = ci < ncand;
             if (valid) p = cand[ci];
-            const int ga = ka->m.pair_geom[2 * p], gb = ka->m.pair_geom[2 * p + 1];
+            const int ga = (TAB(pair_geom) + 2 * p)[0], gb = (TAB(pair_geom) + 2 * p)[1];
             const int tya = geom_type_()[ga], tyb = geom_type_()[gb];
             const bool isbox = valid && tya == G_BOX && tyb == G_BOX;
             const long long tn0_ = profiling ? __builtin_readcyclecounter() : 0;
@@ -2288,9 +2287,9 @@
                 }
             }
             int keepmask = 0;
-            GLB_PTR(const real) ov = bxo + BOX_OVF_W * lane;
+            const GArr<const real> ov = bxo + BOX_OVF_W * lane;
             if (valid) {
-                real mg = ka->m.pair_margin[p];
+                real mg = TAB(pair_margin)[p];
                 for (int k = 0; k < nn; k++)
                     if ((isbox && k >= BOX_SLOTC ? ov[4 * (k - BOX_SLOTC)] : scr[k]) < mg) { keepmask |= 1 << k; n++; }
             }
@@ -2308,9 +2307,9 @@
                     w++;
                     if (c < ka->lay.maxcon) {
                         const bool o = isbox && k >= BOX_SLOTC;
-                        cdist[c] = o ? ov[4 * (k - BOX_SLOTC)] : scr[k];
+                        cdist[c] = o ? (ov + 4 * (k - BOX_SLOTC))[0] : scr[k];
                         cpair[c] = p;
-                        for (int q = 0; q < 3; q++) { cpos[3 * c + q] = o ? ov[4 * (k - BOX_SLOTC) + 1 + q] : scr[SLOT_P + 3 * k + q]; cnrm[3 * c + q] = scr[SLOT_N + q]; }
+                        for (int q = 0; q < 3; q++) { cpos[3 * c + q] = o ? (ov + 4 * (k - BOX_SLOTC))[1 + q] : scr[SLOT_P + 3 * k + q]; cnrm[3 * c + q] = scr[SLOT_N + q]; }
                     }
                 }
             if (ncon + tot > ka->lay.maxcon) ovf = 1;
@@ -2375,7 +2374,7 @@
             int c = base + lane, dim = 0;
             if (c < ncon) {
                 int p = cpair[c];
-                if (cdist[c] < ka->m.pair_margin[p] - ka->m.pair_gap[p]) dim = ka->m.pair_condim[p];
+                if (cdist[c] < TAB(pair_margin)[p] - TAB(pair_gap)[p]) dim = TAB(pair_condim)[p];
             }
             int off = 0, tot = 0;
             for (int j = 1; j <= 6; j++) {
@@ -2403,7 +2402,7 @@
         if (lane == 0) { misc[1] = nefc; if (ovf) misc[2] |= 2; }
         GSYNC();
         ROWPROBE(0);
-        GLB_PTR(real) rJ = rows_();
+        const GArr<real> rJ = rows_();
         real *rowS = r + ka->lay.rowS, *warm = r + ka->lay.warm, *Minv = r + ka->lay.Minv, *asm_ = r + ka->lay.asm_;
         const bool newton = ka->m.solver == 1;
         const bool lead_slim = newton && lead_per_tree();
@@ -2425,26 +2424,26 @@
             real solref[2], solimp[5];
             bool valid = true;
             if (LEAD && type == R_EQ) {
-                GLB_PTR(const real) c = ka->m.eq_polycoef + 5 * id;
-                real q1 = qpos[ka->m.eq_qpos1[id]] - ka->m.qpos0[ka->m.eq_qpos1[id]], q2 = qpos[ka->m.eq_qpos2[id]] - ka->m.qpos0[ka->m.eq_qpos2[id]];
+                const GArr<const real> c = TAB(eq_polycoef) + 5 * id;
+                real q1 = qpos[TAB(eq_qpos1)[id]] - TAB(qpos0)[TAB(eq_qpos1)[id]], q2 = qpos[TAB(eq_qpos2)[id]] - TAB(qpos0)[TAB(eq_qpos2)[id]];
                 real poly = c[0] + q2 * (c[1] + q2 * (c[2] + q2 * (c[3] + q2 * c[4])));
                 real dpoly = c[1] + q2 * (2 * c[2] + q2 * (3 * c[3] + q2 * 4 * c[4]));
-                int d1 = ka->m.eq_dof1[id], d2 = ka->m.eq_dof2[id];
+                int d1 = TAB(eq_dof1)[id], d2 = TAB(eq_dof2)[id];
                 tA = dof_tree_()[d1];
                 pos = q1 - poly;
                 diag0 = dof_invweight0_()[d1] + dof_invweight0_()[d2];
                 j1 = d1 - tree_dofadr_()[tA]; v1 = 1;
                 j2 = d2 - tree_dofadr_()[tA]; v2 = -dpoly;
-                for (int k = 0; k < 2; k++) solref[k] = ka->m.eq_solref[2 * id + k];
-                for (int k = 0; k < 5; k++) solimp[k] = ka->m.eq_solimp[5 * id + k];
+                for (int k = 0; k < 2; k++) solref[k] = (TAB(eq_solref) + 2 * id)[k];
+                for (int k = 0; k < 5; k++) solimp[k] = (TAB(eq_solimp) + 5 * id)[k];
             } else if (LEAD && type == R_FLOSS) {
                 int d = floss_dof_()[id];
                 tA = dof_tree_()[d];
                 diag0 = dof_invweight0_()[d];
                 floss = dof_frictionloss_()[d];
                 j1 = d - tree_dofadr_()[tA]; v1 = 1;
-                for (int k = 0; k < 2; k++) solref[k] = ka->m.dof_solref[2 * d + k];
-                for (int k = 0; k < 5; k++) solimp[k] = ka->m.dof_solimp[5 * d + k];
+                for (int k = 0; k < 2; k++) solref[k] = (TAB(dof_solref) + 2 * d)[k];
+                for (int k = 0; k < 5; k++) solimp[k] = (TAB(dof_solimp) + 5 * d)[k];
             } else if (LEAD && type == R_LIMIT) {
                 int j = id, d = jnt_dofadr_()[j];
                 real q = qpos[jnt_qposadr_()[j]];
@@ -2453,11 +2452,11 @@
                 margin = jnt_margin_()[j];
                 diag0 = dof_invweight0_()[d];
                 j1 = d - tree_dofadr_()[tA]; v1 = sub == 0 ? real(1) : real(-1);
-                for (int k = 0; k < 2; k++) solref[k] = ka->m.jnt_solref[2 * j + k];
-                for (int k = 0; k < 5; k++) solimp[k] = ka->m.jnt_solimp[5 * j + k];
+                for (int k = 0; k < 2; k++) solref[k] = (TAB(jnt_solref) + 2 * j)[k];
+                for (int k = 0; k < 5; k++) solimp[k] = (TAB(jnt_solimp) + 5 * j)[k];
             } else if (!LEAD) {
                 int c = id, p = cpair[c];
-                int g1 = ka->m.pair_geom[2 * p], g2 = ka->m.pair_geom[2 * p + 1], b1 = geom_body_()[g1], b2 = geom_body_()[g2];
+                int g1 = (TAB(pair_geom) + 2 * p)[0], g2 = (TAB(pair_geom) + 2 * p)[1], b1 = geom_body_()[g1], b2 = geom_body_()[g2];
                 int t1 = body_tree_()[b1], t2 = body_tree_()[b2];
                 tA = t1 >= 0 ? t1 : t2;
                 tB = (t1 >= 0 && t2 >= 0 && t2 != t1) ? t2 : -1;
@@ -2490,10 +2489,10 @@
                     }
                 }
                 pos = sub == 0 ? cdist[c] : real(0);
-                margin = ka->m.pair_margin[p] - ka->m.pair_gap[p];
+                margin = TAB(pair_margin)[p] - TAB(pair_gap)[p];
                 diag0 = body_invweight0_()[2 * b1] + body_invweight0_()[2 * b2];
-                for (int k = 0; k < 2; k++) solref[k] = ka->m.pair_solref[2 * p + k];
-                for (int k = 0; k < 5; k++) solimp[k] = ka->m.pair_solimp[5 * p + k];
+                for (int k = 0; k < 2; k++) solref[k] = (TAB(pair_solref) + 2 * p)[k];
+                for (int k = 0; k < 5; k++) solimp[k] = (TAB(pair_solimp) + 5 * p)[k];
             }
             (void)valid;
             const int j2c = j2 >= 0 ? j2 : (j1 >= 0 ? j1 : 0), j1c = j1 >= 0 ? j1 : 0;
@@ -2512,7 +2511,7 @@
                 real imp0 = imp_row;
                 real R0 = tmax(real(1e-15), (1 - imp0) * diag0 / imp0);
                 real R1 = R0 / tmax(real(1e-15), ka->m.impratio);
-                real mu0 = ka->m.pair_friction[5 * p], mur = ka->m.pair_friction[5 * p + sub - 1];
+                real mu0 = (TAB(pair_friction) + 5 * p)[0], mur = (TAB(pair_friction) + 5 * p)[sub - 1];
                 R = sub == 1 ? R1 : R1 * mu0 * mu0 / tmax(real(1e-15), mur * mur);
                 imp = imp0;
                 K = 0;
@@ -2623,7 +2622,7 @@
         GSYNC();
         ROWPROBE(2);
         int* gI = ii + ka->lay.gI;
-        GLB_PTR(real) gA = coup_();
+        const GArr<real> gA = coup_();
         const int nlead = misc[4];
         int ngrp = 0;
         for (int base = 0; base < nefc; base += G) {
@@ -2632,7 +2631,7 @@
             int cnt = 0, isc = 0;
             if (i < nefc) {
                 if (i < nlead) { head = (i % GRP_MAX) == 0; cnt = nlead - i < GRP_MAX ? nlead - i : GRP_MAX; }
-                else { int meta = rmeta[i]; head = ((meta >> 12) & 255) == 0; cnt = ka->m.pair_condim[cpair[(meta >> 2) & 1023]]; isc = 1; }
+                else { int meta = rmeta[i]; head = ((meta >> 12) & 255) == 0; cnt = TAB(pair_condim)[cpair[(meta >> 2) & 1023]]; isc = 1; }
             }
             int tot, rk = group_rank<G>(head, grp, lane, &tot);
             if (head && ngrp + rk < ka->lay.maxgrp) gI[ngrp + rk] = i | (cnt << 16) | (isc << 24);
@@ -2663,9 +2662,9 @@
             real v = 0;
             if (rr < cnt) {
                 int ir = start + rr, is = start + ss, ra = rowI[ir], rs = rowI[is];
-                GLB_PTR(const real) Jr = rJ + ROW_S * ir;
+                const GArr<const real> Jr = rJ + ROW_S * ir;
                 const bool packed_s = g >= nlg && ((rs >> 19) & 15) == 0;
-                GLB_PTR(const real) Bs = packed_s ? (GLB_PTR(const real))(rJ + ROW_S * is + TREE_W) : (GLB_PTR(const real))(rowsB_() + ROW_S * is);
+                const GArr<const real> Bs = packed_s ? GArr<const real>(rJ + ROW_S * is + TREE_W) : GArr<const real>(rowsB_() + ROW_S * is);
 #pragma unroll
                 for (int wr = 0; wr < 2; wr++) {
                     const bool on_r = ((ra >> (13 * wr + 6)) & 15) != 0;
@@ -2696,7 +2695,7 @@
                 mu[j] = in ? real(1) / S[7] : real(1);
                 A[j][j] = in ? real(1) / S[3] : real(1);
 #pragma unroll
-                for (int k = 0; k < j; k++) { const real c = in ? gA[GA_W * g + (j + 1) * j / 2 + (k + 1)] : real(0); A[j][k] = c; A[k][j] = c; }
+                for (int k = 0; k < j; k++) { const real c = in ? (gA + GA_W * g)[(j + 1) * j / 2 + (k + 1)] : real(0); A[j][k] = c; A[k][j] = c; }
             }
 #pragma unroll
             for (int i = 0; i < 5; i++)
@@ -2731,7 +2730,7 @@
             }
 #pragma unroll
             for (int j = 0; j < 5; j++) {
-                GLB_PTR(real) o = gA + GA_W * g + GA_Q + j;
+                const GArr<real> o = gA + GA_W * g + GA_Q + j;
 #pragma unroll
                 for (int k = 0; k < 5; k++) o[8 * k] = mu[j] * Inv[j][k] * mu[k];
                 o[40] = singular ? real(1) : real(0);
@@ -2751,7 +2750,7 @@
         if constexpr (spec_fixed<SPEC>) { solver = ka->m.solver; newton_iters = ka->m.newton_iters; }
         int *misc = ii + ka->lay.misc, *rmeta = ii + ka->lay.rmeta, *cefc = ii + ka->lay.cefc, *rowI = ii + ka->lay.rowI;
         real *qacc = r + ka->lay.qacc, *as = r + ka->lay.asm_, *rowS = r + ka->lay.rowS, *fcon = r + ka->lay.fcon;
-        GLB_PTR(real) rJ = rows_();
+        const GArr<real> rJ = rows_();
         int nefc = misc[1], ncon = misc[0];
         real* Minv = r + ka->lay.Minv;
         if (solver == 1) {
@@ -2785,7 +2784,7 @@
             int first = cefc[c];
             if (first < 0) continue;
             first &= 0xffff;
-            int dim = ka->m.pair_condim[(ii + ka->lay.cpair)[c]];
+            int dim = TAB(pair_condim)[(ii + ka->lay.cpair)[c]];
             real fn = rowS[RS_S * first + 6], s2 = 0;
             for (int s = 1; s < dim; s++) { real t = rowS[RS_S * (first + s) + 6] * rowS[RS_S * (first + s) + 7]; s2 += t * t; }
             if (s2 > fn * fn) { real sc = fn / sqrt(s2); for (int s = 1; s < dim; s++) rowS[RS_S * (first + s) + 6] *= sc; }
@@ -2827,9 +2826,9 @@
         for (int i = lane; i < ka->m.nv; i += G) bad |= !(fabs(qvel[i]) < real(1e6));
         if (!__any(bad)) return;
         diverged = 1;
-        for (int i = lane; i < ka->m.nq; i += G) qpos[i] = ka->m.qpos_home[i];
+        for (int i = lane; i < ka->m.nq; i += G) qpos[i] = TAB(qpos_home)[i];
         GSYNC();
-        for (int i = lane; i < nobj_() * 7; i += G) qpos[ka->m.obj_qadr[i / 7] + i % 7] = (real)ka->m.obj_reset[((size_t)env * nobj_()) * 7 + i];
+        for (int i = lane; i < nobj_() * 7; i += G) qpos[TAB(obj_qadr)[i / 7] + i % 7] = (real)glb_block((GLB_PTR(const double))ka->m.obj_reset, env, (unsigned)(nobj_() * 7))[i];
         for (int i = lane; i < ka->m.nv; i += G) { qvel[i] = 0; warm[i] = 0; }
         if (lane == 0) (ii + ka->lay.misc)[7] = 0;
         GSYNC();
@@ -2843,7 +2842,7 @@
         for (int k = lane; k < ka->m.nv; k += G) out[k] = 0;
         GSYNC();
         rows_jt_force<real>((LDS_PTR(const real))(r + ka->lay.rowS), (LDS_PTR(const int))(ii + ka->lay.rowI), (LDS_PTR(const int))(ii + ka->lay.cefc),
-                            (GLB_PTR(const real))rows_(), (LDS_PTR(real))out, misc[4], misc[0], lane, real(1));
+                            GArr<const real>(rows_()), (LDS_PTR(real))out, misc[4], misc[0], lane, real(1));
         GSYNC();
     }
 
@@ -3399,6 +3398,7 @@
                 }
             }
             if (ovf.size() / 4 >= (1u << 24)) throw std::runtime_error("support table: overflow part too large");
+            if ((tab.size() + ovf.size()) * sizeof(real) >= (1ull << 32)) throw std::runtime_error("support table: 4 GiB or more, beyond the 32-bit offsets of the device's table reads");
             m.hull_ovf = (int)(tab.size() / 4);
             tab.insert(tab.end(), ovf.begin(), ovf.end());
             if (tab.empty()) tab.assign(4, 0.0);
```
